# LSimon95/megatts2

Measured on AMD Instinct MI355X. Metric: mel-frames/sec (whole node), higher is better.
Workload: dtype f32; 1 GPU; C3: B=32/GPU x 1 GPU, Np=70, Tp=431, Tm=431; stages vqpe+mrte+adm+plm+decoder+vocoder; forced durations; weights=synthetic (name-seeded), parallelism=dp1 (utterance shards, one RCCL all-gather of mels per step)

## Files before the change

### include/megatts2_hip.h

```cpp
#ifndef MEGATTS2_HIP_H
#define MEGATTS2_HIP_H

#include <stddef.h>
#include <stdint.h>

#ifdef __cplusplus
extern "C" {
#endif

typedef struct mt2_model mt2_model;

typedef struct mt2_config {
    int32_t mel_bins, mrte_hidden, mrte_kernel, mrte_stride, mrte_n_layer, mrte_n_stack, mrte_n_block;
    int32_t content_ff_dim, content_n_heads, content_n_layers, phone_vocab;
    int32_t vq_mel_bins, vq_stride, vq_hidden, vq_kernel, vq_n_layers, vq_n_stacks, vq_n_blocks, vq_bins, vq_dim;
    int32_t dec_kernel, dec_hidden, dec_n_stack, dec_n_block;
    int32_t plm_layers, plm_heads, plm_vq_dim, plm_tc_dim, plm_bins;
    int32_t adm_layers, adm_heads, adm_emb_dim, adm_tc_dim, adm_tc_emb_dim;
    int32_t hg_in_dim, hg_init_channels, hg_n_up, hg_up_rates[8], hg_up_kernels[8];
    int32_t hg_n_res, hg_res_kernels[4], hg_res_dilations[4][3];
    float hg_slope;
    int32_t max_positions;
    int32_t hg_inference_padding;
    int32_t hg_reflect_pad;
// ... 174 lines not shown
    int32_t struct_bytes;
    const float* X; long long strideX; int32_t ldx, Rx;
    const int32_t* rowbase; int32_t a_mul, shift0, taps, dil, Cin;
    const float* W; long long strideW; int32_t ldw;
    const void* W3; long long w3_plane;
    const void* Wh; const float* wh_inv; long long wh_ldb, wh_gstride, wh_inv_stride;
    int32_t a_planes;
    const float* bias; long long strideB;
    const float* R; long long strideR; int32_t ldr;
    const int32_t* valid;
    float* C; long long strideC; int32_t ldc;
    int32_t M, N, groups;
    int32_t pro_act; float pro_slope; int32_t epi_act; float out_scale;
    int32_t force_cfg;
    int32_t* range_flag;
    int32_t* cfg_out;
} mt2_gemm_desc;
int mt2_op_gemm_grouped(void* stream, const mt2_gemm_desc* d);
int mt2_x3h_guard(mt2_model* m, int* tripped);
int mt2_op_gemm_x6_ln(void* stream, const float* X, int ldx, int Rx, int a_mul, int shift0, const float* W, const void* W3,
                      const float* bias, const float* R, int ldr, float* C, int ldc, int M, int N, int K, int epi_act,
                      int force_cfg, float* stat_out, int32_t* stat_nt, int32_t* stat_w, const float* ln_stat, int ln_nt,
                      int ln_w, const float* ln_s, float ln_eps);
int mt2_op_tile_major(void* stream, const float* W, int N, int K, float* out);
int mt2_op_gemm_tm(void* stream, const float* X, long long x_gstride, int ldx, int Rx, int a_mul, int shift0, const float* Wtm,
                   int Kw, int n0, int k0, long long w_gstride, int groups, const float* bias, const float* R, int ldr,
                   const int32_t* valid, float* C, long long c_gstride, int ldc, int M, int N, int K, int pro_act, float pro_slope,
                   int epi_act, const float* ln_gamma, const float* ln_beta, float ln_eps);
int mt2_op_gemm_tm_pairs(void* stream, const float* X, int ldx, int Rx, int a_mul, int shift0, const float* Wtm, int Kw,
                         const float* bias, const float* R, int ldr, float* C, int ldc, int M, int N, int K, int epi_act,
                         const float* ln_gamma, const float* ln_beta, float ln_eps, float* stat_out, const float* ln_stat, int ln_nt);
int mt2_op_layernorm(void* stream, const float* x, int ldx, const float* gamma, const float* beta, const float* R1,
                     int ldr1, const int32_t* valid, float* out, int ldo, int M, int C, float eps, int act);
int mt2_op_layernorm_ex(void* stream, const float* x, int ldx, const float* gamma, const float* beta, int rows_per_group,
                        const float* R1, int ldr1, int r1_rows, const float* R2, int ldr2, const int32_t* valid, int valid_rows,
                        float* out, int ldo, int M, int C, float eps, int act, int out_planes, int32_t* x3h_flag);
int mt2_op_ln_reduce(void* stream, const float* parts, long long pstride, int S, const float* bias, const float* R, int ldr,
                     const float* gamma, const float* beta, float* xout, int ldx, float* hout, int ldh, int M, int C, float eps,
                     int h_planes, int32_t* x3h_flag);
int mt2_op_row(void* stream, const char* op, void* const* ptrs, int nptrs, const long long* ints, int nints, const float* flts,
               int nflts);
int mt2_op_sample_rows(void* stream, const float* logits, int ld, int N, int A, const mt2_sampling* s, const uint64_t* seeds_dev,
                       const int32_t* positions_dev, int64_t* out);
int mt2_op_sample_mix_rows(void* stream, const float* logits, int ld, int N, int A, const mt2_sampling* s,
                           const uint64_t* seeds_dev, const int32_t* positions_dev, const float* gamma_dev, int64_t* out);
int mt2_op_attention(void* stream, const float* Q, int ldq, const float* K, int ldk, const float* V, int ldv,
                     float* O, int ldo, const int32_t* q_start, const int32_t* q_len, const int32_t* kv_start,
                     const int32_t* kv_len, int B, int H, int D, int max_qlen, float scale);
int mt2_op_attention_tuned(void* stream, const float* Q, int ldq, const float* K, int ldk, const float* V, int ldv,
                           float* O, int ldo, const int32_t* q_start, const int32_t* q_len, const int32_t* kv_start,
                           const int32_t* kv_len, int B, int H, int D, int max_qlen, float scale, int lds_min_qlen,
                           int lds_waves, int x6_min_qlen, int max_kvlen);
int mt2_op_attention_x3h(void* stream, const float* Q, int ldq, const float* K, int ldk, const float* V, int ldv,
                         float* O, int ldo, const int32_t* q_start, const int32_t* q_len, const int32_t* kv_start,
                         const int32_t* kv_len, int B, int H, int D, int max_qlen, float scale, int lds_waves, int max_kvlen,
                         int32_t* range_flag);
enum { MT2_ATTN_NONE = 0, MT2_ATTN_GENERIC = 1, MT2_ATTN_REG = 2, MT2_ATTN_DS = 3, MT2_ATTN_LDS = 4, MT2_ATTN_X6 = 5, MT2_ATTN_X3H = 6 };
typedef struct mt2_attn_desc {
    int32_t struct_bytes;
    const float* Q; int32_t ldq;
    const float* K; int32_t ldk;
    const float* V; int32_t ldv;
    float* O; int32_t ldo;
    const int32_t* q_start; const int32_t* q_len; const int32_t* kv_start; const int32_t* kv_len; const int32_t* o_start;
    int32_t u_qstride, u_qlen, u_kvstride, u_kvlen, u_ostride;
    int32_t B, H, D, max_qlen, max_kvlen; float scale;
    int32_t lds_min_qlen, x6_min_qlen, lds_waves, ds_short, x3h, o_planes;
    int32_t* range_flag;
    int32_t* kernel_out;
} mt2_attn_desc;
int mt2_op_attention_desc(void* stream, const mt2_attn_desc* d);
int mt2_attention_route(const mt2_attn_desc* d, int32_t* err, int32_t* kernel, int32_t* tmpl, int32_t* launch, long long* lds);
int mt2_gemm_trace_begin(mt2_model* m);
int mt2_gemm_trace_end(mt2_model* m, int cap, const char** names, int64_t* launches, double* flops, double* ms);
int mt2_gemm_trace_shapes(mt2_model* m, char* buf, int cap, int top);
int mt2_gemm_config_count(void);
const char* mt2_gemm_config_name(int idx);
int mt2_gemm_route(int M, int N, int K, int taps, int dil, int groups, int pro_act, int operands, int misaligned, int force_cfg,
                   int x3h, int* err, int* cfg, int* variant, long long* lds, int* planes);
int mt2_op_gemm_x3h_ln(void* stream, const float* X, int ldx, int Rx, int a_mul, int shift0, const float* W, const void* W3,
                       const void* Wh, const float* wh_inv, const float* bias, const float* R, int ldr, float* C, int ldc, int M, int N,
                       int K, int epi_act, int force_cfg, float* stat_out, int32_t* stat_nt, int32_t* stat_w, const float* ln_stat,
                       int ln_nt, int ln_w, const float* ln_s, float ln_eps);
int mt2_bench_gemm(void* stream, int M, int N, int K, int taps, int dil, int flags, int force_cfg, int iters,
                   int w_copies, float* avg_ms, char* cfg_name, int cfg_name_cap, double* sustained_ghz);

#ifdef __cplusplus
}
#endif
#endif
```

### megatts2_amd/csrc/capi.inc

```

#include <climits>

namespace mt2 {
extern thread_local std::string g_last_error;
void finalize_model(mt2_model& m);
}

using namespace mt2;

#define MT2_API_BEGIN try {
#define MT2_API_END                                 \
    ::CallScope::verdict_of_open_call();            \
    return 0;                                       \
    }                                               \
    catch (const std::exception& e) {               \
        g_last_error = e.what();                    \
        return -1;                                  \
    }                                               \
    catch (...) {                                   \
        g_last_error = "unknown error";             \
        return -1;                                  \
    }

enum Need { NEED_G = 1, NEED_ADM = 2, NEED_PLM = 4, NEED_VOC = 8 };
// ... 1121 lines not shown
    MT2_HIP(launch_gemm(p, (hipStream_t)stream, &o));
    MT2_API_END
}

int mt2_op_gemm_x6(void* stream, const float* X, int ldx, int Rx, int shift0, int taps, int dil, int Cin, const float* W,
                   const void* W3, const float* bias, const float* R, int ldr, const int32_t* valid, float* C, int ldc,
                   int M, int N, int pro_act, float pro_slope, int epi_act, int force_cfg) {
    MT2_API_BEGIN
    GemmP p{};
    p.X = X; p.ldx = ldx; p.Rx = Rx; p.a_mul = 1; p.shift0 = shift0; p.taps = taps; p.dil = dil; p.Cin = Cin; p.W = W;
    p.W3 = W3; p.ldw = taps * Cin; p.bias = bias; p.R = R; p.ldr = ldr; p.valid = valid; p.C = C; p.ldc = ldc; p.M = M;
    p.N = N; p.K = taps * Cin; p.groups = 1; p.pro_act = pro_act; p.pro_slope = pro_slope; p.epi_act = epi_act;
    p.out_scale = 1.0f;
    EngineOpts o;
    o.force_cfg = force_cfg;
    MT2_HIP(launch_gemm(p, (hipStream_t)stream, &o));
    MT2_API_END
}

int mt2_op_gemm_x3h(void* stream, const float* X, int ldx, int Rx, int shift0, int taps, int dil, int Cin, const float* W,
                    const void* W3, const void* Wh, const float* wh_inv, const float* bias, const float* R, int ldr,
                    const int32_t* valid, float* C, int ldc, int M, int N, int pro_act, float pro_slope, int epi_act, int force_cfg,
                    int32_t* range_flag) {
    MT2_API_BEGIN
    GemmP p{};
    p.X = X; p.ldx = ldx; p.Rx = Rx; p.a_mul = 1; p.shift0 = shift0; p.taps = taps; p.dil = dil; p.Cin = Cin; p.W = W;
    p.W3 = W3; p.Wh = Wh; p.wh_inv = wh_inv; p.ldw = taps * Cin; p.bias = bias; p.R = R; p.ldr = ldr; p.valid = valid; p.C = C;
    p.ldc = ldc; p.M = M; p.N = N; p.K = taps * Cin; p.groups = 1; p.pro_act = pro_act; p.pro_slope = pro_slope; p.epi_act = epi_act;
    p.out_scale = 1.0f;
    EngineOpts o;
    if (force_cfg >= 4000) { p.c_planes = 1; force_cfg -= 4000; }
    if (force_cfg >= 2000) { p.a_planes = 1; force_cfg -= 2000; }
    o.ldr64 = force_cfg >= 1000;
    o.force_cfg = force_cfg >= 1000 ? force_cfg - 1000 : force_cfg;
    o.x3h_flag = range_flag;
    MT2_HIP(launch_gemm(p, (hipStream_t)stream, &o));
    MT2_API_END
}
int mt2_x3h_split(const float* W, long long rows, long long row_len, uint16_t* planes, float* inv) {
    MT2_API_BEGIN
    MT2_REQUIRE(W && planes && inv && rows > 0 && row_len > 0, "bad arguments");
    x3h_split_rows(W, (size_t)rows, (size_t)row_len, planes, inv);
    MT2_API_END
}
int mt2_x3h_group_planes(long long row_len, long long w_off, long long ldw, long long strideW, long long groups, int32_t* form,
                         long long* wh_off, long long* wh_ldb, long long* wh_gstride, long long* inv_off, long long* wh_inv_stride) {
    MT2_API_BEGIN
    MT2_REQUIRE(row_len > 0 && w_off >= 0 && groups >= 1 && form && wh_off && wh_ldb && wh_gstride && inv_off && wh_inv_stride,
                "bad arguments");
    const X3hGroupPlanes g = x3h_group_planes(row_len, w_off, ldw, strideW, groups);
    *form = g.form; *wh_off = g.wh_off; *wh_ldb = g.wh_ldb; *wh_gstride = g.wh_gstride; *inv_off = g.inv_off;
    *wh_inv_stride = g.wh_inv_stride;
    MT2_API_END
}

int mt2_op_gemm_grouped(void* stream, const mt2_gemm_desc* d) {
    MT2_API_BEGIN
    MT2_REQUIRE(d != nullptr, "null descriptor");
    MT2_REQUIRE(d->struct_bytes == (int32_t)sizeof(mt2_gemm_desc), "descriptor size mismatch");
    if (d->cfg_out) *d->cfg_out = -1;
    GemmP p{};
    p.X = d->X; p.strideX = d->strideX; p.ldx = d->ldx; p.Rx = d->Rx;
    p.rowbase = d->rowbase; p.a_mul = d->a_mul; p.shift0 = d->shift0; p.taps = d->taps; p.dil = d->dil; p.Cin = d->Cin;
    p.W = d->W; p.strideW = d->strideW; p.ldw = d->ldw;
    p.W3 = d->W3; p.w3_plane = d->w3_plane;
    p.Wh = d->Wh; p.wh_inv = d->wh_inv; p.wh_ldb = d->wh_ldb; p.wh_gstride = d->wh_gstride; p.wh_inv_stride = d->wh_inv_stride;
    p.a_planes = d->a_planes;
    p.bias = d->bias; p.strideB = d->strideB; p.R = d->R; p.strideR = d->strideR; p.ldr = d->ldr; p.valid = d->valid;
    p.C = d->C; p.strideC = d->strideC; p.ldc = d->ldc;
    p.M = d->M; p.N = d->N; p.K = d->taps * d->Cin; p.groups = d->groups;
    p.pro_act = d->pro_act; p.pro_slope = d->pro_slope; p.epi_act = d->epi_act; p.out_scale = d->out_scale;
    MT2_REQUIRE(p.X && p.W && p.C && p.taps >= 1 && p.dil >= 1 && p.a_mul >= 1 && p.groups >= 1, "bad arguments");
    EngineOpts o;
    o.force_cfg = d->force_cfg;
    o.x3h_flag = d->range_flag;
    if (d->cfg_out) *d->cfg_out = gemm_route(p, o).cfg;
    MT2_HIP(launch_gemm(p, (hipStream_t)stream, &o));
    MT2_API_END
}

static int op_gemm_ln_impl(void* stream, const float* X, int ldx, int Rx, int a_mul, int shift0, const float* W, const void* W3,
                           const void* Wh, const float* wh_inv, const float* bias, const float* R, int ldr, float* C, int ldc, int M,
                           int N, int K, int epi_act, int force_cfg, float* stat_out, int32_t* stat_nt, int32_t* stat_w,
                           const float* ln_stat, int ln_nt, int ln_w, const float* ln_s, float ln_eps);
int mt2_op_gemm_x6_ln(void* stream, const float* X, int ldx, int Rx, int a_mul, int shift0, const float* W, const void* W3,
                      const float* bias, const float* R, int ldr, float* C, int ldc, int M, int N, int K, int epi_act,
                      int force_cfg, float* stat_out, int32_t* stat_nt, int32_t* stat_w, const float* ln_stat, int ln_nt,
                      int ln_w, const float* ln_s, float ln_eps) {
    return op_gemm_ln_impl(stream, X, ldx, Rx, a_mul, shift0, W, W3, nullptr, nullptr, bias, R, ldr, C, ldc, M, N, K, epi_act, force_cfg,
                           stat_out, stat_nt, stat_w, ln_stat, ln_nt, ln_w, ln_s, ln_eps);
}
int mt2_op_gemm_x3h_ln(void* stream, const float* X, int ldx, int Rx, int a_mul, int shift0, const float* W, const void* W3,
                       const void* Wh, const float* wh_inv, const float* bias, const float* R, int ldr, float* C, int ldc, int M, int N,
                       int K, int epi_act, int force_cfg, float* stat_out, int32_t* stat_nt, int32_t* stat_w, const float* ln_stat,
                       int ln_nt, int ln_w, const float* ln_s, float ln_eps) {
    return op_gemm_ln_impl(stream, X, ldx, Rx, a_mul, shift0, W, W3, Wh, wh_inv, bias, R, ldr, C, ldc, M, N, K, epi_act, force_cfg,
                           stat_out, stat_nt, stat_w, ln_stat, ln_nt, ln_w, ln_s, ln_eps);
}
static int op_gemm_ln_impl(void* stream, const float* X, int ldx, int Rx, int a_mul, int shift0, const float* W, const void* W3,
                           const void* Wh, const float* wh_inv, const float* bias, const float* R, int ldr, float* C, int ldc, int M,
                           int N, int K, int epi_act, int force_cfg, float* stat_out, int32_t* stat_nt, int32_t* stat_w,
                           const float* ln_stat, int ln_nt, int ln_w, const float* ln_s, float ln_eps) {
    MT2_API_BEGIN
    GemmP p{};
    p.Wh = Wh; p.wh_inv = wh_inv;
    p.X = X; p.ldx = ldx; p.Rx = Rx; p.a_mul = a_mul ? a_mul : 1; p.shift0 = shift0; p.taps = 1; p.dil = 1; p.Cin = K; p.W = W;
    p.W3 = W3; p.ldw = K; p.bias = bias; p.R = R; p.ldr = ldr; p.C = C; p.ldc = ldc; p.M = M; p.N = N; p.K = K; p.groups = 1;
    p.epi_act = epi_act; p.out_scale = 1.0f; p.stat_out = stat_out;
    if (ln_stat) { p.pro_act = 5; p.ln_stat = ln_stat; p.ln_nt = ln_nt; p.ln_w = ln_w; p.ln_g = ln_s; p.ln_eps = ln_eps; }
    EngineOpts o;
    o.ldr64 = force_cfg >= 1000;
    o.force_cfg = force_cfg >= 1000 ? force_cfg - 1000 : force_cfg;
    const hipError_t e = launch_gemm(p, (hipStream_t)stream, &o);
    MT2_REQUIRE(e != hipErrorNotSupported, "this tile configuration has no pair-fed LayerNorm form");
    MT2_HIP(e);
    if (stat_nt) *stat_nt = o.last_stat_nt;
    if (stat_w) *stat_w = o.last_stat_w;
    MT2_API_END
}

int mt2_op_tile_major(void* stream, const float* W, int N, int K, float* out) {
    MT2_API_BEGIN
    MT2_REQUIRE(W && out && N > 0 && K > 0 && N % 16 == 0 && K % 64 == 0, "tile-major layout needs N % 16 == 0 and K % 64 == 0");
    MT2_HIP(launch_tile_major(W, N, K, out, (hipStream_t)stream));
    MT2_API_END
}

int mt2_op_gemm_tm(void* stream, const float* X, long long x_gstride, int ldx, int Rx, int a_mul, int shift0, const float* Wtm,
                   int Kw, int n0, int k0, long long w_gstride, int groups, const float* bias, const float* R, int ldr,
                   const int32_t* valid, float* C, long long c_gstride, int ldc, int M, int N, int K, int pro_act, float pro_slope,
                   int epi_act, const float* ln_gamma, const float* ln_beta, float ln_eps) {
    MT2_API_BEGIN
    MT2_REQUIRE(X && Wtm && C && Kw % 64 == 0 && n0 % 16 == 0 && k0 % 64 == 0 && groups >= 1, "bad arguments");
    GemmP p{};
    p.X = X; p.strideX = x_gstride; p.ldx = ldx; p.Rx = Rx; p.a_mul = a_mul ? a_mul : 1; p.shift0 = shift0; p.taps = 1; p.dil = 1;
    p.Cin = K; p.K = K; p.W = nullptr; p.strideW = w_gstride; p.ldw = Kw; p.Wtm = Wtm; p.tm_n0 = n0 / 16; p.tm_k0 = k0 / 64;
    p.tm_kb = Kw / 64; p.bias = bias; p.R = R; p.ldr = ldr; p.valid = valid; p.C = C; p.strideC = c_gstride; p.ldc = ldc;
    p.M = M; p.N = N; p.groups = groups; p.pro_act = ln_gamma ? 3 : (pro_act & 0xff); p.pro_slope = pro_slope; p.epi_act = epi_act;
    p.sk_nw = (pro_act & 0x100) ? 8 : 16;
    p.out_scale = 1.0f; p.ln_g = ln_gamma; p.ln_b = ln_beta; p.ln_eps = ln_eps;
    MT2_REQUIRE(gemm_skinny_tm_eligible(p, 64), "shape not served by the tile-major weight-streaming kernel");
    MT2_HIP(launch_gemm_skinny_tm(p, (hipStream_t)stream));
    MT2_API_END
}

int mt2_op_gemm_tm_pairs(void* stream, const float* X, int ldx, int Rx, int a_mul, int shift0, const float* Wtm, int Kw,
                         const float* bias, const float* R, int ldr, float* C, int ldc, int M, int N, int K, int epi_act,
                         const float* ln_gamma, const float* ln_beta, float ln_eps, float* stat_out, const float* ln_stat, int ln_nt) {
    MT2_API_BEGIN
    MT2_REQUIRE(X && Wtm && C && Kw % 64 == 0, "bad arguments");
    GemmP p{};
    p.X = X; p.ldx = ldx; p.Rx = Rx; p.a_mul = a_mul ? a_mul : 1; p.shift0 = shift0; p.taps = 1; p.dil = 1; p.Cin = K; p.K = K;
    p.ldw = Kw; p.Wtm = Wtm; p.tm_kb = Kw / 64; p.bias = bias; p.R = R; p.ldr = ldr; p.C = C; p.ldc = ldc; p.M = M; p.N = N; p.groups = 1;
    p.pro_act = ln_gamma ? 3 : 0; p.epi_act = epi_act; p.out_scale = 1.0f; p.ln_g = ln_gamma; p.ln_b = ln_beta; p.ln_eps = ln_eps;
    p.stat_out = stat_out; p.ln_stat = ln_stat; p.ln_nt = ln_nt; p.ln_w = ln_stat ? 16 : 0;
    EngineOpts o;
    hipError_t e = launch_gemm(p, (hipStream_t)stream, &o);
    MT2_HIP(e);
    MT2_REQUIRE(!stat_out || o.last_stat_w == 16, "the launch did not take the tile-major route with the statistics epilogue");
    MT2_API_END
}

int mt2_op_layernorm(void* stream, const float* x, int ldx, const float* gamma, const float* beta, const float* R1,
                     int ldr1, const int32_t* valid, float* out, int ldo, int M, int C, float eps, int act) {
    MT2_API_BEGIN
    LnP p{};
    p.x = x; p.ldx = ldx; p.gamma = gamma; p.beta = beta; p.R1 = R1; p.ldr1 = ldr1; p.valid = valid;
    p.out = out; p.ldo = ldo; p.M = M; p.C = C; p.eps = eps; p.act = act >= 100 ? act - 100 : act;
    p.out_planes = act >= 100 ? 1 : 0;
    MT2_HIP(launch_layernorm(p, (hipStream_t)stream));
    MT2_API_END
}

int mt2_op_layernorm_ex(void* stream, const float* x, int ldx, const float* gamma, const float* beta, int rows_per_group,
                        const float* R1, int ldr1, int r1_rows, const float* R2, int ldr2, const int32_t* valid, int valid_rows,
                        float* out, int ldo, int M, int C, float eps, int act, int out_planes, int32_t* x3h_flag) {
    MT2_API_BEGIN
    LnP p{};
    p.x = x; p.ldx = ldx; p.gamma = gamma; p.beta = beta; p.rows_per_group = rows_per_group;
    p.R1 = R1; p.ldr1 = ldr1; p.r1_rows = r1_rows; p.R2 = R2; p.ldr2 = ldr2; p.valid = valid; p.valid_rows = valid_rows;
    p.out = out; p.ldo = ldo; p.M = M; p.C = C; p.eps = eps; p.act = act; p.out_planes = out_planes; p.x3h_flag = x3h_flag;
    MT2_HIP(launch_layernorm(p, (hipStream_t)stream));
    MT2_API_END
}

int mt2_op_ln_reduce(void* stream, const float* parts, long long pstride, int S, const float* bias, const float* R, int ldr,
                     const float* gamma, const float* beta, float* xout, int ldx, float* hout, int ldh, int M, int C, float eps,
                     int h_planes, int32_t* x3h_flag) {
    MT2_API_BEGIN
    LnReduceP p{};
    p.parts = parts; p.pstride = pstride; p.S = S; p.bias = bias; p.R = R; p.ldr = ldr; p.gamma = gamma; p.beta = beta;
    p.xout = xout; p.ldx = ldx; p.hout = hout; p.ldh = ldh; p.M = M; p.C = C; p.eps = eps; p.h_planes = h_planes;
    p.x3h_flag = x3h_flag;
    MT2_HIP(launch_ln_reduce(p, (hipStream_t)stream));
    MT2_API_END
}

static int row_int(long long v) {
    MT2_REQUIRE(v >= INT_MIN && v <= INT_MAX, "mt2_op_row: integer argument does not fit the launcher's int parameter");
    return (int)v;
// ... 331 lines not shown
```

### megatts2_amd/csrc/gemm_common.h

```cpp
#pragma once
#include "gemm_tiles.h"
#include "planes_store.h"
#include <type_traits>
#include <utility>

namespace mt2 {

typedef float f32x16 __attribute__((ext_vector_type(16)));
typedef float f32x4 __attribute__((ext_vector_type(4)));

template <int ACT>
__device__ __forceinline__ float apply_act(float v, float slope) {
    if (ACT == ACT_RELU) return fmaxf(v, 0.0f);
    if (ACT == ACT_LRELU) return fmaxf(v, v * slope);
    if (ACT == ACT_TANH) return tanhf(v);
    return v;
}

__device__ __forceinline__ float act_rt(int act, float v, float slope) {
    switch (act) {
        case ACT_RELU: return fmaxf(v, 0.0f);
        case ACT_LRELU: return v >= 0.0f ? v : v * slope;
        case ACT_TANH: return tanhf(v);
        case ACT_LOGCLAMP: return logf(fmaxf(v, slope));
// ... 43 lines not shown
    const int nq = p.ln_nt >> 1;
    const float4* __restrict__ pr = reinterpret_cast<const float4*>(p.ln_stat) + (long long)(ok ? src : 0) * nq;
    float4 q[NQ];
#pragma unroll
    for (int j = 0; j < NQ; ++j) {
        const int qi = j * LPR + part;
        q[j] = (ok && qi < nq) ? pr[qi] : make_float4(0.f, 0.f, 0.f, 0.f);
    }
    float sm = 0.0f;
#pragma unroll
    for (int j = 0; j < NQ; ++j) sm += q[j].x + q[j].z;
#pragma unroll
    for (int o = 1; o < LPR; o <<= 1) sm += __shfl_xor(sm, o * xm);
    const float mean = sm / (float)p.ln_nt, w = (float)p.ln_w;
    float m2 = 0.0f;
#pragma unroll
    for (int j = 0; j < NQ; ++j) {
        const int qi = j * LPR + part;
        if (qi < nq) {
            const float d0 = q[j].x - mean, d1 = q[j].z - mean;
            m2 += (q[j].y + w * d0 * d0) + (q[j].w + w * d1 * d1);
        }
    }
#pragma unroll
    for (int o = 1; o < LPR; o <<= 1) m2 += __shfl_xor(m2, o * xm);
    mu = ok ? mean : 0.0f;
    rs = ok ? 1.0f / sqrtf(m2 / ((float)p.ln_nt * w) + p.ln_eps) : 0.0f;
}

template <int TM, int TN, int EPG = 16>
__device__ __forceinline__ void epilogue(const GemmP& p, f32x16 (&acc)[TM][TN], int g, int mw, int nw, int lane,
                                         int esel = 0) {
    const float* __restrict__ bias = p.bias ? p.bias + (long long)g * p.strideB : nullptr;
    const float* __restrict__ R = p.R ? p.R + (long long)g * p.strideR : nullptr;
    float* __restrict__ C = p.C + (long long)g * p.strideC;
    const int epi_act = p.epi_act;
    const float epi_par = p.pro_slope;
    const float out_scale = p.out_scale;
#pragma unroll
    for (int j = 0; j < TN; ++j) {
        const int n = nw + j * 32 + (lane & 31);
        const bool nok = n < p.N;
        const float bv = (bias && nok) ? bias[n] : 0.0f;
#pragma unroll
        for (int i = 0; i < TM; ++i) {
#pragma unroll
            for (int e = 0; e < 16; ++e) {
                if (EPG < 16 && e / EPG != esel) continue;
                const int m = mw + i * 32 + (e & 3) + 8 * (e >> 2) + 4 * (lane >> 5);
                if (nok && m < p.M) {
                    float v = acc[i][j][e] + bv;
                    v = act_rt(epi_act, v, epi_par) * out_scale;
                    if (R) v += R[(long long)m * p.ldr + n];
                    if (p.valid && p.valid[m] == 0) v = 0.0f;
                    C[(long long)m * p.ldc + n] = v;
                }
            }
        }
    }
}

static __device__ __attribute__((aligned(16))) float g_zero16[4] = {0.f, 0.f, 0.f, 0.f};
static __device__ int g_one_i[4] = {1, 1, 1, 1};
template <int NE> struct EpiPre { float r[NE]; int v[NE]; float b; };
template <int NE>
__device__ __forceinline__ void epi_prefetch(const GemmP& p, EpiPre<NE>& q, int g, int mw, int nw, int lane, int e0) {
    const int n = nw + (lane & 31);
    const bool nok = n < p.N;
    const float* __restrict__ bias = p.bias ? p.bias + (long long)g * p.strideB + (nok ? n : 0) : g_zero16;
    const float* __restrict__ R = p.R ? p.R + (long long)g * p.strideR + (nok ? n : 0) : g_zero16;
    const long long ldr = p.R ? p.ldr : 0;
    const int* __restrict__ vp = p.valid ? p.valid : g_one_i;
    const int vs = p.valid ? 1 : 0;
    q.b = *bias;
#pragma unroll
    for (int i = 0; i < NE; ++i) {
        const int e = e0 + i;
        int m = mw + (e & 3) + 8 * (e >> 2) + 4 * (lane >> 5);
        m = m < p.M ? m : 0;
        q.r[i] = R[m * ldr];
        q.v[i] = vp[m * vs];
    }
}
template <int NE, bool STAT = false>
__device__ __forceinline__ void epilogue_pre(const GemmP& p, const float (&acc)[NE], const EpiPre<NE>& q, int g, int mw,
                                             int nw, int lane, int e0) {
    float* __restrict__ C = p.C + (long long)g * p.strideC;
    const int epi_act = p.epi_act;
    const float epi_par = p.pro_slope;
    const float out_scale = p.out_scale;
    const bool hasR = p.R != nullptr;
    const int n = nw + (lane & 31);
    const bool nok = n < p.N;
    float sv[STAT ? NE : 1], qv[STAT ? NE : 1];
#pragma unroll
    for (int i = 0; i < NE; ++i) {
        const int e = e0 + i;
        const int m = mw + (e & 3) + 8 * (e >> 2) + 4 * (lane >> 5);
        float v = 0.0f;
        if (nok && m < p.M) {
            v = acc[i] + q.b;
            v = act_rt(epi_act, v, epi_par) * out_scale;
            if (hasR) v += q.r[i];
            if (q.v[i] == 0) v = 0.0f;
            C[(long long)m * p.ldc + n] = v;
        }
        if constexpr (STAT) { sv[i] = v; qv[i] = v * v; }
    }
    if constexpr (STAT) emit_row_pairs<NE>(p, sv, qv, mw, nw >> 5, 32.0f, lane, e0);
}

template <int TM, int TN> struct EpiPreT { float r[TM][TN][16]; int v[TM][16]; float b[TN]; };
template <int TM, int TN>
__device__ __forceinline__ void epi_prefetch_t(const GemmP& p, EpiPreT<TM, TN>& q, int g, int mw, int nw, int lane) {
    const float* __restrict__ bias0 = p.bias ? p.bias + (long long)g * p.strideB : g_zero16;
    const float* __restrict__ R0 = p.R ? p.R + (long long)g * p.strideR : g_zero16;
    const long long ldr = p.R ? p.ldr : 0;
    const int* __restrict__ vp = p.valid ? p.valid : g_one_i;
    const int vs = p.valid ? 1 : 0;
#pragma unroll
    for (int j = 0; j < TN; ++j) {
        const int n = nw + j * 32 + (lane & 31);
        const int nc = (n < p.N && (p.bias || p.R)) ? n : 0;
        q.b[j] = bias0[p.bias ? nc : 0];
#pragma unroll
        for (int i = 0; i < TM; ++i)
#pragma unroll
            for (int e = 0; e < 16; ++e) {
                int m = mw + i * 32 + (e & 3) + 8 * (e >> 2) + 4 * (lane >> 5);
                m = m < p.M ? m : 0;
                q.r[i][j][e] = R0[m * ldr + (p.R ? nc : 0)];
            }
    }
#pragma unroll
    for (int i = 0; i < TM; ++i)
#pragma unroll
        for (int e = 0; e < 16; ++e) {
            int m = mw + i * 32 + (e & 3) + 8 * (e >> 2) + 4 * (lane >> 5);
            m = m < p.M ? m : 0;
            q.v[i][e] = vp[m * vs];
        }
}
template <int TM, int TN, bool STAT = false>
__device__ __forceinline__ void epilogue_pre_t(const GemmP& p, f32x16 (&acc)[TM][TN], const EpiPreT<TM, TN>& q, int g,
                                               int mw, int nw, int lane) {
    static_assert(!STAT || TM == 1, "row statistics: one 32-row block per wave");
    float* __restrict__ C = p.C + (long long)g * p.strideC;
    const int epi_act = p.epi_act;
    const float epi_par = p.pro_slope;
    const float out_scale = p.out_scale;
    const bool hasR = p.R != nullptr;
    float sv[STAT ? 16 : 1], qv[STAT ? 16 : 1];
    if constexpr (STAT) {
#pragma unroll
        for (int e = 0; e < 16; ++e) { sv[e] = 0.0f; qv[e] = 0.0f; }
    }
#pragma unroll
    for (int j = 0; j < TN; ++j) {
        const int n = nw + j * 32 + (lane & 31);
        const bool nok = n < p.N;
#pragma unroll
        for (int i = 0; i < TM; ++i)
#pragma unroll
            for (int e = 0; e < 16; ++e) {
                const int m = mw + i * 32 + (e & 3) + 8 * (e >> 2) + 4 * (lane >> 5);
                float v = 0.0f;
                if (nok && m < p.M) {
                    v = acc[i][j][e] + q.b[j];
                    v = act_rt(epi_act, v, epi_par) * out_scale;
                    if (hasR) v += q.r[i][j][e];
                    if (q.v[i][e] == 0) v = 0.0f;
                    C[(long long)m * p.ldc + n] = v;
                }
                if constexpr (STAT) { sv[e] += v; qv[e] += v * v; }
            }
    }
    if constexpr (STAT) emit_row_pairs<16>(p, sv, qv, mw, nw / (32 * TN), 32.0f * TN, lane, 0);
}

__device__ __forceinline__ float dpp_quad(float v, const int ctrl) {
    return __builtin_bit_cast(float, ctrl == 0xB1 ? __builtin_amdgcn_mov_dpp(__builtin_bit_cast(int, v), 0xB1, 0xf, 0xf, true)
                                                  : __builtin_amdgcn_mov_dpp(__builtin_bit_cast(int, v), 0x4E, 0xf, 0xf, true));
}
__device__ __forceinline__ bool epilogue_t4_ok(const GemmP& p) {
    return ((p.N | p.ldc | (p.R ? p.ldr : 0)) & 3) == 0 && (((unsigned long long)p.C | (unsigned long long)p.R | (unsigned long long)p.bias) & 15) == 0 &&
           ((p.strideC | p.strideR | p.strideB) & 3) == 0;
}
template <int TM, int TN, bool STAT = false, bool PLN = false>
__device__ __forceinline__ void epilogue_t4(const GemmP& p, f32x16 (&acc)[TM][TN], int g, int mw, int nw, int lane) {
    static_assert(!STAT || TM == 1, "row statistics: one 32-row block per wave");
    float* __restrict__ C = p.C + (long long)g * p.strideC;
    const int epi_act = p.epi_act;
    const float epi_par = p.pro_slope, out_scale = p.out_scale;
    const bool b0 = lane & 1, b1 = lane & 2;
    const int rr = (lane & 3) + 4 * (lane >> 5), c4 = ((lane & 31) >> 2) * 4;
    const bool hasR = p.R != nullptr, hasB = p.bias != nullptr;
    const float* __restrict__ bias0 = hasB ? p.bias + (long long)g * p.strideB : g_zero16;
    const float* __restrict__ R0 = hasR ? p.R + (long long)g * p.strideR : g_zero16;
    const long long ldr = hasR ? p.ldr : 0;
    const int* __restrict__ vp = p.valid ? p.valid : g_one_i;
    const int vs = p.valid ? 1 : 0;
    f32x4 bv[TN], rv[TM][TN][4];
    int vm[TM][4];
#pragma unroll
    for (int j = 0; j < TN; ++j) {
        const int n = nw + j * 32 + c4;
        bv[j] = *reinterpret_cast<const f32x4*>(bias0 + ((hasB && n < p.N) ? n : 0));
    }
#pragma unroll
    for (int i = 0; i < TM; ++i)
#pragma unroll
        for (int q = 0; q < 4; ++q) {
            int m = mw + i * 32 + 8 * q + rr;
            m = m < p.M ? m : 0;
            vm[i][q] = vp[m * vs];
#pragma unroll
            for (int j = 0; j < TN; ++j) {
                const int n = nw + j * 32 + c4;
                rv[i][j][q] = *reinterpret_cast<const f32x4*>(R0 + m * ldr + ((hasR && n < p.N) ? n : 0));
            }
        }
    float sv[STAT ? 4 : 1], qv[STAT ? 4 : 1];
    if constexpr (STAT) {
#pragma unroll
        for (int q = 0; q < 4; ++q) { sv[q] = 0.0f; qv[q] = 0.0f; }
    }
#pragma unroll
    for (int j = 0; j < TN; ++j) {
        const int n = nw + j * 32 + c4;
        const bool nok = n < p.N;
#pragma unroll
        for (int i = 0; i < TM; ++i) {
#pragma unroll
            for (int q = 0; q < 4; ++q) {
                const float x0 = acc[i][j][4 * q], x1 = acc[i][j][4 * q + 1], x2 = acc[i][j][4 * q + 2], x3 = acc[i][j][4 * q + 3];
                const float p0 = dpp_quad(x0, 0xB1), p1 = dpp_quad(x1, 0xB1), p2 = dpp_quad(x2, 0xB1), p3 = dpp_quad(x3, 0xB1);
                const float y0 = b0 ? p1 : x0, y1 = b0 ? x1 : p0, y2 = b0 ? p3 : x2, y3 = b0 ? x3 : p2;
                const float q0 = dpp_quad(y0, 0x4E), q1 = dpp_quad(y1, 0x4E), q2 = dpp_quad(y2, 0x4E), q3 = dpp_quad(y3, 0x4E);
                f32x4 v = {b1 ? q2 : y0, b1 ? q3 : y1, b1 ? y2 : q0, b1 ? y3 : q1};
                const int m = mw + i * 32 + 8 * q + rr;
                const bool in = nok && m < p.M;
                if (in) {
#pragma unroll
                    for (int e = 0; e < 4; ++e) v[e] = act_rt(epi_act, v[e] + bv[j][e], epi_par) * out_scale;
                    if (hasR) {
#pragma unroll
                        for (int e = 0; e < 4; ++e) v[e] += rv[i][j][q][e];
                    }
                    if (vm[i][q] == 0) v = f32x4{0.f, 0.f, 0.f, 0.f};
                    if (PLN && p.c_planes) {
                        if (store_planes4(C + (long long)m * p.ldc, n, v[0], v[1], v[2], v[3]) >= 65504.0f && p.x3h_flag) atomicOr(p.x3h_flag, 1);
                    } else
                    *reinterpret_cast<f32x4*>(C + (long long)m * p.ldc + n) = v;
                }
                if constexpr (STAT) {
                    if (!in) v = f32x4{0.f, 0.f, 0.f, 0.f};
                    sv[q] += (v[0] + v[1]) + (v[2] + v[3]);
                    qv[q] += (v[0] * v[0] + v[1] * v[1]) + (v[2] * v[2] + v[3] * v[3]);
                }
            }
        }
    }
    if constexpr (STAT) {
        const float w_cols = 32.0f * TN;
        const int t = nw / (32 * TN);
#pragma unroll
        for (int q = 0; q < 4; ++q) {
            float S = sv[q], Q = qv[q];
#pragma unroll
            for (int o = 4; o < 32; o <<= 1) { S += __shfl_xor(S, o); Q += __shfl_xor(Q, o); }
            const int m = mw + 8 * q + rr;
            if ((lane & 28) == 0 && m < p.M) {
                const float mean = S / w_cols;
                float2 pr;
                pr.x = mean;
                pr.y = fmaxf(Q - S * mean, 0.0f);
                *reinterpret_cast<float2*>(p.stat_out + ((long long)m * p.stat_nt + t) * 2) = pr;
            }
        }
    }
}

constexpr int PRO_APL = 3;

__device__ __forceinline__ f32x4 lds_read_b128(unsigned byte_addr) {
    f32x4 v;
    asm volatile("ds_read_b128 %0, %1" : "=v"(v) : "v"(byte_addr) : "memory");
    return v;
}

template <int OFF>
__device__ __forceinline__ f32x4 lds_read_b128_imm(unsigned byte_addr) {
    static_assert(OFF >= 0 && OFF < 65536 && (OFF & 15) == 0, "ds_read_b128 immediate offset");
    f32x4 v;
    asm volatile("ds_read_b128 %0, %1 offset:%2" : "=v"(v) : "v"(byte_addr), "n"(OFF) : "memory");
    return v;
}
template <int... Is, typename F>
__device__ __forceinline__ void static_for(std::integer_sequence<int, Is...>, F&& f) {
    (f(std::integral_constant<int, Is>{}), ...);
}

__device__ __forceinline__ void loader_priority(int prio) {
    if (prio >= 3) __builtin_amdgcn_s_setprio(3);
    else if (prio == 2) __builtin_amdgcn_s_setprio(2);
    else if (prio == 1) __builtin_amdgcn_s_setprio(1);
}

template <int N> __device__ __forceinline__ void wait_vmcnt() {
    static_assert(N >= 0 && N < 64, "vmcnt is a 6-bit field on gfx9");
    __builtin_amdgcn_s_waitcnt((N & 0xF) | ((N >> 4) << 14) | (7 << 4) | (15 << 8));
}

}
```

### megatts2_amd/csrc/gemm_dispatch.hip

```cpp
#include "gemm_tiles.h"

#include <algorithm>
#include <atomic>
#include <cstdio>
#include <cstdlib>
#include <utility>
#include <vector>

namespace mt2 {


static const TileCfg kSkinnyRows[] = {
    { CFG_SKINNY32, 32, 32, 512, 0, "skinny32_f32", {} },
    { CFG_SKINNY64, 64, 32, 512, 0, "skinny64_f32", {} },
    { CFG_SKINNYTM32, 32, 32, 512, 0, "skinnytm32_f32", {} },
    { CFG_SKINNYTM64, 64, 32, 512, 0, "skinnytm64_f32", {} },
};
static const struct { int index; const char* name; } kRetired[] = {
    {0, "retired:128x128_2x2"}, {1, "retired:64x128_2x2"}, {2, "retired:128x64_2x2"}, {4, "retired:32x128_1x4"},
    {5, "retired:32x64_1x2"}, {6, "retired:128x32_4x1"}, {7, "retired:64x32_2x1"},
    {8, "retired:dma128x128_2x2_s3"}, {9, "retired:dma128x128_2x2_s4"}, {10, "retired:dma64x128_2x2_s4"},
    {11, "retired:dma64x64_2x2_s4"}, {13, "retired:dma32x128_1x4_s4"}, {14, "retired:dma32x64_1x2_s4"},
    {19, "retired:dma64x64_2x2_k2_s4"}, {21, "retired:dma32x64_1x2_k4_s3"}, {24, "retired:dma128x64_4x2_s4"},
    {25, "retired:dma128x64_4x2_s2"}, {26, "retired:dma64x64_2x2_k1_s2"}, {27, "retired:dma128x64_4x2_k2_s2"},
// ... 115 lines not shown
        fl_all += fl;
        ++n;
    }
    if (ok && n < cap && !iv.empty()) {
        std::sort(iv.begin(), iv.end());
        double uni = 0.0, lo = iv[0].first, hi = iv[0].second;
        for (auto& x : iv) {
            if (x.first > hi) { uni += hi - lo; lo = x.first; hi = x.second; }
            else if (x.second > hi) hi = x.second;
        }
        uni += hi - lo;
        names[n] = "union"; launches[n] = (int64_t)iv.size(); flops[n] = fl_all; ms[n] = uni;
        ++n;
    }
    for (auto& r : tr) { (void)hipEventDestroy(r.e0); (void)hipEventDestroy(r.e1); }
    tr.clear();
    return ok ? n : -1;
}

template <typename F>
static hipError_t traced_launch(EngineOpts* opts, int cfg, const GemmP& p, hipStream_t s, F&& launch) {
    if (opts) opts->last_cfg = gemm_config_name(cfg);
    if (!(opts && opts->trace_on)) return launch();
    TraceRec r;
    r.cfg = cfg;
    r.flops = 2.0 * p.M * p.N * p.K * p.groups;
    r.M = p.M; r.N = p.N; r.K = p.K; r.groups = p.groups;
    if (hipEventCreate(&r.e0) != hipSuccess || hipEventCreate(&r.e1) != hipSuccess) return hipErrorUnknown;
    (void)hipEventRecord(r.e0, s);
    const hipError_t e = launch();
    (void)hipEventRecord(r.e1, s);
    opts->trace.push_back(r);
    return e;
}


static bool win_eligible(const GemmP& p) {
    return p.taps >= 2 && !p.rowbase && p.a_mul == 1 && p.groups == 1 && p.N == p.Cin &&
           (p.Cin == 32 || p.Cin == 64 || p.Cin == 128) && (p.taps - 1) * p.dil <= 64 && p.pro_act < PRO_LN;
}
static int choose_cfg(const GemmP& p, const EngineOpts& o) {
    const bool forced = o.force_cfg >= 0 && o.force_cfg < kNumCfgs;
    const bool x3h_ok = p.Wh && p.wh_inv;
    if (o.win_conv && win_eligible(p) && !forced) {
        int bi = p.Cin == 32 ? CFG_WIN256x32 : (p.Cin == 64 ? CFG_WIN256x64 : CFG_WIN128x128);
        if (o.x6_conv && p.W3) {
            bi = paired(kX6Form, bi);
            if ((o.x3h & 4) && x3h_ok) bi = paired(kX3hForm, bi);
        }
        return bi;
    }
    if (forced) return o.force_cfg;
    const long long t32 = (long long)((p.M + 31) / 32) * ((p.N + 63) / 64) * p.groups;
    const long long t32x32 = (long long)((p.M + 31) / 32) * ((p.N + 31) / 32) * p.groups;
    const long long t64 = (long long)((p.M + 63) / 64) * ((p.N + 63) / 64) * p.groups;
    const long long t128 = (long long)((p.M + 127) / 128) * ((p.N + 127) / 128) * p.groups;
    const long long t256 = (long long)((p.M + 255) / 256) * ((p.N + 127) / 128) * p.groups;
    int bi = CFG_DMA64x64_S3;
    if (p.N <= 32) bi = CFG_DMA128x32_S4;
    else if (p.N <= 64 && t128 >= 400) bi = CFG_DMA256x64_S3;
    else if (p.N <= 256 && t128 >= 400) bi = CFG_DMA128x128_S4;
    else if (t256 >= 400 || (t256 >= 200 && t256 <= 256)) bi = CFG_DMA256x128_S3;
    else if (t128 >= 400 || (t128 >= 200 && t128 <= 256)) bi = CFG_DMA128x128_S4;
    else if (t32x32 <= o.t32x32 && p.K >= 512) bi = CFG_DMA32x32_K8;
    else if (t32 <= o.t32) bi = CFG_DMA32x64_K4;
    else if (t64 <= o.t_ks4) bi = CFG_DMA64x64_K4;
    else if (t64 <= o.t_ks2) bi = CFG_DMA64x64_K2;
    if (o.x6_gemm && p.W3 && (p.K & 7) == 0 && (p.ldw & 7) == 0 && (p.pro_act < PRO_LN || p.pro_act == PRO_LNX) && p.N > 64) {
        const bool h1 = (o.x3h & 1) && x3h_ok;
        if (t256 >= o.t_x6_256) bi = CFG_X6LDR256x128;
        else if (t128 >= (h1 ? o.t_x3h_128 : o.t_x6_128)) bi = CFG_X6LDR128x128;
        if (o.x6_ks && p.taps == 1) {
            if (bi == CFG_DMA32x64_K4 && p.K % (BK * 4) == 0 && o.x6_ks != 5) bi = paired(kX6Form, bi);
            else if ((bi == CFG_DMA64x64_K4 || bi == CFG_DMA64x64_K2) && p.K % (BK * 2) == 0) bi = paired(kX6Form, bi);
            else if ((o.x6_ks == 2 || o.x6_ks == 4) && bi == CFG_DMA32x32_K8 && p.K % (BK * 8) == 0) bi = paired(kX6Form, bi);
        }
    }
    if ((o.x3h & 1) && x3h_ok && (bi == CFG_X6LDR128x128 || bi == CFG_X6LDR256x128)) bi = paired(kX3hForm, bi);
    if ((o.x3h & 2) && x3h_ok && cfg_table().row[bi]->pipe == PIPE_X6 && cfg_table().row[bi]->x6_ks) bi = paired(kX3hForm, bi);
    return bi;
}


static bool a_planes_ok(const GemmP& p, const TileCfg& c, bool stat) {
    return c.pipe == PIPE_X3H && !c.win_qs && p.pro_act == ACT_NONE && !stat && (p.Cin % BK) == 0 && (p.ldx % BK) == 0 &&
           !(p.groups > 1 && (p.strideX % BK) != 0) && p.a_mul == 1 && !p.rowbase && !(((unsigned long long)p.X) & 127);
}
static bool c_planes_ok(const GemmP& p, const TileCfg& c, bool stat) {
    return c.pipe == PIPE_X3H && !c.x6_ks && !c.win_qs && p.groups == 1 && !p.R && !stat && (p.N & 31) == 0 && (p.ldc & 31) == 0 &&
           (((unsigned long long)p.C) & 127) == 0 && (((unsigned long long)p.bias) & 15) == 0 && ((p.strideC | p.strideB) & 3) == 0 && p.Wh && p.wh_inv && p.M > 64;
}
static long long wh_ldb_of(const GemmP& p) { return p.wh_ldb ? p.wh_ldb : 4ll * ((p.ldw + 31) / 32 * 32); }
static long long wh_gstride_of(const GemmP& p) { return p.groups > 1 && p.wh_gstride == 0 ? p.strideW * 4 : p.wh_gstride; }

GemmRoute gemm_route(const GemmP& p, const EngineOpts& o) {
    GemmRoute r{hipSuccess, -1, V_NONE, 0, 0, 0};
    const auto fail = [&r](hipError_t e) { r.err = e; r.lds = 0; r.stat_nt = r.stat_w = 0; return r; };
    if (p.M <= 0 || p.N <= 0 || p.groups <= 0) return r;
    if ((p.Cin & 3) || (p.ldx & 3) || (p.ldw & 3) || p.K != p.taps * p.Cin) return fail(hipErrorInvalidValue);
    if (p.pro_act < 0 || p.pro_act > PRO_LNX) return fail(hipErrorInvalidValue);
    if (p.c_planes && p.M <= 64) return fail(hipErrorNotSupported);
    if (p.pro_act == PRO_LNX && (p.taps != 1 || p.groups != 1 || !p.ln_g || !p.ln_stat || p.ln_nt < 2 || p.ln_nt > 32 ||
                                 (p.ln_nt & 1) || p.ln_w <= 0 || p.ln_nt * p.ln_w != p.K || (((unsigned long long)p.ln_stat) & 15)))
        return fail(hipErrorInvalidValue);
    const bool sk_forced = o.force_cfg == CFG_SKINNY32 || o.force_cfg == CFG_SKINNY64;
    const bool tm_forced = o.force_cfg == CFG_SKINNYTM32 || o.force_cfg == CFG_SKINNYTM64;
    if (tm_forced || (!p.a_planes && o.skinny_tm && o.skinny_rows > 0 && o.force_cfg < 0 &&
                      gemm_skinny_tm_eligible(p, o.skinny_rows))) {
        if (!gemm_skinny_tm_eligible(p, 64)) return fail(hipErrorInvalidValue);
        r.cfg = p.M <= 32 ? CFG_SKINNYTM32 : CFG_SKINNYTM64;
        if (p.stat_out) {
            const int nt = p.N / 16;
            if (p.groups == 1 && (nt & 1) == 0 && nt <= 64 && ((((unsigned long long)p.stat_out) & 15) == 0)) { r.stat_nt = nt; r.stat_w = 16; }
        }
        return r;
    }
    if (sk_forced || (o.skinny_rows > 0 && o.force_cfg < 0 && gemm_skinny_eligible(p, o.skinny_rows))) {
        if (!gemm_skinny_eligible(p, 64)) return fail(hipErrorInvalidValue);
        r.cfg = p.M <= 32 ? CFG_SKINNY32 : CFG_SKINNY64;
        return r;
    }
    r.cfg = choose_cfg(p, o);
    const TileCfg* c = cfg_table().row[r.cfg];
    if (!c) return fail(hipErrorNotSupported);
    const bool x3h = c->pipe == PIPE_X3H, x3h_ldr = x3h && !c->x6_ks && !c->win_qs;
    const bool has_lnx = c->stat_w && c->fn[V_LNX];
    if (p.pro_act == PRO_LNX && !has_lnx) return fail(hipErrorNotSupported);
    bool stat = p.stat_out != nullptr;
    if (x3h_ldr && (p.pro_act == PRO_LNX || stat)) {
        const bool t4 = ((p.N | p.ldc | (p.R ? p.ldr : 0)) & 3) == 0 && ((p.strideC | p.strideR | p.strideB) & 3) == 0 &&
                        (((unsigned long long)p.C | (unsigned long long)p.R | (unsigned long long)p.bias) & 15) == 0;
        if (!t4) {
            if (p.pro_act == PRO_LNX) return fail(hipErrorNotSupported);
            stat = false;
        }
    }
    if (stat) {
        const int nt = c->stat_w ? p.N / c->stat_w : 0;
        stat = has_lnx && (p.pro_act == ACT_NONE || p.pro_act == PRO_LNX) && p.groups == 1 && p.N % c->stat_w == 0 && nt >= 2 &&
               nt <= 32 && (nt & 1) == 0 && ((((unsigned long long)p.stat_out) & 15) == 0);
        if (stat) { r.stat_w = c->stat_w; r.stat_nt = nt; }
    }
    if (p.a_planes && !a_planes_ok(p, *c, stat)) return fail(hipErrorNotSupported);
    if (p.c_planes && !c_planes_ok(p, *c, stat)) return fail(hipErrorNotSupported);
    if (p.pro_act == PRO_LN || p.pro_act == PRO_LNA) return fail(hipErrorNotSupported);
    r.variant = p.a_planes ? V_APLANES : ((p.pro_act == PRO_LNX || stat) ? V_LNX : (GemmVariant)p.pro_act);
    r.lds = c->lds;
    if (r.variant == V_LNX && !c->x6_ks) r.lds += (size_t)c->bm * 2 * sizeof(float);
    if (x3h) {
        if (!p.Wh || !p.wh_inv || (p.K & 7) || (p.ldw & 7)) return fail(hipErrorInvalidValue);
        if ((((unsigned long long)p.Wh) & 127) || (wh_ldb_of(p) & 127) || (wh_gstride_of(p) & 127)) return fail(hipErrorInvalidValue);
    } else if (c->pipe == PIPE_X6 && (!p.W3 || (p.K & 7) || (p.ldw & 7))) return fail(hipErrorInvalidValue);
    if (c->x6_ks && (p.taps != 1 || p.K % (BK * c->x6_ks) != 0)) return fail(hipErrorInvalidValue);
    if (c->win_qs) {
        if (!win_eligible(p) || p.Cin != 32 * c->win_qs) return fail(hipErrorInvalidValue);
        const int wrp = (c->bm + (p.taps - 1) * p.dil + 7) & ~7;
        r.lds = c->lds + (size_t)c->win_qs * wrp * BK * sizeof(float);
    }
    if (!c->fn[r.variant]) return fail(hipErrorNotSupported);
    return r;
}

static GemmP normalise(GemmP p) {
    if (p.taps <= 0) p.taps = 1;
    if (p.groups <= 0) p.groups = 1;
    if (p.a_mul == 0) p.a_mul = 1;
    p.K = p.taps * p.Cin;
    if (p.ldw == 0) p.ldw = p.K;
    return p;
}
bool gemm_takes_planes(const GemmP& p_in, const EngineOpts& o) {
    const GemmP p = normalise(p_in);
    if (!(o.x3h & 3) || o.force_cfg >= 0 || p.M <= 64 || !p.Wh || !p.wh_inv) return false;
    const TileCfg* c = cfg_table().row[choose_cfg(p, o)];
    return a_planes_ok(p, *c, p.stat_out != nullptr) && c->fn[V_APLANES] != nullptr;
}
bool gemm_writes_planes(const GemmP& p_in, const EngineOpts& o) {
    const GemmP p = normalise(p_in);
    if (!(o.x3h & 1) || o.force_cfg >= 0 || p.M <= 64) return false;
    return c_planes_ok(p, *cfg_table().row[choose_cfg(p, o)], p.stat_out != nullptr);
}

static std::atomic<unsigned long long> g_attr_done[kNumCfgs][kGemmVariants];

hipError_t launch_gemm(const GemmP& p_in, hipStream_t s, EngineOpts* opts) {
    static const EngineOpts kDefaults;
    const EngineOpts& o = opts ? *opts : kDefaults;
    const GemmRoute r = gemm_route(p_in, o);
    if (r.cfg < 0 && r.err == hipSuccess) return hipSuccess;
    if (opts) { opts->last_stat_nt = r.stat_nt; opts->last_stat_w = r.stat_w; }
    if (r.err != hipSuccess) return r.err;
    GemmP p = p_in;
    if (!r.stat_nt) p.stat_out = nullptr;
    p.stat_nt = r.stat_nt; p.stat_w = r.stat_w;
    if (r.cfg == CFG_SKINNYTM32 || r.cfg == CFG_SKINNYTM64) {
        p.sk_nw = o.skinny_nw;
        return traced_launch(opts, r.cfg, p, s, [&] { return launch_gemm_skinny_tm(p, s); });
    }
    if (r.cfg == CFG_SKINNY32 || r.cfg == CFG_SKINNY64) return traced_launch(opts, r.cfg, p, s, [&] { return launch_gemm_skinny(p, s); });
    const TileCfg* c = cfg_table().row[r.cfg];
    if (c->pipe == PIPE_X3H) {
        p.wh_ldb = wh_ldb_of(p);
        p.wh_gstride = wh_gstride_of(p);
        p.x3h_flag = o.x3h_flag;
    }
    if (c->pipe == PIPE_X6 && p.w3_plane == 0) p.w3_plane = (long long)p.N * p.ldw;
    const GemmKernel fn = c->fn[r.variant];
    const size_t lds_attr = c->win_qs ? c->lds + (size_t)c->win_qs * ((c->bm + 64 + 7) & ~7) * BK * sizeof(float) : r.lds;
    const hipError_t e = dyn_lds_once(g_attr_done[r.cfg][r.variant], reinterpret_cast<const void*>(fn), lds_attr);
    if (e != hipSuccess) return e;
    const int tiles = ((p.M + c->bm - 1) / c->bm) * ((p.N + c->bn - 1) / c->bn);
    p.epi_t4 = 1;
    p.ldr_prio = o.ldr_prio;
    p.ldr64 = o.ldr64 ? 1 : 0;
    const dim3 grid(tiles, 1, p.groups), block(c->threads);
    return traced_launch(opts, r.cfg, p, s, [&] {
        hipLaunchKernelGGL(fn, grid, block, r.lds, s, p);
        return hipGetLastError();
    });
}

}
```

### megatts2_amd/csrc/gemm_tiles.h

```cpp
#pragma once
#include "mt2_kernels.h"

namespace mt2 {

constexpr int BK = 32;
constexpr int PRO_LN = 3;
constexpr int PRO_LNA = 4;
constexpr int PRO_LNX = 5;

enum GemmVariant : int {
    V_NONE, V_RELU, V_LRELU,
    V_APLANES,
    V_LNX,
    kGemmVariants
};
static_assert((int)V_NONE == ACT_NONE && (int)V_RELU == ACT_RELU && (int)V_LRELU == ACT_LRELU, "the activation variants are indexed by Act");

enum GemmPipe : int { PIPE_F32, PIPE_X6, PIPE_X3H };

enum CfgIndex : int {
    CFG_64x64 = 3,
    CFG_DMA64x64_S3 = 12, CFG_DMA128x32_S4 = 15, CFG_DMA256x128_S3 = 16, CFG_DMA128x128_S4 = 17,
    CFG_DMA64x64_K2 = 18, CFG_DMA64x64_K4 = 20, CFG_DMA32x64_K4 = 22, CFG_DMA256x64_S3 = 23, CFG_DMA32x32_K8 = 28,
    CFG_WIN256x32 = 30, CFG_WIN256x64 = 31, CFG_WIN128x128 = 32,
    CFG_X6WIN256x32 = 34,
    CFG_X6LDR256x128 = 51, CFG_X6LDR128x128 = 55,
    CFG_X6WINL256x64 = 58, CFG_X6WINL128x128 = 59,
    CFG_X6KS32x64_K4 = 84, CFG_X6KS64x64_K2 = 85, CFG_X6KS32x32_K8 = 86,
    CFG_SKINNY32 = 87, CFG_SKINNY64 = 88, CFG_SKINNYTM32 = 89, CFG_SKINNYTM64 = 90,
    CFG_X3HKS32x64_K4 = 95, CFG_X3HKS64x64_K2 = 96, CFG_X3HKS32x32_K8 = 97,
    CFG_X3HWIN256x32 = 98, CFG_X3HWIN256x64 = 99, CFG_X3HWIN128x128 = 100,
    CFG_X3HLDR128x128 = 103,
    kNumCfgs = 106
};

typedef void (*GemmKernel)(GemmP);
struct TileCfg {
    CfgIndex index;
    int bm, bn, threads;
    size_t lds;
    const char* name;
    GemmKernel fn[kGemmVariants];
    GemmPipe pipe = PIPE_F32;
    int win_qs = 0;
    int x6_ks = 0;
    int stat_w = 0;
};
struct TileRows { const TileCfg* rows; int n; };
TileRows gemm_f32_tile_rows();
TileRows gemm_x3h_tile_rows();

}
```

### megatts2_amd/csrc/gemm_x3h.hip

```cpp
#include "gemm_common.h"

#include <atomic>

#ifndef MT2_X3H_ABLATE
#define MT2_X3H_ABLATE 0
#endif
#define MT2_ABL_NOINGEST (MT2_X3H_ABLATE == 2 || MT2_X3H_ABLATE == 5 || MT2_X3H_ABLATE == 6 || MT2_X3H_ABLATE == 7)
#define MT2_ABL_NOSPLIT (MT2_X3H_ABLATE == 3 || MT2_X3H_ABLATE == 5 || MT2_X3H_ABLATE == 6)
#define MT2_ABL_NOBARRIER (MT2_X3H_ABLATE == 6 || MT2_X3H_ABLATE == 7)
#ifdef MT2_X3H_NO_BUFFER_LOADS
#define MT2_BUFFER_LOADS false
#else
#define MT2_BUFFER_LOADS true
#endif

namespace mt2 {

typedef _Float16 f16x8 __attribute__((ext_vector_type(8)));
typedef _Float16 f16x2 __attribute__((ext_vector_type(2)));
typedef float f32x2 __attribute__((ext_vector_type(2)));
typedef unsigned u32x4 __attribute__((ext_vector_type(4)));

constexpr float kX3hLoScale = 2048.0f, kX3hLoInv = 1.0f / 2048.0f, kX3hMaxIn = 65504.0f;

// ... 130 lines not shown
                for (int j = 0; j < A_IT; ++j) {
                    const int src = abase[j] + dsrc;
                    const long long off = (unsigned)src < (unsigned)Rx ? (long long)src * ldx + (s_cc + akl[j]) : zoff_x;
                    __builtin_amdgcn_global_load_lds((const __attribute__((address_space(1))) void*)(X + off),
                                                     (__attribute__((address_space(3))) void*)(As + j * NL * 256), 16, 0, 0);
                }
#pragma unroll
                for (int j = 0; j < B_IT; ++j) {
                    const long long off = wofs[j] >= 0 ? wofs[j] + (long long)kchunk * 4 : zoff_w;
                    __builtin_amdgcn_global_load_lds((const __attribute__((address_space(1))) void*)(Wh + off),
                                                     (__attribute__((address_space(3))) void*)(Bs + j * NL * 1024), 16, 0, 0);
                }
                s_cc += BK;
                if (multi_tap && s_cc == Cin) { s_cc = 0; ++s_tap; }
                return;
            }
#pragma unroll
            for (int j = 0; j < A_IT; ++j) {
                const int k = kchunk + akl[j];
                int tap = 0, cc = k;
                if (multi_tap) { tap = k / Cin; cc = k - tap * Cin; }
                const int src = abase[j] + tap * dil;
                const bool ok = (k < Kt) & ((unsigned)src < (unsigned)Rx);
                const long long off = ok ? (long long)src * ldx + cc : zoff_x;
                __builtin_amdgcn_global_load_lds((const __attribute__((address_space(1))) void*)(X + off),
                                                 (__attribute__((address_space(3))) void*)(As + j * NL * 256), 16, 0, 0);
            }
#pragma unroll
            for (int j = 0; j < B_IT; ++j) {
                const bool ok = (kchunk < Kt) & (wofs[j] >= 0);
                const long long off = ok ? wofs[j] + (long long)kchunk * 4 : zoff_w;
                __builtin_amdgcn_global_load_lds((const __attribute__((address_space(1))) void*)(Wh + off),
                                                 (__attribute__((address_space(3))) void*)(Bs + j * NL * 1024), 16, 0, 0);
            }
        };
#pragma unroll
        for (int st = 0; st < NST - 1; ++st)
            if (st < nk) issue(st, st);
#ifdef MT2_PHASE_TIMING
        const bool lprobe = p.dbg != nullptr && bid == (int)(gridDim.x / 2) && lw == 0;
        unsigned long long lacc[3] = {0, 0, 0}, lprev = lprobe ? __builtin_readcyclecounter() : 0ull;
#define MT2_LT(i_) do { if (lprobe) { const unsigned long long t_ = __builtin_readcyclecounter(); lacc[i_] += t_ - lprev; lprev = t_; } } while (0)
#define MT2_LT_END() do { if (lprobe && lane == 0) { p.dbg[11] = lacc[0]; p.dbg[12] = lacc[1]; p.dbg[13] = lacc[2]; } } while (0)
#else
#define MT2_LT(i_) do { } while (0)
#define MT2_LT_END() do { } while (0)
#endif
        static_assert(NST >= 3, "cross-chunk form: chunk c-1 is still being read at barrier c");
        for (int c = 0; c < nk; ++c) {
            if (c == 0) { if (NST - 2 < nk) wait_vmcnt<(NST - 2) * L>(); else wait_vmcnt<0>(); }
            else if (c + NST - 3 < nk) wait_vmcnt<(NST - 3) * L>();
            else wait_vmcnt<0>();
            MT2_LT(0);
            if (!MT2_ABL_NOBARRIER || c == 0)
            __builtin_amdgcn_s_barrier();
            MT2_LT(1);
#if MT2_ABL_NOINGEST
            if (c >= 1 && c + NST - 2 < nk && c < 2) {
#else
            if (c >= 1 && c + NST - 2 < nk) {
#endif
                const int cs = (c + NST - 2) % NST;
                issue(c + NST - 2, cs);
            }
            MT2_LT(2);
        }
        MT2_LT_END();
#undef MT2_LT
#undef MT2_LT_END
        return;
    }

    const int wave = wave_all;
    const int wm = wave / WGN, wn = wave % WGN;
    float inv_s[TN];
    {
        const float* __restrict__ inv = p.wh_inv + (long long)g * p.wh_inv_stride;
#pragma unroll
        for (int j = 0; j < TN; ++j) {
            const int n = n0 + wn * WTN + j * 32 + (lane & 31);
            inv_s[j] = inv[n < p.N ? n : 0];
        }
    }
    constexpr bool LNXOK = TM == 1 && TM * TN <= 2 && PRO == PRO_LNX;
    const bool lnx = LNXOK && p.pro_act == PRO_LNX;
    [[maybe_unused]] float* lnstat = reinterpret_cast<float*>(ring + NST * STAGE);
    if constexpr (LNXOK) {
        if (lnx) {
            constexpr int LPR = NW * 64 / BM;
            static_assert(LPR >= 1 && LPR <= 16 && (LPR & (LPR - 1)) == 0, "lanes per row");
            const int tc = wave * 64 + lane, row = tc / LPR;
            float mu, rs;
            lnx_row_stats<LPR>(p, m0 + row, tc % LPR, 1, mu, rs);
            if (tc % LPR == 0) { lnstat[2 * row] = mu; lnstat[2 * row + 1] = rs; }
            asm volatile("s_waitcnt lgkmcnt(0)" ::: "memory");
        }
    }

    f32x16 acc[TM][TN], acl[TM][TN];
#pragma unroll
    for (int i = 0; i < TM; ++i)
#pragma unroll
        for (int j = 0; j < TN; ++j)
#pragma unroll
            for (int e = 0; e < 16; ++e) { acc[i][j][e] = 0.0f; acl[i][j][e] = 0.0f; }

    const float pro_slope = p.pro_slope;
    const int half = lane >> 5;
    const unsigned lds0 = (unsigned)(unsigned long long)(__attribute__((address_space(3))) char*)ring;
    const int swza = (lane >> 1) & 7;
    const unsigned a_lane = lds0 + ((wm * WTM + (lane & 31)) * BK) * 4;
    const int nrow = wn * WTN + (lane & 31);
    const int swzb = (nrow >> 1) & 7;
    const unsigned b_lane = lds0 + STAGE_A + nrow * 128;
    unsigned koffa[2][2], koffb[2][2];
#pragma unroll
    for (int b = 0; b < 2; ++b) {
        koffa[b][0] = (unsigned)(((b * 4 + half * 2) ^ swza) * 16);
        koffa[b][1] = (unsigned)(((b * 4 + half * 2 + 1) ^ swza) * 16);
        koffb[b][0] = (unsigned)(((b * 2 + half) ^ swzb) * 16);
        koffb[b][1] = (unsigned)(((4 + b * 2 + half) ^ swzb) * 16);
    }

    float amax = 0.0f;
    const bool probe = p.dbg != nullptr && bid == (int)(gridDim.x / 2) && wave == 0;
    unsigned long long treal0 = 0, tcyc0 = 0;
    if (probe) {
        treal0 = __builtin_amdgcn_s_memrealtime();
        tcyc0 = __builtin_readcyclecounter();
        if (lane == 0) p.dbg[9] = treal0 - t_entry;
    }
    if constexpr (PRO == PRO_APL) {
        constexpr int N1 = 2 * TM + 2 * TN;
        static_assert(N1 <= 15, "lgkmcnt is four bits wide");
        u32x4 ra[2][TM][2];
        u32x4 rb[2][2][TN];
        unsigned koffah[2][2];
#pragma unroll
        for (int b = 0; b < 2; ++b) {
            koffah[b][0] = (unsigned)(((b * 2 + half) ^ swza) * 16);
            koffah[b][1] = (unsigned)(((4 + b * 2 + half) ^ swza) * 16);
        }
        auto fetch_a = [&](int b, unsigned sa) __attribute__((always_inline)) {
            const unsigned vh = sa + koffah[b][0], vl = sa + koffah[b][1];
            static_for(std::make_integer_sequence<int, TM>{}, [&](auto ic) {
                constexpr int i = decltype(ic)::value;
                ra[b][i][0] = __builtin_bit_cast(u32x4, lds_read_b128_imm<i * 32 * BK * 4>(vh));
                ra[b][i][1] = __builtin_bit_cast(u32x4, lds_read_b128_imm<i * 32 * BK * 4>(vl));
            });
        };
        auto fetch_b = [&](int b, unsigned sb) __attribute__((always_inline)) {
            const unsigned vb0 = sb + koffb[b][0], vb1 = sb + koffb[b][1];
            static_for(std::make_integer_sequence<int, TN>{}, [&](auto ic) {
                constexpr int j = decltype(ic)::value;
                rb[b][0][j] = __builtin_bit_cast(u32x4, lds_read_b128_imm<j * 32 * 128>(vb0));
                rb[b][1][j] = __builtin_bit_cast(u32x4, lds_read_b128_imm<j * 32 * 128>(vb1));
            });
        };
        auto tie_set = [&](int b) __attribute__((always_inline)) {
#pragma unroll
            for (int i = 0; i < TM; ++i) asm volatile("" : "+v"(ra[b][i][0]), "+v"(ra[b][i][1]));
#pragma unroll
            for (int pl = 0; pl < 2; ++pl)
#pragma unroll
                for (int j = 0; j < TN; ++j) asm volatile("" : "+v"(rb[b][pl][j]));
        };
        auto products = [&](int b) __attribute__((always_inline)) {
#pragma unroll
            for (int i = 0; i < TM; ++i) {
                const f16x8 Ah = __builtin_bit_cast(f16x8, ra[b][i][0]), Al = __builtin_bit_cast(f16x8, ra[b][i][1]);
#pragma unroll
                for (int j = 0; j < TN; ++j)
                    acl[i][j] = __builtin_amdgcn_mfma_f32_32x32x16_f16(Ah, __builtin_bit_cast(f16x8, rb[b][1][j]), acl[i][j], 0, 0, 0);
#pragma unroll
                for (int j = 0; j < TN; ++j)
                    acc[i][j] = __builtin_amdgcn_mfma_f32_32x32x16_f16(Ah, __builtin_bit_cast(f16x8, rb[b][0][j]), acc[i][j], 0, 0, 0);
#pragma unroll
                for (int j = 0; j < TN; ++j)
                    acl[i][j] = __builtin_amdgcn_mfma_f32_32x32x16_f16(Al, __builtin_bit_cast(f16x8, rb[b][0][j]), acl[i][j], 0, 0, 0);
            }
        };
        __builtin_amdgcn_s_barrier();
        asm volatile("" ::: "memory");
        fetch_a(0, a_lane); fetch_b(0, b_lane); fetch_a(1, a_lane); fetch_b(1, b_lane);
        __builtin_amdgcn_sched_barrier(0);
        int stn = 1 % NST;
        auto chunk = [&](auto last_c) __attribute__((always_inline)) {
            constexpr bool last = decltype(last_c)::value;
            const unsigned sa = a_lane + (unsigned)stn * STAGE, sb = b_lane + (unsigned)stn * STAGE;
#pragma unroll
            for (int b = 0; b < 2; ++b) {
                if (last && b == 1) asm volatile("s_waitcnt lgkmcnt(0)" ::: "memory");
                else asm volatile("s_waitcnt lgkmcnt(%0)" :: "n"(N1) : "memory");
                tie_set(b);
                __builtin_amdgcn_sched_barrier(0);
                products(b);
                __builtin_amdgcn_sched_barrier(0);
                if constexpr (!last) {
                    if (b == 0) {
                        __builtin_amdgcn_s_barrier();
                        asm volatile("" ::: "memory");
                    }
                    fetch_a(b, sa);
                    fetch_b(b, sb);
                    __builtin_amdgcn_sched_barrier(0);
                }
            }
            stn = stn + 1 == NST ? 0 : stn + 1;
        };
        for (int c = 0; c + 1 < nk; ++c) chunk(std::false_type{});
        chunk(std::true_type{});
    } else {
    f32x4 ra[2][TM][2];
    u32x4 rb[2][2][TN];
    u32x4 pln[2][2];
// ... 67 lines not shown
        auto chunk = [&](auto last_c) __attribute__((always_inline)) {
            constexpr bool last = decltype(last_c)::value;
            const unsigned sa = a_lane + (unsigned)stn * STAGE, sb = b_lane + (unsigned)stn * STAGE;
#pragma unroll
            for (int s = 0; s < FS; ++s) {
                const int b = s / TM, i = s % TM;
                if (i == 0 && TM > 1) {
                    if constexpr (last) asm volatile("s_waitcnt lgkmcnt(0)" ::: "memory");
                    else asm volatile("s_waitcnt lgkmcnt(%0)" :: "n"(N1) : "memory");
                    tie_b(b);
                    __builtin_amdgcn_sched_barrier(0);
                }
                if (i == TM - 1) {
                    if constexpr (!last) {
                        if (b == 0 && !MT2_ABL_NOBARRIER) {
                            __builtin_amdgcn_s_barrier();
                            asm volatile("" ::: "memory");
                        }
                        fetch_a(b, sa);
                        __builtin_amdgcn_sched_barrier(0);
                        asm volatile("s_waitcnt lgkmcnt(%0)" :: "n"(N1) : "memory");
                    } else {
                        asm volatile("s_waitcnt lgkmcnt(0)" ::: "memory");
                    }
                    tie_a(b ^ 1);
                    if (TM == 1) tie_b(b);
                    __builtin_amdgcn_sched_barrier(0);
                }
                const bool more = s + 1 < FS || !last;
                if (more) {
                    const int s2 = (s + 1) % FS, b2 = s2 / TM, i2 = s2 % TM;
                    if (b2 == b) tie(b2, i2);
                    split2_f16<PRO>(ra[b2][i2][0], ra[b2][i2][1], pro_slope, pln[(s + 1) & 1][0], pln[(s + 1) & 1][1], amax);
                    products(b, i, pln[s & 1]);
                    pattern();
                    __builtin_amdgcn_sched_barrier(0);
                } else {
                    products(b, i, pln[s & 1]);
                    __builtin_amdgcn_sched_barrier(0);
                }
                if constexpr (!last) {
                    if (i == TM - 1) {
                        fetch_b(b, sb);
                        __builtin_amdgcn_sched_barrier(0);
                    }
                }
            }
            stn = stn + 1 == NST ? 0 : stn + 1;
        };
        for (int c = 0; c + 1 < nk; ++c) chunk(std::false_type{});
        chunk(std::true_type{});
    }
    }
    unsigned long long t_loop_end = 0;
    if (probe) {
        t_loop_end = __builtin_amdgcn_s_memrealtime();
        if (lane == 0) {
            p.dbg[6] = (unsigned long long)nk;
            p.dbg[7] = t_loop_end - treal0;
            p.dbg[8] = __builtin_readcyclecounter() - tcyc0;
        }
    }
    if (p.x3h_flag != nullptr && __builtin_amdgcn_ballot_w64(amax >= kX3hMaxIn) != 0ull && lane == 0) atomicOr(p.x3h_flag, 1);
#pragma unroll
    for (int i = 0; i < TM; ++i)
#pragma unroll
        for (int j = 0; j < TN; ++j)
#pragma unroll
            for (int e = 0; e < 16; ++e) acc[i][j][e] = __builtin_fmaf(acl[i][j][e], kX3hLoInv, acc[i][j][e]) * inv_s[j];

    if constexpr (LNXOK) {
        if (lnx) {
#pragma unroll
            for (int j = 0; j < TN; ++j) {
                const int n = n0 + wn * WTN + j * 32 + (lane & 31);
                const float s_n = n < p.N ? p.ln_g[n] : 0.0f;
#pragma unroll
                for (int e = 0; e < 16; ++e) {
                    const float2 st2 = reinterpret_cast<const float2*>(lnstat)[wm * WTM + (e & 3) + 8 * (e >> 2) + 4 * half];
                    acc[0][j][e] = st2.y * (acc[0][j][e] - st2.x * s_n);
                }
            }
        }
        if (p.stat_out) epilogue_t4<TM, TN, true>(p, acc, g, m0 + wm * WTM, n0 + wn * WTN, lane);
        else epilogue_t4<TM, TN, false, true>(p, acc, g, m0 + wm * WTM, n0 + wn * WTN, lane);
    } else if (p.epi_t4 && epilogue_t4_ok(p)) epilogue_t4<TM, TN, false, true>(p, acc, g, m0 + wm * WTM, n0 + wn * WTN, lane);
    else epilogue<TM, TN>(p, acc, g, m0 + wm * WTM, n0 + wn * WTN, lane);
    if (probe) {
        __builtin_amdgcn_s_waitcnt(0);
        const unsigned long long t_end = __builtin_amdgcn_s_memrealtime();
        if (lane == 0) p.dbg[10] = t_end - t_loop_end;
    }
}

template <int BM, int BN, int WGM, int WGN, int KS, int NL, int NST, int PRO>
__global__ __launch_bounds__((WGM * WGN * KS + NL) * 64) void gemm_x3h_ks_kernel(GemmP p) {
    constexpr int NW = WGM * WGN;
    constexpr int NWC = NW * KS;
    constexpr int PA = BM / 8, PB = BN / 8;
    constexpr int PG = PA + PB, PT = PG * KS;
    constexpr int LW = PT / NL;
    constexpr int STAGE_A = BM * BK * 4, STAGE_B = PB * 1024, STAGE = STAGE_A + STAGE_B;
    constexpr int EPG = 16 / KS;
    static_assert(BM == 32 * WGM && BN == 32 * WGN, "one 32x32 tile per wave");
    static_assert(PT % NL == 0 && 16 % KS == 0 && NST >= 2 && (NST - 2) * LW < 64 && NWC + NL <= 16, "config");
    static_assert(KS * NST * STAGE >= NWC * 16 * 64 * 4 || KS == 1, "the K-group reduction reuses the ring");

    extern __shared__ __attribute__((aligned(16))) float smem[];
    char* ring = reinterpret_cast<char*>(smem);
    const int tid = threadIdx.x, lane = tid & 63;
    const int wave_all = __builtin_amdgcn_readfirstlane(tid >> 6);
    const int g = blockIdx.z;
    const unsigned long long t_entry = p.dbg ? __builtin_amdgcn_s_memrealtime() : 0ull;
    const int ntm = (p.M + BM - 1) / BM, ntn = (p.N + BN - 1) / BN, nt = ntm * ntn;
    const int bid = blockIdx.x;
    const int xcd = bid & 7, q = nt >> 3, r = nt & 7;
    const int tile = (xcd < r ? xcd * (q + 1) : r * (q + 1) + (xcd - r) * q) + (bid >> 3);
    const bool nmajor = p.M < p.N;
    const int m0 = (nmajor ? tile % ntm : tile / ntn) * BM, n0 = (nmajor ? tile / ntm : tile % ntn) * BN;
    const int nr = p.K / (BK * KS);

    if (wave_all >= NWC) {
        loader_priority(p.ldr_prio);
        const int lw = wave_all - NWC;
        const char* __restrict__ Xb = reinterpret_cast<const char*>(p.X + (long long)g * p.strideX);
        const char* __restrict__ Wb = reinterpret_cast<const char*>(p.Wh) + (long long)g * p.wh_gstride;
        const char* zero = reinterpret_cast<const char*>(g_zero16);
        const char* base[LW];
        long long rowb[LW];
        int ldsoff[LW];
        int grp[LW];
#pragma unroll
        for (int j = 0; j < LW; ++j) {
            const int pi = j * NL + lw, kg = pi / PG, w = pi - kg * PG;
            grp[j] = kg;
            if (w < PA) {
                const int m = m0 + w * 8 + (lane >> 3);
                int src = kInvalidRow;
                if (m < p.M) src = p.rowbase ? p.rowbase[m] : m * p.a_mul + p.shift0;
                const int kl = ((lane & 7) ^ ((w * 4 + (lane >> 4)) & 7)) * 4;
                base[j] = Xb; ldsoff[j] = w * 1024;
                rowb[j] = (unsigned)src < (unsigned)p.Rx ? ((long long)src * p.ldx + kl) * 4 : -1;
            } else {
                const int bp = w - PA;
                const int nl = bp * 8 + (lane >> 3), n = n0 + nl;
                const int sl = (lane & 7) ^ ((nl >> 1) & 7);
                base[j] = Wb; ldsoff[j] = STAGE_A + bp * 1024;
                rowb[j] = n < p.N ? (long long)n * p.wh_ldb + sl * 16 : -1;
            }
        }
        wait_vmcnt<0>();
        constexpr unsigned kOut = 0x80000000u;
        const bool fast32 = MT2_BUFFER_LOADS && !p.ldr64 && (long long)p.Rx * p.ldx * 4 + (long long)p.K * 4 < 0x7fffffffll && (long long)p.N * p.wh_ldb < 0x7fffffffll;
        const __amdgpu_buffer_rsrc_t rs_x = __builtin_amdgcn_make_buffer_rsrc(const_cast<char*>(Xb), 0, (int)kOut, 0x00020000);
        const __amdgpu_buffer_rsrc_t rs_w = __builtin_amdgcn_make_buffer_rsrc(const_cast<char*>(Wb), 0, (int)kOut, 0x00020000);
        unsigned vo[LW];
#pragma unroll
        for (int j = 0; j < LW; ++j) vo[j] = rowb[j] >= 0 ? (unsigned)rowb[j] + (unsigned)grp[j] * (BK * 4) : kOut;
        auto issue = [&](int rd, int st) __attribute__((always_inline)) {
            if (fast32) {
                const int so = rd * KS * BK * 4;
#pragma unroll
                for (int j = 0; j < LW; ++j) {
                    const bool is_a = base[j] == Xb;
                    __builtin_amdgcn_raw_ptr_buffer_load_lds(is_a ? rs_x : rs_w,
                                                             (__attribute__((address_space(3))) void*)(ring + (grp[j] * NST + st) * STAGE + ldsoff[j]),
                                                             16, (int)vo[j], so, 0, 0);
                }
                return;
            }
#pragma unroll
            for (int j = 0; j < LW; ++j) {
                const long long kb = (long long)(rd * KS + grp[j]) * BK * 4;
                const char* src = rowb[j] >= 0 ? base[j] + rowb[j] + kb : zero;
                __builtin_amdgcn_global_load_lds((const __attribute__((address_space(1))) void*)src,
                                                 (__attribute__((address_space(3))) void*)(ring + (grp[j] * NST + st) * STAGE + ldsoff[j]),
                                                 16, 0, 0);
            }
        };
#pragma unroll
        for (int st = 0; st < NST - 1; ++st)
            if (st < nr) issue(st, st);
#ifdef MT2_PHASE_TIMING
        const bool lprobe = p.dbg != nullptr && bid == (int)(gridDim.x / 2) && lw == 0;
        unsigned long long lacc[3] = {0, 0, 0}, lprev = lprobe ? __builtin_readcyclecounter() : 0ull;
#define MT2_LT(i_) do { if (lprobe) { const unsigned long long t_ = __builtin_readcyclecounter(); lacc[i_] += t_ - lprev; lprev = t_; } } while (0)
#else
#define MT2_LT(i_) do { } while (0)
#endif
        int st = 0;
        for (int rd = 0; rd < nr; ++rd) {
            if (rd + NST - 2 < nr) wait_vmcnt<(NST - 2) * LW>();
            else wait_vmcnt<0>();
            MT2_LT(0);
            __builtin_amdgcn_s_barrier();
            MT2_LT(1);
            if (rd + NST - 1 < nr) issue(rd + NST - 1, st == 0 ? NST - 1 : st - 1);
            MT2_LT(2);
            st = st + 1 == NST ? 0 : st + 1;
        }
#ifdef MT2_PHASE_TIMING
        if (lprobe && lane == 0) { p.dbg[11] = lacc[0]; p.dbg[12] = lacc[1]; p.dbg[13] = lacc[2]; }
#endif
#undef MT2_LT
        return;
    }

    const int kg = wave_all / NW, wave = wave_all % NW;
    const int wm = wave / WGN, wn = wave % WGN;
    EpiPre<EPG> pre;
    epi_prefetch<EPG>(p, pre, g, m0 + wm * 32, n0 + wn * 32, lane, kg * EPG);
    float inv_s;
    {
        const int n = n0 + wn * 32 + (lane & 31);
        inv_s = (p.wh_inv + (long long)g * p.wh_inv_stride)[n < p.N ? n : 0];
    }
    float ln_mu = 0.0f, ln_rs = 0.0f;
    const bool lnx = PRO == PRO_LNX && p.pro_act == PRO_LNX;
    if (lnx) lnx_row_stats<2>(p, m0 + wm * 32 + (lane & 31), lane >> 5, 32, ln_mu, ln_rs);
    f32x16 acc, acl;
#pragma unroll
    for (int e = 0; e < 16; ++e) { acc[e] = 0.0f; acl[e] = 0.0f; }
    const float pro_slope = p.pro_slope;
    const int half = lane >> 5;
    const unsigned lds0 = (unsigned)(unsigned long long)(__attribute__((address_space(3))) char*)ring + (unsigned)(kg * NST) * STAGE;
    const int swza = (lane >> 1) & 7;
    const unsigned a_lane = lds0 + ((wm * 32 + (lane & 31)) * BK) * 4;
    const int nrow = wn * 32 + (lane & 31);
    const int swzb = (nrow >> 1) & 7;
    const unsigned b_lane = lds0 + STAGE_A + nrow * 128;
    unsigned koffa[2][2], koffb[2][2];
#pragma unroll
    for (int b = 0; b < 2; ++b) {
        koffa[b][0] = (unsigned)(((b * 4 + half * 2) ^ swza) * 16);
        koffa[b][1] = (unsigned)(((b * 4 + half * 2 + 1) ^ swza) * 16);
        koffb[b][0] = (unsigned)(((b * 2 + half) ^ swzb) * 16);
        koffb[b][1] = (unsigned)(((4 + b * 2 + half) ^ swzb) * 16);
    }
    float amax = 0.0f;
    f32x4 ra[2][2];
    u32x4 rb[2][2], pln[2];
    auto fetch = [&](int b, unsigned sa, unsigned sb) {
        ra[b][0] = lds_read_b128(sa + (PRO == PRO_APL ? (unsigned)(((b * 2 + half) ^ swza) * 16) : koffa[b][0]));
        ra[b][1] = lds_read_b128(sa + (PRO == PRO_APL ? (unsigned)(((4 + b * 2 + half) ^ swza) * 16) : koffa[b][1]));
        rb[b][0] = __builtin_bit_cast(u32x4, lds_read_b128(sb + koffb[b][0]));
        rb[b][1] = __builtin_bit_cast(u32x4, lds_read_b128(sb + koffb[b][1]));
    };
    auto wait_block = [&](int b) {
        asm volatile("s_waitcnt lgkmcnt(0)" ::: "memory");
        asm volatile("" : "+v"(ra[b][0]), "+v"(ra[b][1]), "+v"(rb[b][0]), "+v"(rb[b][1]));
    };
    auto products = [&](int b) {
        const f16x8 Ah = __builtin_bit_cast(f16x8, pln[0]), Al = __builtin_bit_cast(f16x8, pln[1]);
        acl = __builtin_amdgcn_mfma_f32_32x32x16_f16(Ah, __builtin_bit_cast(f16x8, rb[b][1]), acl, 0, 0, 0);
        acc = __builtin_amdgcn_mfma_f32_32x32x16_f16(Ah, __builtin_bit_cast(f16x8, rb[b][0]), acc, 0, 0, 0);
        acl = __builtin_amdgcn_mfma_f32_32x32x16_f16(Al, __builtin_bit_cast(f16x8, rb[b][0]), acl, 0, 0, 0);
    };
    const bool probe = p.dbg != nullptr && blockIdx.x == gridDim.x / 2 && wave_all == 0;
    unsigned long long treal0 = 0, tcyc0 = 0;
    if (probe) {
        treal0 = __builtin_amdgcn_s_memrealtime();
        tcyc0 = __builtin_readcyclecounter();
        if (lane == 0) p.dbg[9] = treal0 - t_entry;
    }
    int st = 0;
    for (int rd = 0; rd < nr; ++rd) {
        __builtin_amdgcn_s_barrier();
        asm volatile("" ::: "memory");
        const unsigned sa = a_lane + (unsigned)st * STAGE, sb = b_lane + (unsigned)st * STAGE;
        fetch(0, sa, sb);
        fetch(1, sa, sb);
        __builtin_amdgcn_sched_barrier(0);
        wait_block(0);
        wait_block(1);
        __builtin_amdgcn_sched_barrier(0);
        if constexpr (PRO == PRO_APL) { pln[0] = __builtin_bit_cast(u32x4, ra[0][0]); pln[1] = __builtin_bit_cast(u32x4, ra[0][1]); }
        else split2_f16<PRO>(ra[0][0], ra[0][1], pro_slope, pln[0], pln[1], amax);
        products(0);
        __builtin_amdgcn_sched_barrier(0);
        if constexpr (PRO == PRO_APL) { pln[0] = __builtin_bit_cast(u32x4, ra[1][0]); pln[1] = __builtin_bit_cast(u32x4, ra[1][1]); }
        else split2_f16<PRO>(ra[1][0], ra[1][1], pro_slope, pln[0], pln[1], amax);
        products(1);
        __builtin_amdgcn_sched_barrier(0);
        st = st + 1 == NST ? 0 : st + 1;
    }
    unsigned long long t_loop_end = 0;
    if (probe) {
        t_loop_end = __builtin_amdgcn_s_memrealtime();
        if (lane == 0) {
            p.dbg[6] = (unsigned long long)(nr * KS);
            p.dbg[7] = t_loop_end - treal0;
            p.dbg[8] = __builtin_readcyclecounter() - tcyc0;
        }
    }
    if (p.x3h_flag != nullptr && __builtin_amdgcn_ballot_w64(amax >= kX3hMaxIn) != 0ull && lane == 0) atomicOr(p.x3h_flag, 1);
#pragma unroll
    for (int e = 0; e < 16; ++e) acc[e] = __builtin_fmaf(acl[e], kX3hLoInv, acc[e]);
    if constexpr (KS > 1) {
        __syncthreads();
        float* red = smem + ((kg * NW + wave) * 16) * 64 + lane;
#pragma unroll
        for (int e = 0; e < 16; ++e) red[e * 64] = acc[e];
        __syncthreads();
        float out[EPG];
#pragma unroll
        for (int i = 0; i < EPG; ++i) {
            const int e = kg * EPG + i;
            float v = 0.0f;
#pragma unroll
            for (int g2 = 0; g2 < KS; ++g2) v += smem[(((g2 * NW + wave) * 16) + e) * 64 + lane];
            out[i] = v * inv_s;
        }
        if (lnx) {
            const int n = n0 + wn * 32 + (lane & 31);
            const float s_n = n < p.N ? p.ln_g[n] : 0.0f;
#pragma unroll
            for (int i = 0; i < EPG; ++i) {
                const int e = kg * EPG + i, rr = (e & 3) + 8 * (e >> 2) + 4 * half;
                out[i] = __shfl(ln_rs, rr) * (out[i] - __shfl(ln_mu, rr) * s_n);
            }
        }
        if (PRO == PRO_LNX && p.stat_out) epilogue_pre<EPG, PRO == PRO_LNX>(p, out, pre, g, m0 + wm * 32, n0 + wn * 32, lane, kg * EPG);
        else epilogue_pre<EPG>(p, out, pre, g, m0 + wm * 32, n0 + wn * 32, lane, kg * EPG);
    } else {
        float out[16];
#pragma unroll
        for (int e = 0; e < 16; ++e) out[e] = acc[e] * inv_s;
        if (lnx) {
            const int n = n0 + wn * 32 + (lane & 31);
            const float s_n = n < p.N ? p.ln_g[n] : 0.0f;
#pragma unroll
            for (int e = 0; e < 16; ++e) {
                const int rr = (e & 3) + 8 * (e >> 2) + 4 * half;
                out[e] = __shfl(ln_rs, rr) * (out[e] - __shfl(ln_mu, rr) * s_n);
            }
        }
        if (PRO == PRO_LNX && p.stat_out) epilogue_pre<16, PRO == PRO_LNX>(p, out, pre, g, m0 + wm * 32, n0 + wn * 32, lane, 0);
        else epilogue_pre<16>(p, out, pre, g, m0 + wm * 32, n0 + wn * 32, lane, 0);
    }
    if (probe) {
        __builtin_amdgcn_s_waitcnt(0);
        const unsigned long long t_end = __builtin_amdgcn_s_memrealtime();
        if (lane == 0) p.dbg[10] = t_end - t_loop_end;
    }
}

template <int QS, int BM, int BN, int WGM, int WGN, int NST, int PRO, int NL>
__global__ __launch_bounds__((WGM * WGN + NL) * 64) void conv_win_x3h_kernel(GemmP p) {
    constexpr int NW = WGM * WGN;
    constexpr int WTM = BM / WGM, WTN = BN / WGN;
    constexpr int TM = WTM / 32, TN = WTN / 32;
    constexpr int BPIECES = BN / 8;
    constexpr int NI = NL;
    constexpr int B_IT = (BPIECES + NI - 1) / NI;
    constexpr int STAGE_B = B_IT * NI * 1024;
    static_assert(NL > 0 && WTM % 32 == 0 && WTN % 32 == 0 && NST >= 3 && (NST - 2) * B_IT < 64 && BN == 32 * QS, "config");

    extern __shared__ __attribute__((aligned(16))) float smem[];
    const int tid = threadIdx.x, lane = tid & 63;
    const int wave_all = __builtin_amdgcn_readfirstlane(tid >> 6);
    const bool loader = wave_all >= NW;
    const int wave = loader ? wave_all - NW : wave_all;
    const int wm = wave / WGN, wn = wave % WGN;
    const int taps = p.taps, dil = p.dil;
    const int WR = BM + (taps - 1) * dil, WRp = (WR + 7) & ~7;
    char* ring = reinterpret_cast<char*>(smem);
    float* win = smem + NST * STAGE_B / 4;

    const int ntm = (p.M + BM - 1) / BM;
    const int bid = blockIdx.x;
    const int xcd = bid & 7, qq = ntm >> 3, rr = ntm & 7;
    const int tile = (xcd < rr ? xcd * (qq + 1) : rr * (qq + 1) + (xcd - rr) * qq) + (bid >> 3);
    const int m0 = tile * BM;

    const float* __restrict__ X = p.X;
    const char* __restrict__ Wh = reinterpret_cast<const char*>(p.Wh);
    const long long zoff_x = (const float*)g_zero16 - X;
    const long long zoff_w = (const char*)g_zero16 - Wh;
    const int ldx = p.ldx, Rx = p.Rx, Kt = p.K;

    {
        const int lrow = lane >> 3;
        const int ppq = WRp >> 3, pieces = QS * ppq;
        const int row_first = m0 + p.shift0;
        for (int pc = wave_all; pc < pieces; pc += NW + NL) {
            const int q = pc / ppq, r8 = pc - q * ppq;
            const int row = r8 * 8 + lrow;
            const int grow = row_first + row;
            const int slot = (lane & 7) ^ ((row >> 1) & 7);
            const bool ok = (row < WR) & ((unsigned)grow < (unsigned)Rx);
            const long long off = ok ? (long long)grow * ldx + q * 32 + slot * 4 : zoff_x;
            __builtin_amdgcn_global_load_lds((const __attribute__((address_space(1))) void*)(X + off),
                                             (__attribute__((address_space(3))) void*)(win + (q * WRp + r8 * 8) * 32), 16, 0, 0);
        }
    }
    const int nk = Kt / 32;
    long long wofs[B_IT];
#pragma unroll
    for (int j = 0; j < B_IT; ++j) {
        const int pc = j * NI + wave;
        const int n = pc * 8 + (lane >> 3);
        const int sl = (lane & 7) ^ ((n >> 1) & 7);
        wofs[j] = (pc < BPIECES && n < p.N) ? (long long)n * p.wh_ldb + sl * 16 : -1;
    }
    constexpr unsigned kOut = 0x80000000u;
    const bool fast32 = MT2_BUFFER_LOADS && !p.ldr64 && (long long)p.N * p.wh_ldb < 0x7fffffffll;
    const __amdgpu_buffer_rsrc_t rs_w = __builtin_amdgcn_make_buffer_rsrc(const_cast<char*>(Wh), 0, (int)kOut, 0x00020000);
    unsigned vob[B_IT];
#pragma unroll
    for (int j = 0; j < B_IT; ++j) vob[j] = wofs[j] >= 0 ? (unsigned)wofs[j] : kOut;
    auto issue = [&](int c, int st) __attribute__((always_inline)) {
        char* Bs = ring + st * STAGE_B + wave * 1024;
        if (fast32) {
#pragma unroll
            for (int j = 0; j < B_IT; ++j)
                __builtin_amdgcn_raw_ptr_buffer_load_lds(rs_w, (__attribute__((address_space(3))) void*)(Bs + j * NI * 1024), 16, (int)vob[j], c * 128, 0, 0);
            return;
        }
#pragma unroll
        for (int j = 0; j < B_IT; ++j) {
            const long long off = wofs[j] >= 0 ? wofs[j] + (long long)c * 128 : zoff_w;
// ... 112 lines not shown
            constexpr int j = decltype(ic)::value;
            rb[b][0][j] = __builtin_bit_cast(u32x4, lds_read_b128_imm<j * 32 * 128>(vb0));
            rb[b][1][j] = __builtin_bit_cast(u32x4, lds_read_b128_imm<j * 32 * 128>(vb1));
        });
    };
    auto tie_set = [&](int b) __attribute__((always_inline)) {
#pragma unroll
        for (int i = 0; i < TM; ++i) asm volatile("" : "+v"(ra[b][i][0]), "+v"(ra[b][i][1]));
#pragma unroll
        for (int pl = 0; pl < 2; ++pl)
#pragma unroll
            for (int j = 0; j < TN; ++j) asm volatile("" : "+v"(rb[b][pl][j]));
    };
    auto products = [&](int b) __attribute__((always_inline)) {
#pragma unroll
        for (int i = 0; i < TM; ++i) {
            const f16x8 Ah = __builtin_bit_cast(f16x8, ra[b][i][0]), Al = __builtin_bit_cast(f16x8, ra[b][i][1]);
#pragma unroll
            for (int j = 0; j < TN; ++j)
                acl[i][j] = __builtin_amdgcn_mfma_f32_32x32x16_f16(Ah, __builtin_bit_cast(f16x8, rb[b][1][j]), acl[i][j], 0, 0, 0);
#pragma unroll
            for (int j = 0; j < TN; ++j)
                acc[i][j] = __builtin_amdgcn_mfma_f32_32x32x16_f16(Ah, __builtin_bit_cast(f16x8, rb[b][0][j]), acc[i][j], 0, 0, 0);
#pragma unroll
            for (int j = 0; j < TN; ++j)
                acl[i][j] = __builtin_amdgcn_mfma_f32_32x32x16_f16(Al, __builtin_bit_cast(f16x8, rb[b][0][j]), acl[i][j], 0, 0, 0);
        }
    };
    __builtin_amdgcn_s_barrier();
    asm volatile("" ::: "memory");
    {
        const unsigned sa0 = lds_win + (unsigned)(arow0 * BK) * 4;
        const int swz0 = (arow0 >> 1) & 7;
        fetch_a(0, sa0, swz0); fetch_b(0, b_lane); fetch_a(1, sa0, swz0); fetch_b(1, b_lane);
    }
    __builtin_amdgcn_sched_barrier(0);
    int stn = 1 % NST, tapn = 0, qn = 1;
    if (qn == QS) { qn = 0; tapn = 1; }
    auto chunk = [&](auto last_c) __attribute__((always_inline)) {
        constexpr bool last = decltype(last_c)::value;
        const int arow = arow0 + tapn * dil;
        const int swza = (arow >> 1) & 7;
        const unsigned sa = lds_win + (unsigned)((qn * WRp + arow) * BK) * 4;
        const unsigned sb = b_lane + (unsigned)stn * STAGE_B;
#pragma unroll
        for (int b = 0; b < 2; ++b) {
            if (last && b == 1) asm volatile("s_waitcnt lgkmcnt(0)" ::: "memory");
            else asm volatile("s_waitcnt lgkmcnt(%0)" :: "n"(N1) : "memory");
            tie_set(b);
            __builtin_amdgcn_sched_barrier(0);
            products(b);
            __builtin_amdgcn_sched_barrier(0);
            if constexpr (!last) {
                if (b == 0) {
                    __builtin_amdgcn_s_barrier();
                    asm volatile("" ::: "memory");
                }
                fetch_a(b, sa, swza);
                fetch_b(b, sb);
                __builtin_amdgcn_sched_barrier(0);
            }
        }
        stn = stn + 1 == NST ? 0 : stn + 1;
        if (++qn == QS) { qn = 0; ++tapn; }
    };
    for (int c = 0; c + 1 < nk; ++c) chunk(std::false_type{});
    chunk(std::true_type{});
#pragma unroll
    for (int i = 0; i < TM; ++i)
#pragma unroll
        for (int j = 0; j < TN; ++j)
#pragma unroll
            for (int e = 0; e < 16; ++e) acc[i][j][e] = __builtin_fmaf(acl[i][j][e], kX3hLoInv, acc[i][j][e]) * inv_s[j];
    if (epilogue_t4_ok(p)) epilogue_t4<TM, TN>(p, acc, 0, m0 + wm * WTM, wn * WTN, lane);
    else epilogue<TM, TN>(p, acc, 0, m0 + wm * WTM, wn * WTN, lane);
}


#define MT2_X3H_LDR(IDX_, BM_, BN_, WM_, WN_, NL_, NST_)                                                                    \
    { IDX_, BM_, BN_, (WM_* WN_ + NL_) * 64, (size_t)NST_ * ((size_t)BM_ * BK * 4 + (size_t)(2 * BN_ / 16) * 1024),         \
      "x3hldr" #BM_ "x" #BN_ "_" #WM_ "x" #WN_ "+" #NL_ "_s" #NST_ "xc",                                                    \
      { gemm_x3h_ldr_kernel<BM_, BN_, WM_, WN_, NL_, NST_, ACT_NONE>, gemm_x3h_ldr_kernel<BM_, BN_, WM_, WN_, NL_, NST_, ACT_RELU>, \
        gemm_x3h_ldr_kernel<BM_, BN_, WM_, WN_, NL_, NST_, ACT_LRELU>, gemm_x3h_ldr_kernel<BM_, BN_, WM_, WN_, NL_, NST_, PRO_APL>, \
        gemm_x3h_ldr_kernel<BM_, BN_, WM_, WN_, NL_, NST_, PRO_LNX> }, PIPE_X3H, 0, 0, (BN_) / (WN_) }
#define MT2_X3H_KS(IDX_, BM_, BN_, WM_, WN_, KS_, NL_, NST_)                                                                \
    { IDX_, BM_, BN_, (WM_* WN_ * KS_ + NL_) * 64, (size_t)KS_ * NST_ * ((size_t)BM_ * BK * 4 + (size_t)(2 * BN_ / 16) * 1024), \
      "x3hks" #BM_ "x" #BN_ "_" #WM_ "x" #WN_ "_k" #KS_ "+" #NL_ "_s" #NST_,                                                \
      { gemm_x3h_ks_kernel<BM_, BN_, WM_, WN_, KS_, NL_, NST_, ACT_NONE>, gemm_x3h_ks_kernel<BM_, BN_, WM_, WN_, KS_, NL_, NST_, ACT_RELU>, \
        gemm_x3h_ks_kernel<BM_, BN_, WM_, WN_, KS_, NL_, NST_, ACT_LRELU>, gemm_x3h_ks_kernel<BM_, BN_, WM_, WN_, KS_, NL_, NST_, PRO_APL>, \
        gemm_x3h_ks_kernel<BM_, BN_, WM_, WN_, KS_, NL_, NST_, PRO_LNX> }, PIPE_X3H, 0, KS_, 32 }
#define MT2_X3H_WIN(IDX_, QS_, BM_, BN_, WM_, WN_, NST_, NL_)                                                               \
    { IDX_, BM_, BN_, (WM_* WN_ + NL_) * 64, (size_t)NST_ * (((2 * BN_ / 16 + NL_ - 1) / NL_) * NL_ * 1024),                  \
      "x3hwin" #BM_ "x" #BN_ "_" #WM_ "x" #WN_ "+" #NL_ "_s" #NST_,                                                          \
      { conv_win_x3h_kernel<QS_, BM_, BN_, WM_, WN_, NST_, ACT_NONE, NL_>, conv_win_x3h_kernel<QS_, BM_, BN_, WM_, WN_, NST_, ACT_RELU, NL_>, \
        conv_win_x3h_kernel<QS_, BM_, BN_, WM_, WN_, NST_, ACT_LRELU, NL_> }, PIPE_X3H, QS_ }

static const TileCfg kX3hRows[] = {
    MT2_X3H_KS(CFG_X3HKS32x64_K4, 32, 64, 1, 2, 4, 8, 2),
    MT2_X3H_KS(CFG_X3HKS64x64_K2, 64, 64, 2, 2, 2, 8, 3),
    MT2_X3H_KS(CFG_X3HKS32x32_K8, 32, 32, 1, 1, 8, 8, 2),
    MT2_X3H_WIN(CFG_X3HWIN256x32, 1, 256, 32, 8, 1, 4, 4),
    MT2_X3H_WIN(CFG_X3HWIN256x64, 2, 256, 64, 8, 1, 4, 4),
    MT2_X3H_WIN(CFG_X3HWIN128x128, 4, 128, 128, 4, 2, 3, 4),
    MT2_X3H_LDR(CFG_X3HLDR128x128, 128, 128, 4, 2, 4, 4),
};
TileRows gemm_x3h_tile_rows() { return {kX3hRows, (int)(sizeof(kX3hRows) / sizeof(kX3hRows[0]))}; }

}
```

### megatts2_amd/csrc/model_stages.hip

```cpp
#include "mt2_model.h"
#include "x3h_planes.h"
#include "gemm_tiles.h"

#include <algorithm>
#include <cmath>
#include <cstring>
#include <numeric>

namespace mt2 {



static RowSet make_rows(const int* lens, int B, int G) {
    RowSet rs;
    rs.B = B; rs.G = G;
    rs.len.assign(lens, lens + B);
    rs.off.resize(B);
    int r = G;
    for (int b = 0; b < B; ++b) {
        MT2_REQUIRE(lens[b] >= 0, "negative utterance length");
        rs.off[b] = r;
        r += lens[b] + G;
        rs.maxlen = std::max(rs.maxlen, lens[b]);
    }
// ... 27 lines not shown
struct Ctx {
    mt2_model& m;
    hipStream_t s;
    Arena& ws;
};

static void attach_planes(const mt2_model& m, GemmP& p) {
    if (p.W3 || m.planes.empty()) return;
    auto it = std::upper_bound(m.planes.begin(), m.planes.end(), p.W,
                               [](const float* w, const PlaneRange& r) { return w < r.base; });
    if (it == m.planes.begin()) return;
    --it;
    if (p.W < it->base + it->n) {
        p.W3 = it->p3 + (p.W - it->base);
        p.w3_plane = (long long)it->n;
        const int ldw = p.ldw ? p.ldw : (p.taps > 0 ? p.taps : 1) * p.Cin;
        const X3hGroupPlanes g = x3h_group_planes((long long)it->row_len, (long long)(p.W - it->base), ldw, p.strideW, p.groups);
        if (it->ph && g.form != X3H_NO_PLANES) {
            p.Wh = reinterpret_cast<const char*>(it->ph) + g.wh_off;
            p.wh_ldb = g.wh_ldb;
            p.wh_gstride = g.wh_gstride;
            p.wh_inv = it->inv + g.inv_off;
            p.wh_inv_stride = g.wh_inv_stride;
        }
    }
}
static void attach_tm(const mt2_model& m, GemmP& p) {
    if (p.Wtm || m.tm.empty() || p.M > 64) return;
    auto it = std::upper_bound(m.tm.begin(), m.tm.end(), p.W, [](const float* w, const TmRange& r) { return w < r.base; });
    if (it == m.tm.begin()) return;
    --it;
    if (p.W >= it->base + it->n) return;
    const size_t off = (size_t)(p.W - it->base);
    const int n0 = (int)(off / it->K), k0 = (int)(off % it->K);
    if ((n0 & 15) || (k0 & 63) || p.ldw != it->K) return;
    p.Wtm = it->tm; p.tm_n0 = n0 / 16; p.tm_k0 = k0 / 64; p.tm_kb = it->K / 64;
}
static void gemm(const Ctx& c, GemmP p) {
    attach_planes(c.m, p);
    if (p.ldw == 0) p.ldw = p.taps > 0 ? p.taps * p.Cin : p.Cin;
    attach_tm(c.m, p);
    if (p.taps <= 0) p.taps = 1;
    if (p.dil <= 0) p.dil = 1;
    if (p.a_mul == 0) p.a_mul = 1;
    if (p.groups <= 0) p.groups = 1;
    if (p.out_scale == 0.0f) p.out_scale = 1.0f;
    p.K = p.taps * p.Cin;
    if (p.ldw == 0) p.ldw = p.K;
    MT2_HIP(launch_gemm(p, c.s, &c.m.opts));
}

static void linear(const Ctx& c, const float* x, int ldx, int M, const float* W, const float* b, int N, int K,
                   float* y, int ldy, const float* R = nullptr, int ldr = 0, const int* valid = nullptr,
                   int epi_act = ACT_NONE, bool a_planes = false, bool c_planes = false) {
    GemmP p{};
    p.X = x; p.ldx = ldx; p.Rx = M; p.Cin = K; p.W = W; p.bias = b; p.R = R; p.ldr = ldr; p.valid = valid;
    p.C = y; p.ldc = ldy; p.M = M; p.N = N; p.epi_act = epi_act; p.a_planes = a_planes ? 1 : 0; p.c_planes = c_planes ? 1 : 0;
    gemm(c, p);
}
static GemmP planned(const Ctx& c, GemmP p) {
    if (p.taps <= 0) p.taps = 1;
    if (p.dil <= 0) p.dil = 1;
    if (p.a_mul == 0) p.a_mul = 1;
    if (p.groups <= 0) p.groups = 1;
    if (p.out_scale == 0.0f) p.out_scale = 1.0f;
    p.K = p.taps * p.Cin;
    if (p.ldw == 0) p.ldw = p.K;
    attach_planes(c.m, p);
    return p;
}
static bool linear_takes_planes(const Ctx& c, const float* x, int ldx, int M, const float* W, const float* b, int N, int K,
                                float* y, int ldy, int epi_act) {
    if (!(c.m.opts.a_planes & 1)) return false;
    GemmP p{};
    p.X = x; p.ldx = ldx; p.Rx = M; p.Cin = K; p.W = W; p.bias = b; p.C = y; p.ldc = ldy; p.M = M; p.N = N; p.epi_act = epi_act;
    p.taps = 1; p.dil = 1; p.a_mul = 1; p.groups = 1; p.out_scale = 1.0f; p.K = K; p.ldw = K;
    attach_planes(c.m, p);
    return gemm_takes_planes(p, c.m.opts);
}

struct Pending {
    const float* parts = nullptr; long long pstride = 0; int S = 0; const float* bias = nullptr;
    const float* stat = nullptr; int stat_nt = 0, stat_w = 0;
};
struct LnOps {
    const float *g, *b, *W, *bias;
    const float *Wl, *s, *c;
};
static LnOps ln_ops(const float* g, const float* b, const float* W, const float* bias, const float* Wl, const float* s,
                    const float* c, int n0, int K) {
    return LnOps{g, b, W + (size_t)n0 * K, bias + n0, Wl ? Wl + (size_t)n0 * K : nullptr, s ? s + n0 : nullptr,
                 c ? c + n0 : nullptr};
}
static void ln_linear(const Ctx& c, const float* x, int ldx, int Rx, int a_mul, int shift0, int M, const LnOps& w, int N,
                      int K, float* y, int ldy, float* h_scratch, int epi_act = ACT_NONE, const Pending* st = nullptr,
                      bool c_planes = false) {
    GemmP p{};
    p.c_planes = c_planes ? 1 : 0;
    p.X = x; p.ldx = ldx; p.Rx = Rx; p.a_mul = a_mul ? a_mul : 1; p.shift0 = shift0; p.taps = 1; p.dil = 1; p.Cin = K;
    p.K = K; p.W = w.W; p.ldw = K; p.bias = w.bias; p.C = y; p.ldc = ldy; p.M = M; p.N = N; p.groups = 1; p.out_scale = 1.0f;
    p.epi_act = epi_act; p.ln_eps = 1e-5f;
    if (c.m.opts.skinny_tm && M <= c.m.opts.skinny_rows && c.m.opts.force_cfg < 0) {
        GemmP q = p;
        q.pro_act = 3; q.ln_g = w.g; q.ln_b = w.b;
        if (st && st->stat && st->stat_w == 16 && c.m.opts.skinny_pairs) {
            q.ln_stat = st->stat; q.ln_nt = st->stat_nt; q.ln_w = 16;
        }
        attach_tm(c.m, q);
        if (q.Wtm && gemm_skinny_tm_eligible(q, c.m.opts.skinny_rows)) {
            const hipError_t e = launch_gemm(q, c.s, &c.m.opts);
            if (e == hipSuccess) return;
            if (e != hipErrorNotSupported) MT2_HIP(e);
        }
    }
    if (st && st->stat && st->stat_nt > 0 && st->stat_w != 16 && st->stat_nt <= 32 && (st->stat_nt & 1) == 0 && c.m.opts.ln_pairs && w.Wl &&
        c.m.opts.force_cfg < 0 && M <= c.m.opts.ln_pairs_maxm) {
        GemmP q = p;
        q.pro_act = 5; q.W = w.Wl; q.bias = w.c; q.ln_g = w.s; q.ln_stat = st->stat; q.ln_nt = st->stat_nt; q.ln_w = st->stat_w;
        attach_planes(c.m, q);
        const hipError_t e = launch_gemm(q, c.s, &c.m.opts);
        if (e == hipSuccess) return;
        if (e != hipErrorNotSupported) MT2_HIP(e);
    }
    const bool planes = linear_takes_planes(c, h_scratch, K, M, w.W, w.bias, N, K, y, ldy, epi_act);
    LnP q{};
    q.x = x + (long long)shift0 * ldx; q.ldx = ldx * p.a_mul; q.gamma = w.g; q.beta = w.b; q.out = h_scratch; q.ldo = K;
    q.M = M; q.C = K; q.eps = 1e-5f; q.act = ACT_NONE; q.out_planes = planes ? 1 : 0; q.x3h_flag = c.m.opts.x3h_flag;
    MT2_HIP(launch_layernorm(q, c.s));
    linear(c, h_scratch, K, M, w.W, w.bias, N, K, y, ldy, nullptr, 0, nullptr, epi_act, planes, c_planes);
}
static LnOps ln1_qkv(const EncLayerW& w, int d, int n0 = 0) {
    return ln_ops(w.ln1g, w.ln1b, w.wqkv, w.bqkv, w.wqkv_l, w.sqkv, w.cqkv, n0, d);
}
static LnOps ln2_ff0(const EncLayerW& w, int d) {
    return ln_ops(w.ln2g, w.ln2b, w.ff0w, w.ff0b, w.ff0_l, w.sff0, w.cff0, 0, d);
}

static void conv_same(const Ctx& c, const float* x, int ldx, int R, const ConvW& w, float* y, int ldy,
                      const int* valid, int pro_act = ACT_NONE, float slope = 0.f, int epi_act = ACT_NONE,
                      const float* Rsd = nullptr, int ldr = 0, int dil = 1) {
    GemmP p{};
    p.X = x; p.ldx = ldx; p.Rx = R; p.taps = w.k; p.dil = dil; p.shift0 = -((w.k - 1) / 2) * dil; p.Cin = w.cin;
    p.W = w.w; p.bias = w.b; p.R = Rsd; p.ldr = ldr; p.valid = valid; p.C = y; p.ldc = ldy; p.M = R; p.N = w.cout;
    p.pro_act = pro_act; p.pro_slope = slope; p.epi_act = epi_act;
    gemm(c, p);
}

static void layernorm(const Ctx& c, const float* x, int ldx, const float* g, const float* b, int M, int C,
                      float* out, int ldo, const int* valid = nullptr, int valid_rows = 0,
                      const float* R1 = nullptr, int ldr1 = 0, int r1_rows = 0, int rows_per_group = 0,
                      int act = ACT_NONE, bool out_planes = false) {
    LnP p{};
    p.x = x; p.ldx = ldx; p.gamma = g; p.beta = b; p.rows_per_group = rows_per_group;
    p.R1 = R1; p.ldr1 = ldr1; p.r1_rows = r1_rows; p.valid = valid; p.valid_rows = valid_rows;
    p.out = out; p.ldo = ldo; p.M = M; p.C = C; p.eps = 1e-5f; p.act = act;
    p.out_planes = out_planes ? 1 : 0; p.x3h_flag = c.m.opts.x3h_flag;
    MT2_HIP(launch_layernorm(p, c.s));
}

static float* run_stack(const Ctx& c, const StackW& w, const float* x_in, bool shared_in, int R,
                        const int* valid) {
    const int C = w.C, G = w.groups;
    const size_t per = (size_t)R * C;
    float* T = c.ws.get<float>(per * G);
    float* Y = c.ws.get<float>(per * G);
    float* XA = c.ws.get<float>(per * G);
    float* XB = c.ws.get<float>(per * G);
    const float* cur = x_in;
    bool cur_shared = shared_in;
    float* nxt = XA;
    const size_t wsz = (size_t)C * w.k * C;
    for (int st = 0; st < w.nstack; ++st) {
        const float* bin = cur;
        bool bin_shared = cur_shared;
        bool bin_relued = false;
        bool bin_planes = false;
        auto block_conv = [&](int blk, const float* in, bool in_shared, bool relued, bool planes) {
            const size_t e = w.idx(st, blk);
            GemmP p{};
            p.X = in; p.strideX = in_shared ? 0 : (long long)per; p.ldx = C; p.Rx = R;
            p.taps = w.k; p.shift0 = -((w.k - 1) / 2); p.Cin = C;
            p.W = w.w + e * wsz; p.strideW = (long long)wsz;
            p.bias = w.b + e * C; p.strideB = C;
            p.valid = valid; p.C = T; p.strideC = (long long)per; p.ldc = C; p.M = R; p.N = C; p.groups = G;
            p.pro_act = relued ? ACT_NONE : ACT_RELU;
            p.a_planes = planes ? 1 : 0;
            return p;
        };
        for (int blk = 0; blk < w.nblock; ++blk) {
            const size_t e = w.idx(st, blk);
            gemm(c, block_conv(blk, bin, bin_shared, bin_relued, bin_planes));
            const bool last = blk == w.nblock - 1;
            bool planes = false;
            if (!last && (c.m.opts.a_planes & 1)) {
                GemmP q = block_conv(blk + 1, Y, false, true, false);
                q.dil = 1; q.a_mul = 1; q.out_scale = 1.0f; q.K = q.taps * q.Cin; q.ldw = q.K;
                attach_planes(c.m, q);
                planes = gemm_takes_planes(q, c.m.opts);
            }
            if (last)
                layernorm(c, T, C, w.g + e * C, w.be + e * C, R * G, C, nxt, C, valid, R, cur, C,
                          cur_shared ? R : 0, R);
            else
                layernorm(c, T, C, w.g + e * C, w.be + e * C, R * G, C, Y, C, valid, R, nullptr, 0, 0, R, ACT_RELU, planes);
            bin = Y;
            bin_shared = false;
            bin_relued = !last;
            bin_planes = planes;
        }
        cur = nxt;
        cur_shared = false;
        nxt = (nxt == XA) ? XB : XA;
    }
    return const_cast<float*>(cur);
}

struct AttnGeom {
    const int* start = nullptr; const int* len = nullptr;
    int u_stride = 0, u_len = 0, B = 0, max_len = 0;
};
struct EncScratch { float *h, *qkv, *att, *f, *parts, *stat; };
static EncScratch enc_scratch(const Ctx& c, const EncW& e, int M) {
    EncScratch s;
    s.h = c.ws.get<float>((size_t)M * e.d);
    s.qkv = c.ws.get<float>((size_t)M * 3 * e.d);
    s.att = c.ws.get<float>((size_t)M * e.d);
    s.f = c.ws.get<float>((size_t)M * e.ff);
    s.parts = c.ws.get<float>(std::max((size_t)256 * 32 * 64 + (size_t)16 * 32 * e.d, (size_t)8 * M * e.d));
    s.stat = c.ws.get<float>((size_t)M * 128);
    return s;
}
static AttnP attn_params(const Ctx& c, int H, int D) {
    AttnP a{};
    a.H = H; a.D = D; a.scale = 1.0f / std::sqrt((float)D);
    a.lds_min_qlen = c.m.opts.attn_lds_min; a.x6_min_qlen = c.m.opts.attn_x6_min;
    a.x3h = (c.m.opts.x3h & 8) ? 1 : 0; a.x3h_flag = c.m.opts.x3h_flag;
    return a;
}
static AttnP attn_params(const Ctx& c, const EncW& e) { return attn_params(c, e.heads, e.d / e.heads); }
static void attention_self(const Ctx& c, const EncW& e, const AttnGeom& g, const float* qkv, float* att, bool o_planes = false) {
    AttnP a = attn_params(c, e);
    a.o_planes = o_planes ? 1 : 0;
    const int d = e.d;
    a.Q = qkv; a.ldq = 3 * d; a.K = qkv + d; a.ldk = 3 * d; a.V = qkv + 2 * d; a.ldv = 3 * d;
    a.O = att; a.ldo = d;
    a.q_start = g.start; a.q_len = g.len; a.kv_start = g.start; a.kv_len = g.len;
    a.u_qstride = g.u_stride; a.u_qlen = g.u_len; a.u_kvstride = g.u_stride; a.u_kvlen = g.u_len;
    a.B = g.B; a.max_qlen = g.max_len; a.max_kvlen = g.max_len;
    MT2_HIP(launch_attention(a, c.s));
}
static void encoder_layer(const Ctx& c, const EncW& e, const EncLayerW& w, float* x, int M, const AttnGeom& g,
                          const int* valid, const EncScratch& s) {
    const int d = e.d;
    layernorm(c, x, d, w.ln1g, w.ln1b, M, d, s.h, d, valid);
    linear(c, s.h, d, M, w.wqkv, w.bqkv, 3 * d, d, s.qkv, 3 * d);
    attention_self(c, e, g, s.qkv, s.att);
    linear(c, s.att, d, M, w.wo, w.bo, d, d, x, d, x, d, valid);
    if (e.conv_ff) {
        layernorm(c, x, d, w.ln2g, w.ln2b, M, d, s.h, d, valid);
        ConvW c1{w.ff0w, w.ff0b, e.ff, d, 5}, c2{w.ff1w, w.ff1b, d, e.ff, 5};
        conv_same(c, s.h, d, M, c1, s.f, e.ff, valid, ACT_NONE, 0.f, ACT_RELU);
        conv_same(c, s.f, e.ff, M, c2, x, d, valid, ACT_NONE, 0.f, ACT_NONE, s.h, d);
    } else {
        layernorm(c, x, d, w.ln2g, w.ln2b, M, d, s.h, d, valid);
        linear(c, s.h, d, M, w.ff0w, w.ff0b, e.ff, d, s.f, e.ff, nullptr, 0, nullptr, ACT_RELU);
        linear(c, s.f, e.ff, M, w.ff1w, w.ff1b, d, e.ff, x, d, x, d, valid);
    }
}

static int choose_split(const Ctx& c, int M, int N, int K) {
    if (!c.m.opts.splitk) return 1;
    if (c.m.opts.skinny_tm && c.m.opts.skinny_rows > 0 && M <= c.m.opts.skinny_rows && M <= 64 && c.m.opts.force_cfg < 0 &&
        (N & 15) == 0 && (K & 63) == 0) {
        if (K <= 1536) return 1;
        int S = 1;
        const int kmin = 1024;
        while (S < 16 && K % (S * 2) == 0 && K / (S * 2) >= kmin && (K / (S * 2)) % 64 == 0) S *= 2;
        return S;
    }
    if (c.m.opts.x6_gemm && (N & 127) == 0 && (K & 31) == 0) {
        const long long t128 = (long long)((M + 127) / 128) * (N / 128);
        if (t128 < c.m.opts.t_x6_128) {
            int S = 1;
            while (S < 8 && t128 * S < 2 * c.m.opts.t_x6_128 && K % (S * 2) == 0 && K / (S * 2) >= 512 && (K / (S * 2)) % 32 == 0)
                S *= 2;
            if (S > 1 && t128 * S >= c.m.opts.t_x6_128) return S;
        }
    }
    const long long tiles = (long long)((M + 31) / 32) * ((N + 63) / 64);
    int S = 1;
    while (S < 16 && tiles * (S * 2) <= 256 && K % (S * 2) == 0 && K / (S * 2) >= 256 && (K / (S * 2)) % 32 == 0) S *= 2;
    return S;
}
static GemmP splitk_params(const float* x, int ldx, int M, const float* W, int N, int K, int S, float* parts) {
    GemmP p{};
    p.X = x; p.strideX = K / S; p.ldx = ldx; p.Rx = M; p.Cin = K / S; p.W = W; p.strideW = K / S; p.ldw = K;
    p.C = parts; p.strideC = (long long)M * N; p.ldc = N; p.M = M; p.N = N; p.groups = S;
    return p;
}
static void linear_splitk(const Ctx& c, const float* x, int ldx, int M, const float* W, int N, int K, int S,
                          float* parts, bool a_planes = false) {
    GemmP p = splitk_params(x, ldx, M, W, N, K, S, parts);
    p.a_planes = a_planes ? 1 : 0;
    gemm(c, p);
}
static void ln_pending(const Ctx& c, float* x, int d, int M, const Pending& in, const float* g, const float* b,
                       float* h, bool h_planes = false) {
    if (in.S == 0) {
        LnP q{};
        q.x = x; q.ldx = d; q.gamma = g; q.beta = b; q.out = h; q.ldo = d; q.M = M; q.C = d; q.eps = 1e-5f; q.act = ACT_NONE;
        q.out_planes = h_planes ? 1 : 0; q.x3h_flag = c.m.opts.x3h_flag;
        MT2_HIP(launch_layernorm(q, c.s));
        return;
    }
    LnReduceP p{};
    p.parts = in.parts; p.pstride = in.pstride; p.S = in.S; p.bias = in.bias; p.R = x; p.ldr = d;
    p.gamma = g; p.beta = b; p.xout = x; p.ldx = d; p.hout = h; p.ldh = d; p.M = M; p.C = d; p.eps = 1e-5f;
    p.h_planes = h_planes ? 1 : 0; p.x3h_flag = c.m.opts.x3h_flag;
    MT2_HIP(launch_ln_reduce(p, c.s));
}
static void ln_pending_linear(const Ctx& c, float* x, int d, int M, const Pending& in, const float* g, const float* b, float* h,
                              const float* W, const float* bias, int N, float* y, int ldy, int epi_act = ACT_NONE,
                              bool c_planes = false) {
    const bool planes = M <= 4096 && linear_takes_planes(c, h, d, M, W, bias, N, d, y, ldy, epi_act);
    ln_pending(c, x, d, M, in, g, b, h, planes);
    linear(c, h, d, M, W, bias, N, d, y, ldy, nullptr, 0, nullptr, epi_act, planes, c_planes);
}
static GemmP residual_params(const Ctx& c, const float* a, int lda, int M, const float* W, const float* b, int N, int K,
                             float* x, float* stat, const float* res, int ldr) {
    GemmP p{};
    p.X = a; p.ldx = lda; p.Rx = M; p.Cin = K; p.W = W; p.bias = b; p.R = res ? res : x; p.ldr = res ? ldr : N; p.C = x; p.ldc = N;
    p.M = M; p.N = N;
    const bool small = M <= 64 && M <= c.m.opts.skinny_rows && c.m.opts.skinny_tm && c.m.opts.skinny_pairs;
    const bool want = stat != nullptr && c.m.opts.force_cfg < 0 &&
                      (small || (c.m.opts.ln_pairs > 0 && M > 64 && M <= c.m.opts.ln_pairs_maxm));
    if (want) p.stat_out = stat;
    return p;
}
static Pending linear_residual(const Ctx& c, const float* a, int lda, int M, const float* W, const float* b, int N, int K,
                               float* x, float* stat, const float* res = nullptr, int ldr = 0, bool a_planes = false) {
    GemmP p = residual_params(c, a, lda, M, W, b, N, K, x, stat, res, ldr);
    const bool want = p.stat_out != nullptr;
    p.a_planes = a_planes ? 1 : 0;
    gemm(c, p);
    Pending r{};
    if (want && c.m.opts.last_stat_nt > 0) { r.stat = stat; r.stat_nt = c.m.opts.last_stat_nt; r.stat_w = c.m.opts.last_stat_w; }
    return r;
}
static void ar_tail_splits(const Ctx& c, const EncW& e, int M, int& S1, int& S2) {
    const int d = e.d;
    const bool unsplit = c.m.opts.ln_pairs >= 2 && M > 64 && M <= c.m.opts.ln_pairs_maxm && c.m.opts.force_cfg < 0;
    S1 = choose_split(c, M, d, d);
    if (unsplit && d <= c.m.opts.ln_pairs_maxk) S1 = 1;
    S2 = choose_split(c, M, d, e.ff);
    if (unsplit && e.ff <= c.m.opts.ln_pairs_maxk) S2 = 1;
}
static bool ar_outproj_takes_planes(const Ctx& c, const EncW& e, const EncLayerW& w, float* x, int M, const float* att,
                                    const EncScratch& s) {
    const int d = e.d;
    if (!(c.m.opts.a_planes & 4) || M <= 64 || M > 4096 || (d & 31) || ((d / e.heads) & 31)) return false;
    int S1, S2;
    ar_tail_splits(c, e, M, S1, S2);
    const GemmP q = S1 > 1 ? splitk_params(att, d, M, w.wo, d, d, S1, s.parts)
                           : residual_params(c, att, d, M, w.wo, w.bo, d, d, x, s.stat, nullptr, 0);
    return gemm_takes_planes(planned(c, q), c.m.opts);
}
static Pending ar_layer_tail(const Ctx& c, const EncW& e, const EncLayerW& w, float* x, int M, const float* att,
                             const EncScratch& s, bool att_planes = false) {
    const int d = e.d;
    int S1, S2;
    ar_tail_splits(c, e, M, S1, S2);
    bool fpl = false;
    if ((c.m.opts.a_planes & 2) && M > 64 && M <= 4096) {
        GemmP q0{};
        q0.X = s.h; q0.ldx = d; q0.Rx = M; q0.Cin = d; q0.W = w.ff0w; q0.bias = w.ff0b; q0.C = s.f; q0.ldc = e.ff; q0.M = M; q0.N = e.ff;
        q0.epi_act = ACT_RELU;
        const GemmP q3 = S2 > 1 ? splitk_params(s.f, e.ff, M, w.ff1w, d, e.ff, S2, s.parts)
                                : residual_params(c, s.f, e.ff, M, w.ff1w, w.ff1b, d, e.ff, x, s.stat, nullptr, 0);
        fpl = gemm_writes_planes(planned(c, q0), c.m.opts) && gemm_takes_planes(planned(c, q3), c.m.opts);
    }
    if (S1 > 1) {
        linear_splitk(c, att, d, M, w.wo, d, d, S1, s.parts, att_planes);
        Pending p1{s.parts, (long long)M * d, S1, w.bo};
        ln_pending_linear(c, x, d, M, p1, w.ln2g, w.ln2b, s.h, w.ff0w, w.ff0b, e.ff, s.f, e.ff, ACT_RELU, fpl);
    } else {
        const Pending p1 = linear_residual(c, att, d, M, w.wo, w.bo, d, d, x, s.stat, nullptr, 0, att_planes);
        ln_linear(c, x, d, M, 1, 0, M, ln2_ff0(w, d), e.ff, d, s.f, e.ff, s.h, ACT_RELU, &p1, fpl);
    }
    if (S2 > 1) {
        linear_splitk(c, s.f, e.ff, M, w.ff1w, d, e.ff, S2, s.parts, fpl);
        return Pending{s.parts, (long long)M * d, S2, w.ff1b};
    }
    return linear_residual(c, s.f, e.ff, M, w.ff1w, w.ff1b, d, e.ff, x, s.stat, nullptr, 0, fpl);
}

static Pending encoder_layer_ar(const Ctx& c, const EncW& e, const EncLayerW& w, float* x, int M, const AttnGeom& g,
                                const EncScratch& s, const Pending& in) {
    MT2_REQUIRE(!e.conv_ff, "AR step layers use the Linear feed-forward");
    const int d = e.d;
    if (in.S) {
        ln_pending_linear(c, x, d, M, in, w.ln1g, w.ln1b, s.h, w.wqkv, w.bqkv, 3 * d, s.qkv, 3 * d);
    } else {
        ln_linear(c, x, d, M, 1, 0, M, ln1_qkv(w, d), 3 * d, d, s.qkv, 3 * d, s.h, ACT_NONE, &in);
    }
    const bool opl = !g.start && ar_outproj_takes_planes(c, e, w, x, M, s.att, s);
    attention_self(c, e, g, s.qkv, s.att, opl);
    return ar_layer_tail(c, e, w, x, M, s.att, s, opl);
}

static void encoder_layer_last(const Ctx& c, const EncW& e, const EncLayerW& w, float* x, int n, int A,
                               const EncScratch& s, float* y, const Pending& in) {
    MT2_REQUIRE(!e.conv_ff, "AR step layers use the Linear feed-forward");
    const int d = e.d, M = A * n;
    float* kv = s.qkv;
    float* q = s.att;
    float* att = s.att + (size_t)A * d;
    AttnP a = attn_params(c, e);
    if (c.m.opts.skinny_tm && M <= c.m.opts.skinny_rows && M <= 64 && c.m.opts.force_cfg < 0) {
        float* qkv = s.qkv;
        if (in.S) {
            ln_pending(c, x, d, M, in, w.ln1g, w.ln1b, s.h);
            linear(c, s.h, d, M, w.wqkv, w.bqkv, 3 * d, d, qkv, 3 * d);
        } else {
            ln_linear(c, x, d, M, 1, 0, M, ln1_qkv(w, d), 3 * d, d, qkv, 3 * d, s.h, ACT_NONE, &in);
        }
        a.Q = qkv + (size_t)(n - 1) * 3 * d; a.ldq = 3 * d; a.u_qstride = n;
        a.K = qkv + d; a.ldk = 3 * d; a.V = qkv + 2 * d; a.ldv = 3 * d;
        a.u_ostride = 1;
    } else if (in.S) {
        ln_pending(c, x, d, M, in, w.ln1g, w.ln1b, s.h);
        linear(c, s.h, d, M, w.wqkv + (size_t)d * d, w.bqkv + d, 2 * d, d, kv, 2 * d);
        GemmP p{};
        p.X = s.h; p.ldx = d; p.Rx = M; p.a_mul = n; p.shift0 = n - 1; p.Cin = d; p.W = w.wqkv; p.bias = w.bqkv;
        p.C = q; p.ldc = d; p.M = A; p.N = d;
        gemm(c, p);
    } else {
        ln_linear(c, x, d, M, 1, 0, M, ln1_qkv(w, d, d), 2 * d, d, kv, 2 * d, s.h, ACT_NONE, &in);
        ln_linear(c, x, d, M, n, n - 1, A, ln1_qkv(w, d), d, d, q, d, s.f, ACT_NONE, &in);
    }
    if (!a.Q) {
        a.Q = q; a.ldq = d; a.K = kv; a.ldk = 2 * d; a.V = kv + d; a.ldv = 2 * d;
        a.u_qstride = 1;
    }
    a.O = att; a.ldo = d;
    a.u_qlen = 1; a.u_kvstride = n; a.u_kvlen = n; a.B = A; a.max_qlen = 1;
    MT2_HIP(launch_attention(a, c.s));
    const Pending py = linear_residual(c, att, d, A, w.wo, w.bo, d, d, y, s.stat, x + (size_t)(n - 1) * d, n * d);
    ln_linear(c, y, d, A, 1, 0, A, ln2_ff0(w, d), e.ff, d, s.f, e.ff, s.h, ACT_RELU, &py);
    linear(c, s.f, e.ff, A, w.ff1w, w.ff1b, d, e.ff, y, d, y, d);
}

static Pending encoder_layer_first_cached(const Ctx& c, const EncW& e, const EncLayerW& w, float* x, int n, int A,
                                          float* qkv_cache, int cs, const EncScratch& s, bool fill_all) {
    MT2_REQUIRE(!e.conv_ff, "AR step layers use the Linear feed-forward");
    const int d = e.d, M = A * n;
    if (fill_all && n > 1) {
        ln_linear(c, x, d, M, 1, 0, M, ln1_qkv(w, d), 3 * d, d, s.qkv, 3 * d, s.h);
        MT2_HIP(launch_copy_2d(s.qkv, (long long)n * 3 * d, qkv_cache, (long long)cs * 3 * d, (long long)n * 3 * d, A,
                               c.s));
    } else {
        ln_linear(c, x, d, M, n, n - 1, A, ln1_qkv(w, d), 3 * d, d, qkv_cache + (size_t)(n - 1) * 3 * d, cs * 3 * d, s.h);
    }
    AttnP a = attn_params(c, e);
    a.Q = qkv_cache; a.ldq = 3 * d; a.K = qkv_cache + d; a.ldk = 3 * d; a.V = qkv_cache + 2 * d; a.ldv = 3 * d;
    a.O = s.att; a.ldo = d;
    a.u_qstride = cs; a.u_qlen = n; a.u_kvstride = cs; a.u_kvlen = n; a.u_ostride = n;
    a.B = A; a.max_qlen = n;
    const bool opl = ar_outproj_takes_planes(c, e, w, x, M, s.att, s);
    a.o_planes = opl ? 1 : 0;
    MT2_HIP(launch_attention(a, c.s));
    return ar_layer_tail(c, e, w, x, M, s.att, s, opl);
}

static const float* ar_step_layers(const Ctx& c, const EncW& e, float* x, int n, int A, float* qkv_cache, int cs,
                                   const EncScratch& sc, float* ylast, bool fill_cache = false) {
    const int L = (int)e.layers.size();
    AttnGeom g;
    g.u_stride = n; g.u_len = n; g.B = A; g.max_len = n;
    Pending pend;
    for (int l = 0; l < L; ++l) {
        if (l == L - 1) encoder_layer_last(c, e, e.layers[l], x, n, A, sc, ylast, pend);
        else if (l == 0 && qkv_cache) pend = encoder_layer_first_cached(c, e, e.layers[l], x, n, A, qkv_cache, cs, sc, fill_cache);
        else pend = encoder_layer_ar(c, e, e.layers[l], x, A * n, g, sc, pend);
    }
    return ylast;
}


struct Stages {
    mt2_model& m;
    hipStream_t s;
    std::vector<hipEvent_t> ev;
    std::vector<std::string> names;
    explicit Stages(mt2_model& mm, hipStream_t ss) : m(mm), s(ss) {}
    int nmark = 0;
    void mark(const char* name) {
        if (m.opts.markers) MT2_HIP(launch_stage_marker(nmark, s));
        ++nmark;
        if (!m.profiling) return;
        hipEvent_t e;
        MT2_HIP(hipEventCreate(&e));
        MT2_HIP(hipEventRecord(e, s));
        ev.push_back(e);
        names.push_back(name);
    }
    void finish() {
        if (!m.profiling || ev.empty()) return;
        MT2_HIP(hipEventSynchronize(ev.back()));
        m.stage_names.clear();
        m.stage_ms.clear();
        for (size_t i = 1; i < ev.size(); ++i) {
            float ms = 0.f;
            MT2_HIP(hipEventElapsedTime(&ms, ev[i - 1], ev[i]));
            m.stage_names.push_back(names[i]);
            m.stage_ms.push_back(ms);
        }
        for (auto e : ev) (void)hipEventDestroy(e);
        ev.clear();
    }
};


static float* mel_context_rows(const Ctx& c, const float* xmel, int ld_mel, RowSet& F, RowSet& X,
                               const int* d_rowbase) {
    mt2_model& m = c.m;
    const int C = m.cfg.mrte_hidden, G = m.mel_s1.groups;
    float* h0 = c.ws.get<float>((size_t)F.R * C);
    {
        GemmP p{};
        p.X = xmel; p.ldx = ld_mel; p.Rx = F.R; p.taps = m.mel_first.k; p.shift0 = -((m.mel_first.k - 1) / 2);
        p.Cin = m.mel_first.cin; p.W = m.mel_first.w; p.bias = m.mel_first.b; p.valid = F.d_valid;
        p.C = h0; p.ldc = C; p.M = F.R; p.N = C;
        gemm(c, p);
    }
    float* s1 = run_stack(c, m.mel_s1, h0, true, F.R, F.d_valid);
    float* mid = c.ws.get<float>((size_t)G * X.R * C);
    {
        GemmP p{};
        p.X = s1; p.strideX = (long long)F.R * C; p.ldx = C; p.Rx = F.R; p.rowbase = d_rowbase;
        p.taps = m.mel_mid.k; p.Cin = C; p.W = m.mel_mid.w; p.strideW = 0; p.bias = m.mel_mid.b; p.strideB = 0;
        p.valid = X.d_valid; p.C = mid; p.strideC = (long long)X.R * C; p.ldc = C; p.M = X.R; p.N = C; p.groups = G;
        gemm(c, p);
    }
    float* s2 = run_stack(c, m.mel_s2, mid, false, X.R, X.d_valid);
    float* sum = c.ws.get<float>((size_t)X.R * C);
    MT2_HIP(launch_sum_groups(s2, (long long)X.R * C, G, C, sum, C, C, X.R, c.s));
    float* ctx = c.ws.get<float>((size_t)X.R * C);
    conv_same(c, sum, C, X.R, m.mel_last, ctx, C, X.d_valid);
    return ctx;
}

struct MelPlan {
    RowSet F, X;
    int o_rowmapF, o_rowbase, o_rowmapX;
    RowPlanOffsets oF, oX;
};
static MelPlan plan_mel(IntPlan& ip, const mt2_config& cfg, const int* mel_lens, int B, int Tp_max, int Tc_max) {
    MelPlan mp;
    const int s = cfg.mrte_stride;
    mp.F = make_rows(mel_lens, B, std::max(s / 2, 2));
    std::vector<int> xl(B);
    for (int b = 0; b < B; ++b) {
        MT2_REQUIRE(mel_lens[b] >= 1 && mel_lens[b] <= Tp_max, "prompt mel length out of range");
        xl[b] = (mel_lens[b] - 1) / s + 1;
    }
    mp.X = make_rows(xl.data(), B, 2);
// ... 1256 lines not shown
```

### megatts2_amd/csrc/mt2_kernels.h

```cpp
#pragma once
#include <hip/hip_runtime.h>
#include <stdint.h>

#include <atomic>
#include <vector>

namespace mt2 {

inline hipError_t dyn_lds_once(std::atomic<unsigned long long>& done, const void* fn, size_t bytes) {
    int dev = 0;
    hipError_t e = hipGetDevice(&dev);
    if (e != hipSuccess) return e;
    const unsigned long long bit = 1ull << (dev & 63);
    if (done.load(std::memory_order_acquire) & bit) return hipSuccess;
    e = hipFuncSetAttribute(fn, hipFuncAttributeMaxDynamicSharedMemorySize, (int)bytes);
    if (e != hipSuccess) return e;
    done.fetch_or(bit, std::memory_order_release);
    return hipSuccess;
}

constexpr int kInvalidRow = -(1 << 30);

enum Act : int { ACT_NONE = 0, ACT_RELU = 1, ACT_LRELU = 2, ACT_TANH = 3,
                 ACT_LOGCLAMP = 4 };

struct GemmP {
    const float* X; long long strideX; int ldx; int Rx;
    const int* rowbase; int a_mul; int shift0; int taps; int dil; int Cin;
    const float* W; long long strideW; int ldw;
    unsigned long long* dbg = nullptr;
    int epi_t4 = 1;
    int sk_nw = 8;
    int a_planes = 0;
    int c_planes = 0;
    int ldr64 = 0;
    int ldr_prio = 0;
    const void* W3 = nullptr;
    long long w3_plane = 0;
    const void* Wh = nullptr;
    long long wh_ldb = 0;
    long long wh_gstride = 0;
    const float* wh_inv = nullptr;
    long long wh_inv_stride = 0;
    int* x3h_flag = nullptr;
    const float* Wtm = nullptr;
    int tm_n0 = 0, tm_k0 = 0;
    int tm_kb = 0;
    const float* bias; long long strideB;
    const float* R; long long strideR; int ldr;
    const int* valid;
    float* C; long long strideC; int ldc;
    int M, N, K, groups;
    int pro_act; float pro_slope; int epi_act; float out_scale;
    const float* ln_g; const float* ln_b; float ln_eps;
    float* stat_out = nullptr; int stat_nt = 0, stat_w = 0;
    const float* ln_stat = nullptr; int ln_nt = 0, ln_w = 0;
};
struct TraceRec { int cfg; double flops; hipEvent_t e0, e1; int M, N, K, groups; };
struct EngineOpts {
    int force_cfg = -1;
    int t_ks4 = 256, t_ks2 = 640, t32 = 64, t32x32 = 160;
    bool splitk = true;
    int voc_streams = 3;
    bool win_conv = true;
    bool x6_conv = true;
    bool x6_gemm = true;
    int x3h = 15;
    int* x3h_flag = nullptr;
    int t_x3h_128 = 72;
    int t_x6_256 = 160, t_x6_128 = 72;
    int x6_ks = 4;
    int a_planes = 3;
    bool ldr64 = false;
    int ldr_prio = 3;
    int skinny_rows = 64;
    int attn_lds_min = 640;
    int attn_x6_min = 192;
    bool skinny_tm = true;
    int skinny_pairs = 1;
    int skinny_nw = 16;
    bool markers = false;
    bool trace_on = false;
    std::vector<TraceRec> trace;
    const char* last_cfg = "";
    int last_stat_nt = 0, last_stat_w = 0;
    int ln_pairs = 0;
    int ln_pairs_adm = 2;
    int ln_pairs_maxk = 1024;
    int ln_pairs_maxm = 1280;
};
struct GemmRoute { hipError_t err; int cfg; int variant; size_t lds; int stat_nt, stat_w; };
GemmRoute gemm_route(const GemmP& p, const EngineOpts& o);
hipError_t launch_gemm(const GemmP& p, hipStream_t s, EngineOpts* o = nullptr);
bool gemm_takes_planes(const GemmP& p, const EngineOpts& o);
bool gemm_writes_planes(const GemmP& p, const EngineOpts& o);
bool gemm_skinny_eligible(const GemmP& p, int max_rows);
hipError_t launch_gemm_skinny(const GemmP& p, hipStream_t s);
bool gemm_skinny_tm_eligible(const GemmP& p, int max_rows);
hipError_t launch_gemm_skinny_tm(const GemmP& p, hipStream_t s);
hipError_t launch_tile_major(const float* W, int N, int K, float* out, hipStream_t s);
int gemm_num_configs();
const char* gemm_config_name(int idx);
int gemm_trace_collect(EngineOpts& o, int cap, const char** names, int64_t* launches, double* flops, double* ms);
int gemm_trace_shapes(EngineOpts& o, char* buf, int cap, int top);

struct LnP {
    const float* x; int ldx;
    const float* gamma; const float* beta; int rows_per_group;
    const float* R1; int ldr1; int r1_rows; const float* R2; int ldr2;
    const int* valid; int valid_rows;
    float* out; int ldo;
    int M, C; float eps; int act;
    int out_planes = 0;
    int* x3h_flag = nullptr;
};
hipError_t launch_layernorm(const LnP& p, hipStream_t s);

struct LnReduceP {
    const float* parts; long long pstride; int S;
    const float* bias; const float* R; int ldr;
    const float* gamma; const float* beta;
    float* xout; int ldx; float* hout; int ldh;
    int M, C; float eps;
    int h_planes = 0;
    int* x3h_flag = nullptr;
};
hipError_t launch_ln_reduce(const LnReduceP& p, hipStream_t s);

struct AttnP {
    const float* Q; int ldq; const float* K; int ldk; const float* V; int ldv;
    float* O; int ldo;
    const int* q_start; const int* q_len; const int* kv_start; const int* kv_len; const int* o_start;
    int u_qstride, u_qlen, u_kvstride, u_kvlen, u_ostride;
    int B, H, D, max_qlen; float scale;
    int max_kvlen;
    int lds_min_qlen = 640;
    int x6_min_qlen = 0;
    int lds_waves = 0;
    int ds_short = 1;
    int x3h = 0;
    int o_planes = 0;
    int* x3h_flag = nullptr;
};
enum AttnKernel {
    ATTN_NONE = 0,
    ATTN_GENERIC = 1,
    ATTN_REG = 2,
    ATTN_DS = 3,
    ATTN_LDS = 4,
    ATTN_X6 = 5,
    ATTN_X3H = 6,
};
struct AttnRoute {
    hipError_t err; int kernel;
    int d;
    int nwq;
    int nkv;
    int nwv;
    unsigned gx, gy, gz, block;
    size_t lds;
};
AttnRoute attn_route(const AttnP& p);
hipError_t launch_attention(const AttnP& p, hipStream_t s);

hipError_t launch_embed_pe(const float* table, int C, const int64_t* ids, const int* idmap, const int* pos,
                           const float* pe, float* out, int ldo, int R, int vocab, hipStream_t s);
hipError_t launch_gather_rows(const float* src, int lds_, const int* map, float* out, int ldo, int C, int R,
                              hipStream_t s);
hipError_t launch_pool_max(const float* src, int lds_, const int* first, const int* cnt, float* out, int ldo,
                           int C, int R, hipStream_t s);
hipError_t launch_sum_groups(const float* x, long long strideG, int groups, int ld, float* out, int ldo, int C,
                             int R, hipStream_t s);
hipError_t launch_avg3(const float* a, const float* b, const float* d, float scale, float* out, long long n,
                       hipStream_t s);
// ... 138 lines not shown
```

### megatts2_amd/csrc/mt2_model.h

```cpp
#pragma once
#include "../../include/megatts2_hip.h"
#include "mt2_kernels.h"

#include <map>
#include <mutex>
#include <stdexcept>
#include <string>
#include <vector>

namespace mt2 {

struct Error : std::runtime_error {
    using std::runtime_error::runtime_error;
};
void check_hip(hipError_t e, const char* what, const char* file, int line);
#define MT2_HIP(x) ::mt2::check_hip((x), #x, __FILE__, __LINE__)
#define MT2_REQUIRE(cond, msg)                                                                   \
    do {                                                                                         \
        if (!(cond)) throw ::mt2::Error(std::string(msg) + " [" #cond "] at " __FILE__ ":" +     \
                                        std::to_string(__LINE__));                               \
    } while (0)

class Arena {
  public:
// ... 35 lines not shown
    const int* d_valid = nullptr;
    const int* d_start = nullptr;
    const int* d_len = nullptr;
};

class IntPlan {
  public:
    int add(const std::vector<int>& v);
    int add_fill(size_t n, int value);
    std::vector<int>& host() { return h_; }
    void upload(Arena& a, PinnedPool& pin, hipStream_t s);
    const int* dev(int offset) const { return d_ + offset; }

  private:
    std::vector<int> h_;
    int* d_ = nullptr;
};

struct ConvW { float* w = nullptr; float* b = nullptr; int cout = 0, cin = 0, k = 0; };
struct PlaneRange { const float* base; size_t n; const uint16_t* p3; const uint16_t* ph = nullptr; const float* inv = nullptr; size_t row_len = 0; };
struct TmRange { const float* base; size_t n; int K; const float* tm; };
struct StackW {
    float *w = nullptr, *b = nullptr, *g = nullptr, *be = nullptr;
    int C = 0, k = 0, nstack = 0, nblock = 0, groups = 0;
    size_t idx(int s, int blk) const { return (size_t)(s * nblock + blk) * groups; }
};
struct EncLayerW {
    float *ln1g, *ln1b, *ln2g, *ln2b, *wqkv, *bqkv, *wo, *bo, *ff0w, *ff0b, *ff1w, *ff1b;
    float *wqkv_l = nullptr, *sqkv = nullptr, *cqkv = nullptr, *ff0_l = nullptr, *sff0 = nullptr, *cff0 = nullptr;
};
struct EncW {
    std::vector<EncLayerW> layers;
    int d = 0, ff = 0, heads = 0;
    bool conv_ff = false;
};
struct UpW { float *wlo, *whi, *bias; int cin, cout, stride; };
struct ResW { ConvW c1[3], c2[3]; int k; int dil[3]; };

struct StageTimer {
    std::vector<std::string> names;
    std::vector<hipEvent_t> ev;
};

}

struct mt2_model {
    mt2_config cfg{};
    bool finalized = false;
    bool has_g = false, has_adm = false, has_plm = false;
    std::map<std::string, mt2::HostTensor> host;
    std::vector<void*> dev_allocs;
    std::vector<mt2::PlaneRange> planes;
    std::vector<mt2::TmRange> tm;
    size_t weight_bytes = 0;
    mt2::Arena ws;

    float *phone_emb = nullptr, *pe_mrte = nullptr;
    mt2::ConvW mel_first, mel_mid, mel_last;
    mt2::StackW mel_s1, mel_s2;
    mt2::EncW phone_enc;
    float *x_wq, *x_bq, *x_wkv, *x_bkv, *x_wo, *x_bo, *x_ng, *x_nb;
    mt2::ConvW vq_first, vq_last;
    mt2::StackW vq_s1, vq_s2;
    float *codebook = nullptr, *codebook_sq = nullptr;
    mt2::ConvW dec_first, dec_last;
    mt2::StackW dec_stack;
    mt2::EncW adm_enc;
    float *adm_wdt, *adm_wtc, *adm_wpred, *pe_adm;
    mt2::EncW plm_enc;
    float *plm_emb, *plm_wpred, *pe_plm;
    bool has_vocoder = false;
    mt2::ConvW hg_pre, hg_post;
    std::vector<mt2::UpW> hg_up;
    std::vector<mt2::ResW> hg_res;

    std::mutex call_mutex;
    mt2::PinnedPool pin[2];
    int pin_idx = 0;
    hipStream_t last_stream = nullptr;
    hipEvent_t ev_call_end = nullptr;
    bool call_pending = false;
    mt2::PinnedPool& pinned() { return pin[pin_idx]; }

    mt2::EngineOpts opts;

    int ar_groups = 2;
    int adm_groups = 0, plm_groups = 0;
    std::vector<hipStream_t> aux_streams;
    hipEvent_t ev_fork = nullptr;
    std::vector<hipEvent_t> ev_join;
    hipStream_t vq_stream = nullptr;
    hipEvent_t ev_vq_fork = nullptr, ev_vq_join = nullptr, ev_vq_t0 = nullptr, ev_vq_t1 = nullptr;
    bool aux_forked = false, vq_forked = false;
    hipStream_t id_stream = nullptr;
    hipEvent_t ev_id_fork = nullptr, ev_id_done = nullptr;
    int* id_flag_dev = nullptr;
    int* id_flag_host = nullptr;
    bool id_open = false;
    int* x3h_flag_dev = nullptr;
    int* x3h_flag_host = nullptr;

    mt2_audio_config fe_cfg{};
    float *fe_basis = nullptr, *fe_fb = nullptr;
    int fe_nfreq = 0, fe_nfreq_pad = 0;
    float *gl_ibasis = nullptr, *gl_w2 = nullptr, *gl_P = nullptr;
    std::map<std::pair<int, int>, float*> rs_tables;

    bool profiling = false;
    std::vector<std::string> stage_names;
    std::vector<float> stage_ms;
};
```

### megatts2_amd/csrc/planes_store.h

```cpp
#pragma once
#include <hip/hip_runtime.h>

namespace mt2 {

typedef _Float16 pl_f16x2 __attribute__((ext_vector_type(2)));
typedef float pl_f32x2 __attribute__((ext_vector_type(2)));
__device__ __forceinline__ float store_planes4(float* __restrict__ row, int c, float y0, float y1, float y2, float y3) {
    const pl_f16x2 h01 = __builtin_convertvector((pl_f32x2){y0, y1}, pl_f16x2), h23 = __builtin_convertvector((pl_f32x2){y2, y3}, pl_f16x2);
    const float s = 2048.0f;
    const pl_f16x2 l01 = __builtin_convertvector((pl_f32x2){__builtin_fmaf((float)h01[0], -s, y0 * s), __builtin_fmaf((float)h01[1], -s, y1 * s)}, pl_f16x2);
    const pl_f16x2 l23 = __builtin_convertvector((pl_f32x2){__builtin_fmaf((float)h23[0], -s, y2 * s), __builtin_fmaf((float)h23[1], -s, y3 * s)}, pl_f16x2);
    char* blk = reinterpret_cast<char*>(row) + (c >> 5) * 128 + (c & 31) * 2;
    *reinterpret_cast<uint2*>(blk) = make_uint2(__builtin_bit_cast(unsigned, h01), __builtin_bit_cast(unsigned, h23));
    *reinterpret_cast<uint2*>(blk + 64) = make_uint2(__builtin_bit_cast(unsigned, l01), __builtin_bit_cast(unsigned, l23));
    return fmaxf(fmaxf(fabsf(y0), fabsf(y1)), fmaxf(fabsf(y2), fabsf(y3)));
}
__device__ __forceinline__ float store_planes4(float* __restrict__ row, int c, const float4& y) {
    return store_planes4(row, c, y.x, y.y, y.z, y.w);
}

}
```

### megatts2_amd/runtime.py

```python
from __future__ import annotations

import ctypes as C
import math
import os
from typing import Dict, Optional, Sequence

import numpy as np

from . import config as cfgmod
from . import sampling as sampmod

_LIB = None
MAX_POSITIONS = 8192

MT2_RUN_PLM, MT2_RUN_VOCODER, MT2_SKIP_ADM, MT2_PROMPT_VQPE = 1, 2, 4, 8
ACT_NONE, ACT_RELU, ACT_LRELU, ACT_TANH = 0, 1, 2, 3
ACT_LOGCLAMP = 4
MT2_RESAMPLE_NORMALIZE = 1
TRIM_FRAME, TRIM_HOP = 2048, 512
F0_FRAME, F0_WINDOW, F0_MAX_LAG = 1024, 768, 256
DTW_MAX_LEN, DTW_DIR_COLS = 4096, 16


class NativeError(RuntimeError):
# ... 886 lines not shown
    nz = mx > 0
    e[nz] = np.clip(15 - np.frexp(mx[nz])[1], -100, 100)
    s = np.ldexp(np.float32(1), e).astype(np.float32)
    v = (w * s[:, None]).astype(np.float32)
    hi = v.astype(np.float16)
    lo = ((v - hi.astype(np.float32)) * np.float32(2048)).astype(np.float16)
    Kp = -(-K // 32) * 32
    planes = np.zeros((N, Kp // 32, 2, 32), np.int16)
    pad = np.zeros((N, Kp), np.int16)
    pad[:, :K] = hi.view(np.int16)
    planes[:, :, 0, :] = pad.reshape(N, Kp // 32, 32)
    pad[:, :K] = lo.view(np.int16)
    planes[:, :, 1, :] = pad.reshape(N, Kp // 32, 32)
    return torch.from_numpy(planes), torch.from_numpy(np.ldexp(np.float32(1), -e).astype(np.float32))


def x3h_split_native(W):
    import torch
    lib = load_library()
    w = W.detach().to(torch.float32).cpu().contiguous()
    kp = -(-w.shape[1] // 32) * 32
    planes = torch.empty(w.shape[0], kp // 32, 2, 32, dtype=torch.int16)
    inv = torch.empty(w.shape[0], dtype=torch.float32)
    _check(lib.mt2_x3h_split(C.c_void_p(w.data_ptr()), C.c_longlong(w.shape[0]), C.c_longlong(w.shape[1]),
                             C.c_void_p(planes.data_ptr()), C.c_void_p(inv.data_ptr())))
    return planes, inv


def op_conv_x3h(X, W, bias=None, R=None, valid=None, shift0=0, taps=1, dil=1, Cin=None, pro_act=ACT_NONE, pro_slope=0.0,
                epi_act=ACT_NONE, force_cfg=-1, want_flag=False):
    import torch
    lib = load_library()
    Cin = Cin or X.shape[1]
    N, M = W.shape[0], X.shape[0]
    W3 = split_bf16x3(W).to(X.device)
    ph, inv = split_f16x2_rows(W)
    ph, inv = ph.to(X.device), inv.to(X.device)
    out = torch.empty(M, N, device=X.device, dtype=torch.float32)
    flag = torch.zeros(4, device=X.device, dtype=torch.int32)
    _check(lib.mt2_op_gemm_x3h(_stream(), _ptr(X), X.shape[1], M, shift0, taps, dil, Cin, _ptr(W), _ptr(W3), _ptr(ph), _ptr(inv),
                               _ptr(bias), _ptr(R), R.shape[1] if R is not None else 0, _ptr(valid), _ptr(out), N, M, N, pro_act,
                               C.c_float(pro_slope), epi_act, force_cfg, _ptr(flag)))
    return (out, int(flag[0].item())) if want_flag else out


def op_gemm_x6_ln(X, W, bias=None, R=None, M=None, a_mul=1, shift0=0, epi_act=ACT_NONE, force_cfg=-1, want_stats=False,
                  ln=None, eps=1e-5, x3h=False):
    import torch
    lib = load_library()
    K, N = X.shape[1], W.shape[0]
    M = M or X.shape[0]
    dev = X.device
    out = torch.empty(M, N, device=dev, dtype=torch.float32)
    stat = torch.zeros(M, 32, 2, device=dev, dtype=torch.float32) if want_stats else None
    nt, pw = C.c_int32(0), C.c_int32(0)
    ln_stat, ln_nt, ln_w, ln_s = None, 0, 0, None
    if ln is not None:
        gamma, beta, pairs, ln_w = ln
        Wd = W.double().cpu()
        Wl = (W.cpu() * gamma.cpu()[None, :]).to(torch.float32)
        ln_s = Wl.double().sum(1).to(torch.float32).to(dev)
        bias = (Wd @ beta.double().cpu() + (bias.double().cpu() if bias is not None else 0.0)).to(torch.float32).to(dev)
        W = Wl.to(dev)
        ln_stat = pairs.contiguous()
        ln_nt = pairs.shape[1]
    W = W.contiguous()
    W3 = split_bf16x3(W).to(dev)
    if x3h:
        ph, inv = split_f16x2_rows(W)
        ph, inv = ph.to(dev), inv.to(dev)
        _check(lib.mt2_op_gemm_x3h_ln(_stream(), _ptr(X), K, X.shape[0], a_mul, shift0, _ptr(W), _ptr(W3), _ptr(ph), _ptr(inv),
                                      _ptr(bias), _ptr(R), R.shape[1] if R is not None else 0, _ptr(out), N, M, N, K, epi_act,
                                      force_cfg, _ptr(stat), C.byref(nt), C.byref(pw), _ptr(ln_stat), ln_nt, int(ln_w), _ptr(ln_s),
                                      C.c_float(eps)))
    else:
        _check(lib.mt2_op_gemm_x6_ln(_stream(), _ptr(X), K, X.shape[0], a_mul, shift0, _ptr(W), _ptr(W3), _ptr(bias), _ptr(R),
                                     R.shape[1] if R is not None else 0, _ptr(out), N, M, N, K, epi_act, force_cfg, _ptr(stat),
                                     C.byref(nt), C.byref(pw), _ptr(ln_stat), ln_nt, int(ln_w), _ptr(ln_s), C.c_float(eps)))
    if want_stats:
        return out, stat.view(-1)[:M * nt.value * 2].reshape(M, nt.value, 2).clone(), pw.value
    return out


def op_sample_rows(logits, sampling, seeds, positions):
    import torch
    lib = load_library()
    A, N = logits.shape
    assert logits.is_cuda and logits.dtype == torch.float32 and logits.stride(1) == 1
    seeds = seeds.contiguous().to(torch.int64)
    positions = positions.contiguous().to(torch.int32)
    assert seeds.shape == (A,) and positions.shape == (A,)
    out = torch.empty(A, device=logits.device, dtype=torch.int64)
    s = sampmod.as_sampling(sampling).to_c(np.zeros(1, np.uint64))
    s.seeds = C.cast(C.c_void_p(0), C.POINTER(C.c_uint64))
    _check(lib.mt2_op_sample_rows(_stream(), _ptr(logits), logits.stride(0), N, A, C.byref(s), _ptr(seeds), _ptr(positions),
                                  _ptr(out)))
    return out


def op_sample_mix_rows(logits, sampling, seeds, positions, gamma):
    import torch
    lib = load_library()
    A, N = logits.shape[0] // 2, logits.shape[1]
    assert logits.is_cuda and logits.dtype == torch.float32 and logits.stride(1) == 1 and logits.shape[0] == 2 * A
    gamma = gamma.contiguous().to(torch.float32)
    assert gamma.shape == (A,)
    s = None
    if sampling is not None:
        seeds = seeds.contiguous().to(torch.int64)
        positions = positions.contiguous().to(torch.int32)
        assert seeds.shape == (A,) and positions.shape == (A,)
        s = sampmod.as_sampling(sampling).to_c(np.zeros(1, np.uint64))
        s.seeds = C.cast(C.c_void_p(0), C.POINTER(C.c_uint64))
    else:
        seeds = positions = None
    out = torch.empty(2 * A, device=logits.device, dtype=torch.int64)
    _check(lib.mt2_op_sample_mix_rows(_stream(), _ptr(logits), logits.stride(0), N, A, C.byref(s) if s is not None else None,
                                      _ptr(seeds), _ptr(positions), _ptr(gamma), _ptr(out)))
    return out


def op_layernorm(x, gamma, beta, R1=None, valid=None, eps=1e-5, act=ACT_NONE):
    import torch
    lib = load_library()
    M, Cc = x.shape
    out = torch.empty_like(x)
    _check(lib.mt2_op_layernorm(_stream(), _ptr(x), Cc, _ptr(gamma), _ptr(beta), _ptr(R1), Cc, _ptr(valid), _ptr(out),
                                Cc, M, Cc, C.c_float(eps), act))
    return out



def op_layernorm_ex(x, ldx, gamma, beta, rows_per_group, R1, ldr1, r1_rows, R2, ldr2, valid, valid_rows, out, ldo, M, Cc, eps=1e-5,
                    act=ACT_NONE, out_planes=0, x3h_flag=None):
    _check(load_library().mt2_op_layernorm_ex(_stream(), _ptr(x), ldx, _ptr(gamma), _ptr(beta), rows_per_group, _ptr(R1), ldr1,
                                              r1_rows, _ptr(R2), ldr2, _ptr(valid), valid_rows, _ptr(out), ldo, M, Cc,
                                              C.c_float(eps), act, out_planes, _ptr(x3h_flag)))


def op_ln_reduce(parts, pstride, S, bias, R, ldr, gamma, beta, xout, ldx, hout, ldh, M, Cc, eps=1e-5, h_planes=0, x3h_flag=None):
    _check(load_library().mt2_op_ln_reduce(_stream(), _ptr(parts), C.c_longlong(pstride), S, _ptr(bias), _ptr(R), ldr, _ptr(gamma),
                                           _ptr(beta), _ptr(xout), ldx, _ptr(hout), ldh, M, Cc, C.c_float(eps), h_planes,
                                           _ptr(x3h_flag)))


def op_row(op, *args, stream=None):
    ptrs, ints, flts = [], [], []
    for a in args:
        if isinstance(a, float):
            flts.append(a)
        elif isinstance(a, (int, np.integer)) and not isinstance(a, bool):
            ints.append(int(a))
        else:
            ptrs.append(a.data_ptr() if a is not None else 0)
    _check(load_library().mt2_op_row(stream if stream is not None else _stream(), op.encode(), (C.c_void_p * len(ptrs))(*ptrs), len(ptrs),
                                     (C.c_longlong * len(ints))(*ints), len(ints), (C.c_float * len(flts))(*flts), len(flts)))


def op_embed_pe(table, Cc, ids, idmap, pos, pe, out, ldo, R, vocab): op_row("embed_pe", table, Cc, ids, idmap, pos, pe, out, ldo, R, vocab)
def op_gather_rows(src, lds_, map_, out, ldo, Cc, R): op_row("gather_rows", src, lds_, map_, out, ldo, Cc, R)
def op_pool_max(src, lds_, first, cnt, out, ldo, Cc, R): op_row("pool_max", src, lds_, first, cnt, out, ldo, Cc, R)
def op_sum_groups(x, strideG, groups, ld, out, ldo, Cc, R): op_row("sum_groups", x, strideG, groups, ld, out, ldo, Cc, R)
def op_avg3(a, b, d, scale, out, n): op_row("avg3", a, b, d, float(scale), out, n)
def op_conv_post(x0, x1, x2, scale, R, ch, k, w, bias, slope, valid, out): op_row("conv_post", x0, x1, x2, float(scale), R, ch, k, w, bias, float(slope), valid, out)
def op_fill_reflect(x, ld, Cc, start, len_, B, scale, G): op_row("fill_reflect", x, ld, Cc, start, len_, B, scale, G)
def op_pack_rows(src, Cc, Tmax, cmajor, rowmap, dst, ldd, R): op_row("pack_rows", src, Cc, Tmax, cmajor, rowmap, dst, ldd, R)
# ... 250 lines not shown
```

Measured before the change: 78320 mel-frames/s.

## Hand over f16 plane-split activations between fused LayerNorm GEMM stages

Adds a LayerNorm-prologue variant that reads pre-split f16 A planes (V_LNXAPL). GEMM epilogues that emit row statistics can now also write a plane-split copy of their output, and the pair-row epilogue can store planes directly. The encoder AR layers pass this copy to the next LN-fused GEMM, so the consumer does not have to re-split f32 activations. It costs extra epilogue stores and shuffles, more kernel variants, and overflow-flag checks, and it is enabled through the model's default engine options.

After: 78550 mel-frames/s, median of 2. No clear change (+0.3%).

```diff
diff --git a/include/megatts2_hip.h b/include/megatts2_hip.h
--- a/include/megatts2_hip.h
+++ b/include/megatts2_hip.h
@@ -280,6 +280,11 @@
                        const void* Wh, const float* wh_inv, const float* bias, const float* R, int ldr, float* C, int ldc, int M, int N,
                        int K, int epi_act, int force_cfg, float* stat_out, int32_t* stat_nt, int32_t* stat_w, const float* ln_stat,
                        int ln_nt, int ln_w, const float* ln_s, float ln_eps);
+int mt2_op_gemm_x3h_handover(void* stream, const float* X, int ldx, int Rx, int a_mul, int shift0, const float* W, const void* W3,
+                             const void* Wh, const float* wh_inv, const float* bias, const float* R, int ldr, float* C, int ldc, int M,
+                             int N, int K, int epi_act, int force_cfg, float* stat_out, int32_t* stat_nt, int32_t* stat_w,
+                             const float* ln_stat, int ln_nt, int ln_w, const float* ln_s, float ln_eps, int planes, float* c_copy,
+                             int32_t* copied, int32_t* range_flag);
 int mt2_bench_gemm(void* stream, int M, int N, int K, int taps, int dil, int flags, int force_cfg, int iters,
                    int w_copies, float* avg_ms, char* cfg_name, int cfg_name_cap, double* sustained_ghz);
 
diff --git a/megatts2_amd/csrc/capi.inc b/megatts2_amd/csrc/capi.inc
--- a/megatts2_amd/csrc/capi.inc
+++ b/megatts2_amd/csrc/capi.inc
@@ -1227,7 +1227,8 @@
 static int op_gemm_ln_impl(void* stream, const float* X, int ldx, int Rx, int a_mul, int shift0, const float* W, const void* W3,
                            const void* Wh, const float* wh_inv, const float* bias, const float* R, int ldr, float* C, int ldc, int M,
                            int N, int K, int epi_act, int force_cfg, float* stat_out, int32_t* stat_nt, int32_t* stat_w,
-                           const float* ln_stat, int ln_nt, int ln_w, const float* ln_s, float ln_eps);
+                           const float* ln_stat, int ln_nt, int ln_w, const float* ln_s, float ln_eps, int planes = 0,
+                           float* c_copy = nullptr, int32_t* copied = nullptr, int32_t* range_flag = nullptr);
 int mt2_op_gemm_x6_ln(void* stream, const float* X, int ldx, int Rx, int a_mul, int shift0, const float* W, const void* W3,
                       const float* bias, const float* R, int ldr, float* C, int ldc, int M, int N, int K, int epi_act,
                       int force_cfg, float* stat_out, int32_t* stat_nt, int32_t* stat_w, const float* ln_stat, int ln_nt,
@@ -1242,10 +1243,19 @@
     return op_gemm_ln_impl(stream, X, ldx, Rx, a_mul, shift0, W, W3, Wh, wh_inv, bias, R, ldr, C, ldc, M, N, K, epi_act, force_cfg,
                            stat_out, stat_nt, stat_w, ln_stat, ln_nt, ln_w, ln_s, ln_eps);
 }
+int mt2_op_gemm_x3h_handover(void* stream, const float* X, int ldx, int Rx, int a_mul, int shift0, const float* W, const void* W3,
+                             const void* Wh, const float* wh_inv, const float* bias, const float* R, int ldr, float* C, int ldc, int M,
+                             int N, int K, int epi_act, int force_cfg, float* stat_out, int32_t* stat_nt, int32_t* stat_w,
+                             const float* ln_stat, int ln_nt, int ln_w, const float* ln_s, float ln_eps, int planes, float* c_copy,
+                             int32_t* copied, int32_t* range_flag) {
+    return op_gemm_ln_impl(stream, X, ldx, Rx, a_mul, shift0, W, W3, Wh, wh_inv, bias, R, ldr, C, ldc, M, N, K, epi_act, force_cfg,
+                           stat_out, stat_nt, stat_w, ln_stat, ln_nt, ln_w, ln_s, ln_eps, planes | 0x100, c_copy, copied, range_flag);
+}
 static int op_gemm_ln_impl(void* stream, const float* X, int ldx, int Rx, int a_mul, int shift0, const float* W, const void* W3,
                            const void* Wh, const float* wh_inv, const float* bias, const float* R, int ldr, float* C, int ldc, int M,
                            int N, int K, int epi_act, int force_cfg, float* stat_out, int32_t* stat_nt, int32_t* stat_w,
-                           const float* ln_stat, int ln_nt, int ln_w, const float* ln_s, float ln_eps) {
+                           const float* ln_stat, int ln_nt, int ln_w, const float* ln_s, float ln_eps, int planes, float* c_copy,
+                           int32_t* copied, int32_t* range_flag) {
     MT2_API_BEGIN
     GemmP p{};
     p.Wh = Wh; p.wh_inv = wh_inv;
@@ -1253,14 +1263,18 @@
     p.W3 = W3; p.ldw = K; p.bias = bias; p.R = R; p.ldr = ldr; p.C = C; p.ldc = ldc; p.M = M; p.N = N; p.K = K; p.groups = 1;
     p.epi_act = epi_act; p.out_scale = 1.0f; p.stat_out = stat_out;
     if (ln_stat) { p.pro_act = 5; p.ln_stat = ln_stat; p.ln_nt = ln_nt; p.ln_w = ln_w; p.ln_g = ln_s; p.ln_eps = ln_eps; }
+    p.a_planes = (planes & 1) ? 1 : 0; p.c_planes = (planes & 2) ? 1 : 0; p.Cpl = c_copy;
     EngineOpts o;
+    if (planes & 0x100) o.a_planes |= kModelPlanesBits;
     o.ldr64 = force_cfg >= 1000;
     o.force_cfg = force_cfg >= 1000 ? force_cfg - 1000 : force_cfg;
+    o.x3h_flag = range_flag;
     const hipError_t e = launch_gemm(p, (hipStream_t)stream, &o);
     MT2_REQUIRE(e != hipErrorNotSupported, "this tile configuration has no pair-fed LayerNorm form");
     MT2_HIP(e);
     if (stat_nt) *stat_nt = o.last_stat_nt;
     if (stat_w) *stat_w = o.last_stat_w;
+    if (copied) *copied = o.last_cpl;
     MT2_API_END
 }
 
diff --git a/megatts2_amd/csrc/gemm_common.h b/megatts2_amd/csrc/gemm_common.h
--- a/megatts2_amd/csrc/gemm_common.h
+++ b/megatts2_amd/csrc/gemm_common.h
@@ -149,10 +149,15 @@
         q.v[i] = vp[m * vs];
     }
 }
-template <int NE, bool STAT = false>
+template <int NE, bool STAT = false, bool PLN = false>
 __device__ __forceinline__ void epilogue_pre(const GemmP& p, const float (&acc)[NE], const EpiPre<NE>& q, int g, int mw,
                                              int nw, int lane, int e0) {
     float* __restrict__ C = p.C + (long long)g * p.strideC;
+    float* __restrict__ P = nullptr;
+    if constexpr (PLN) P = p.c_planes ? C : (p.Cpl ? p.Cpl + (long long)g * p.strideC : nullptr);
+    const bool f32_out = !(PLN && p.c_planes);
+    float pv[PLN ? NE : 1];
+    static_assert(!PLN || (NE & 1) == 0, "planes: rows in pairs");
     const int epi_act = p.epi_act;
     const float epi_par = p.pro_slope;
     const float out_scale = p.out_scale;
@@ -170,9 +175,23 @@
             v = act_rt(epi_act, v, epi_par) * out_scale;
             if (hasR) v += q.r[i];
             if (q.v[i] == 0) v = 0.0f;
-            C[(long long)m * p.ldc + n] = v;
-        }
+            if (f32_out) C[(long long)m * p.ldc + n] = v;
+        }
+        if constexpr (PLN) pv[i] = v;
         if constexpr (STAT) { sv[i] = v; qv[i] = v * v; }
+    }
+    if constexpr (PLN) {
+        if (P) {
+            float amax = 0.0f;
+#pragma unroll
+            for (int i = 0; i < NE; i += 2) {
+                const int ea = e0 + i, eb = ea + 1;
+                const int ma = mw + (ea & 3) + 8 * (ea >> 2) + 4 * (lane >> 5), mb = mw + (eb & 3) + 8 * (eb >> 2) + 4 * (lane >> 5);
+                amax = fmaxf(amax, store_planes_pair(P + (long long)ma * p.ldc, P + (long long)mb * p.ldc, n, pv[i], pv[i + 1], nok && ma < p.M,
+                                                     nok && mb < p.M, lane));
+            }
+            if (p.x3h_flag != nullptr && __builtin_amdgcn_ballot_w64(amax >= 65504.0f) != 0ull && lane == 0) atomicOr(p.x3h_flag, 1);
+        }
     }
     if constexpr (STAT) emit_row_pairs<NE>(p, sv, qv, mw, nw >> 5, 32.0f, lane, e0);
 }
@@ -253,7 +272,7 @@
     return ((p.N | p.ldc | (p.R ? p.ldr : 0)) & 3) == 0 && (((unsigned long long)p.C | (unsigned long long)p.R | (unsigned long long)p.bias) & 15) == 0 &&
            ((p.strideC | p.strideR | p.strideB) & 3) == 0;
 }
-template <int TM, int TN, bool STAT = false, bool PLN = false>
+template <int TM, int TN, bool STAT = false, bool PLN = false, bool CPL = false>
 __device__ __forceinline__ void epilogue_t4(const GemmP& p, f32x16 (&acc)[TM][TN], int g, int mw, int nw, int lane) {
     static_assert(!STAT || TM == 1, "row statistics: one 32-row block per wave");
     float* __restrict__ C = p.C + (long long)g * p.strideC;
@@ -319,6 +338,10 @@
                         if (store_planes4(C + (long long)m * p.ldc, n, v[0], v[1], v[2], v[3]) >= 65504.0f && p.x3h_flag) atomicOr(p.x3h_flag, 1);
                     } else
                     *reinterpret_cast<f32x4*>(C + (long long)m * p.ldc + n) = v;
+                    if (CPL && p.Cpl) {
+                        if (store_planes4(p.Cpl + (long long)g * p.strideC + (long long)m * p.ldc, n, v[0], v[1], v[2], v[3]) >= 65504.0f && p.x3h_flag)
+                            atomicOr(p.x3h_flag, 1);
+                    }
                 }
                 if constexpr (STAT) {
                     if (!in) v = f32x4{0.f, 0.f, 0.f, 0.f};
@@ -349,6 +372,7 @@
 }
 
 constexpr int PRO_APL = 3;
+constexpr int PRO_LNXAPL = 6;
 
 __device__ __forceinline__ f32x4 lds_read_b128(unsigned byte_addr) {
     f32x4 v;
diff --git a/megatts2_amd/csrc/gemm_dispatch.hip b/megatts2_amd/csrc/gemm_dispatch.hip
--- a/megatts2_amd/csrc/gemm_dispatch.hip
+++ b/megatts2_amd/csrc/gemm_dispatch.hip
@@ -221,12 +221,16 @@
 }
 
 
-static bool a_planes_ok(const GemmP& p, const TileCfg& c, bool stat) {
-    return c.pipe == PIPE_X3H && !c.win_qs && p.pro_act == ACT_NONE && !stat && (p.Cin % BK) == 0 && (p.ldx % BK) == 0 &&
+static GemmVariant planes_variant(const GemmP& p, bool stat) { return (p.pro_act == PRO_LNX || stat) ? V_LNXAPL : V_APLANES; }
+static bool a_planes_ok(const GemmP& p, const TileCfg& c, bool stat, const EngineOpts& o) {
+    if (planes_variant(p, stat) == V_LNXAPL && !(o.a_planes & 8)) return false;
+    return c.pipe == PIPE_X3H && !c.win_qs && (p.pro_act == ACT_NONE || p.pro_act == PRO_LNX) && c.fn[planes_variant(p, stat)] != nullptr &&
+           (p.Cin % BK) == 0 && (p.ldx % BK) == 0 &&
            !(p.groups > 1 && (p.strideX % BK) != 0) && p.a_mul == 1 && !p.rowbase && !(((unsigned long long)p.X) & 127);
 }
-static bool c_planes_ok(const GemmP& p, const TileCfg& c, bool stat) {
-    return c.pipe == PIPE_X3H && !c.x6_ks && !c.win_qs && p.groups == 1 && !p.R && !stat && (p.N & 31) == 0 && (p.ldc & 31) == 0 &&
+static bool c_planes_ok(const GemmP& p, const TileCfg& c, bool stat, const EngineOpts& o) {
+    if (c.x6_ks && !(o.a_planes & 16)) return false;
+    return c.pipe == PIPE_X3H && !c.win_qs && p.groups == 1 && !p.R && !stat && (p.N & 31) == 0 && (p.ldc & 31) == 0 &&
            (((unsigned long long)p.C) & 127) == 0 && (((unsigned long long)p.bias) & 15) == 0 && ((p.strideC | p.strideB) & 3) == 0 && p.Wh && p.wh_inv && p.M > 64;
 }
 static long long wh_ldb_of(const GemmP& p) { return p.wh_ldb ? p.wh_ldb : 4ll * ((p.ldw + 31) / 32 * 32); }
@@ -280,12 +284,13 @@
                nt <= 32 && (nt & 1) == 0 && ((((unsigned long long)p.stat_out) & 15) == 0);
         if (stat) { r.stat_w = c->stat_w; r.stat_nt = nt; }
     }
-    if (p.a_planes && !a_planes_ok(p, *c, stat)) return fail(hipErrorNotSupported);
-    if (p.c_planes && !c_planes_ok(p, *c, stat)) return fail(hipErrorNotSupported);
+    if (p.a_planes && !a_planes_ok(p, *c, stat, o)) return fail(hipErrorNotSupported);
+    if (p.c_planes && !c_planes_ok(p, *c, stat, o)) return fail(hipErrorNotSupported);
+    r.cpl = p.Cpl && x3h && !c->win_qs && stat && !p.c_planes && (p.N & 31) == 0 && (p.ldc & 31) == 0 && (((unsigned long long)p.Cpl) & 127) == 0;
     if (p.pro_act == PRO_LN || p.pro_act == PRO_LNA) return fail(hipErrorNotSupported);
-    r.variant = p.a_planes ? V_APLANES : ((p.pro_act == PRO_LNX || stat) ? V_LNX : (GemmVariant)p.pro_act);
+    r.variant = p.a_planes ? planes_variant(p, stat) : ((p.pro_act == PRO_LNX || stat) ? V_LNX : (GemmVariant)p.pro_act);
     r.lds = c->lds;
-    if (r.variant == V_LNX && !c->x6_ks) r.lds += (size_t)c->bm * 2 * sizeof(float);
+    if ((r.variant == V_LNX || r.variant == V_LNXAPL) && !c->x6_ks) r.lds += (size_t)c->bm * 2 * sizeof(float);
     if (x3h) {
         if (!p.Wh || !p.wh_inv || (p.K & 7) || (p.ldw & 7)) return fail(hipErrorInvalidValue);
         if ((((unsigned long long)p.Wh) & 127) || (wh_ldb_of(p) & 127) || (wh_gstride_of(p) & 127)) return fail(hipErrorInvalidValue);
@@ -312,12 +317,14 @@
     const GemmP p = normalise(p_in);
     if (!(o.x3h & 3) || o.force_cfg >= 0 || p.M <= 64 || !p.Wh || !p.wh_inv) return false;
     const TileCfg* c = cfg_table().row[choose_cfg(p, o)];
-    return a_planes_ok(p, *c, p.stat_out != nullptr) && c->fn[V_APLANES] != nullptr;
+    return a_planes_ok(p, *c, p.stat_out != nullptr, o);
 }
 bool gemm_writes_planes(const GemmP& p_in, const EngineOpts& o) {
     const GemmP p = normalise(p_in);
-    if (!(o.x3h & 1) || o.force_cfg >= 0 || p.M <= 64) return false;
-    return c_planes_ok(p, *cfg_table().row[choose_cfg(p, o)], p.stat_out != nullptr);
+    if (o.force_cfg >= 0 || p.M <= 64) return false;
+    const TileCfg* c = cfg_table().row[choose_cfg(p, o)];
+    if (!(o.x3h & (c->x6_ks ? 2 : 1))) return false;
+    return c_planes_ok(p, *c, p.stat_out != nullptr, o);
 }
 
 static std::atomic<unsigned long long> g_attr_done[kNumCfgs][kGemmVariants];
@@ -327,10 +334,11 @@
     const EngineOpts& o = opts ? *opts : kDefaults;
     const GemmRoute r = gemm_route(p_in, o);
     if (r.cfg < 0 && r.err == hipSuccess) return hipSuccess;
-    if (opts) { opts->last_stat_nt = r.stat_nt; opts->last_stat_w = r.stat_w; }
+    if (opts) { opts->last_stat_nt = r.stat_nt; opts->last_stat_w = r.stat_w; opts->last_cpl = r.cpl; }
     if (r.err != hipSuccess) return r.err;
     GemmP p = p_in;
     if (!r.stat_nt) p.stat_out = nullptr;
+    if (!r.cpl) p.Cpl = nullptr;
     p.stat_nt = r.stat_nt; p.stat_w = r.stat_w;
     if (r.cfg == CFG_SKINNYTM32 || r.cfg == CFG_SKINNYTM64) {
         p.sk_nw = o.skinny_nw;
diff --git a/megatts2_amd/csrc/gemm_tiles.h b/megatts2_amd/csrc/gemm_tiles.h
--- a/megatts2_amd/csrc/gemm_tiles.h
+++ b/megatts2_amd/csrc/gemm_tiles.h
@@ -12,6 +12,7 @@
     V_NONE, V_RELU, V_LRELU,
     V_APLANES,
     V_LNX,
+    V_LNXAPL,
     kGemmVariants
 };
 static_assert((int)V_NONE == ACT_NONE && (int)V_RELU == ACT_RELU && (int)V_LRELU == ACT_LRELU, "the activation variants are indexed by Act");
diff --git a/megatts2_amd/csrc/gemm_x3h.hip b/megatts2_amd/csrc/gemm_x3h.hip
--- a/megatts2_amd/csrc/gemm_x3h.hip
+++ b/megatts2_amd/csrc/gemm_x3h.hip
@@ -236,7 +236,8 @@
             inv_s[j] = inv[n < p.N ? n : 0];
         }
     }
-    constexpr bool LNXOK = TM == 1 && TM * TN <= 2 && PRO == PRO_LNX;
+    constexpr bool APL = PRO == PRO_APL || PRO == PRO_LNXAPL;
+    constexpr bool LNXOK = TM == 1 && TM * TN <= 2 && (PRO == PRO_LNX || PRO == PRO_LNXAPL);
     const bool lnx = LNXOK && p.pro_act == PRO_LNX;
     [[maybe_unused]] float* lnstat = reinterpret_cast<float*>(ring + NST * STAGE);
     if constexpr (LNXOK) {
@@ -284,7 +285,7 @@
         tcyc0 = __builtin_readcyclecounter();
         if (lane == 0) p.dbg[9] = treal0 - t_entry;
     }
-    if constexpr (PRO == PRO_APL) {
+    if constexpr (APL) {
         constexpr int N1 = 2 * TM + 2 * TN;
         static_assert(N1 <= 15, "lgkmcnt is four bits wide");
         u32x4 ra[2][TM][2];
@@ -518,7 +519,7 @@
                 }
             }
         }
-        if (p.stat_out) epilogue_t4<TM, TN, true>(p, acc, g, m0 + wm * WTM, n0 + wn * WTN, lane);
+        if (p.stat_out) epilogue_t4<TM, TN, true, false, true>(p, acc, g, m0 + wm * WTM, n0 + wn * WTN, lane);
         else epilogue_t4<TM, TN, false, true>(p, acc, g, m0 + wm * WTM, n0 + wn * WTN, lane);
     } else if (p.epi_t4 && epilogue_t4_ok(p)) epilogue_t4<TM, TN, false, true>(p, acc, g, m0 + wm * WTM, n0 + wn * WTN, lane);
     else epilogue<TM, TN>(p, acc, g, m0 + wm * WTM, n0 + wn * WTN, lane);
@@ -651,8 +652,10 @@
         const int n = n0 + wn * 32 + (lane & 31);
         inv_s = (p.wh_inv + (long long)g * p.wh_inv_stride)[n < p.N ? n : 0];
     }
+    constexpr bool APL = PRO == PRO_APL || PRO == PRO_LNXAPL;
+    constexpr bool LNX = PRO == PRO_LNX || PRO == PRO_LNXAPL;
     float ln_mu = 0.0f, ln_rs = 0.0f;
-    const bool lnx = PRO == PRO_LNX && p.pro_act == PRO_LNX;
+    const bool lnx = LNX && p.pro_act == PRO_LNX;
     if (lnx) lnx_row_stats<2>(p, m0 + wm * 32 + (lane & 31), lane >> 5, 32, ln_mu, ln_rs);
     f32x16 acc, acl;
 #pragma unroll
@@ -677,8 +680,8 @@
     f32x4 ra[2][2];
     u32x4 rb[2][2], pln[2];
     auto fetch = [&](int b, unsigned sa, unsigned sb) {
-        ra[b][0] = lds_read_b128(sa + (PRO == PRO_APL ? (unsigned)(((b * 2 + half) ^ swza) * 16) : koffa[b][0]));
-        ra[b][1] = lds_read_b128(sa + (PRO == PRO_APL ? (unsigned)(((4 + b * 2 + half) ^ swza) * 16) : koffa[b][1]));
+        ra[b][0] = lds_read_b128(sa + (APL ? (unsigned)(((b * 2 + half) ^ swza) * 16) : koffa[b][0]));
+        ra[b][1] = lds_read_b128(sa + (APL ? (unsigned)(((4 + b * 2 + half) ^ swza) * 16) : koffa[b][1]));
         rb[b][0] = __builtin_bit_cast(u32x4, lds_read_b128(sb + koffb[b][0]));
         rb[b][1] = __builtin_bit_cast(u32x4, lds_read_b128(sb + koffb[b][1]));
     };
@@ -710,11 +713,11 @@
         wait_block(0);
         wait_block(1);
         __builtin_amdgcn_sched_barrier(0);
-        if constexpr (PRO == PRO_APL) { pln[0] = __builtin_bit_cast(u32x4, ra[0][0]); pln[1] = __builtin_bit_cast(u32x4, ra[0][1]); }
+        if constexpr (APL) { pln[0] = __builtin_bit_cast(u32x4, ra[0][0]); pln[1] = __builtin_bit_cast(u32x4, ra[0][1]); }
         else split2_f16<PRO>(ra[0][0], ra[0][1], pro_slope, pln[0], pln[1], amax);
         products(0);
         __builtin_amdgcn_sched_barrier(0);
-        if constexpr (PRO == PRO_APL) { pln[0] = __builtin_bit_cast(u32x4, ra[1][0]); pln[1] = __builtin_bit_cast(u32x4, ra[1][1]); }
+        if constexpr (APL) { pln[0] = __builtin_bit_cast(u32x4, ra[1][0]); pln[1] = __builtin_bit_cast(u32x4, ra[1][1]); }
         else split2_f16<PRO>(ra[1][0], ra[1][1], pro_slope, pln[0], pln[1], amax);
         products(1);
         __builtin_amdgcn_sched_barrier(0);
@@ -756,8 +759,8 @@
                 out[i] = __shfl(ln_rs, rr) * (out[i] - __shfl(ln_mu, rr) * s_n);
             }
         }
-        if (PRO == PRO_LNX && p.stat_out) epilogue_pre<EPG, PRO == PRO_LNX>(p, out, pre, g, m0 + wm * 32, n0 + wn * 32, lane, kg * EPG);
-        else epilogue_pre<EPG>(p, out, pre, g, m0 + wm * 32, n0 + wn * 32, lane, kg * EPG);
+        if (LNX && p.stat_out) epilogue_pre<EPG, LNX, true>(p, out, pre, g, m0 + wm * 32, n0 + wn * 32, lane, kg * EPG);
+        else epilogue_pre<EPG, false, true>(p, out, pre, g, m0 + wm * 32, n0 + wn * 32, lane, kg * EPG);
     } else {
         float out[16];
 #pragma unroll
@@ -771,8 +774,8 @@
                 out[e] = __shfl(ln_rs, rr) * (out[e] - __shfl(ln_mu, rr) * s_n);
             }
         }
-        if (PRO == PRO_LNX && p.stat_out) epilogue_pre<16, PRO == PRO_LNX>(p, out, pre, g, m0 + wm * 32, n0 + wn * 32, lane, 0);
-        else epilogue_pre<16>(p, out, pre, g, m0 + wm * 32, n0 + wn * 32, lane, 0);
+        if (LNX && p.stat_out) epilogue_pre<16, LNX, true>(p, out, pre, g, m0 + wm * 32, n0 + wn * 32, lane, 0);
+        else epilogue_pre<16, false, true>(p, out, pre, g, m0 + wm * 32, n0 + wn * 32, lane, 0);
     }
     if (probe) {
         __builtin_amdgcn_s_waitcnt(0);
@@ -1051,13 +1054,15 @@
       "x3hldr" #BM_ "x" #BN_ "_" #WM_ "x" #WN_ "+" #NL_ "_s" #NST_ "xc",                                                    \
       { gemm_x3h_ldr_kernel<BM_, BN_, WM_, WN_, NL_, NST_, ACT_NONE>, gemm_x3h_ldr_kernel<BM_, BN_, WM_, WN_, NL_, NST_, ACT_RELU>, \
         gemm_x3h_ldr_kernel<BM_, BN_, WM_, WN_, NL_, NST_, ACT_LRELU>, gemm_x3h_ldr_kernel<BM_, BN_, WM_, WN_, NL_, NST_, PRO_APL>, \
-        gemm_x3h_ldr_kernel<BM_, BN_, WM_, WN_, NL_, NST_, PRO_LNX> }, PIPE_X3H, 0, 0, (BN_) / (WN_) }
+        gemm_x3h_ldr_kernel<BM_, BN_, WM_, WN_, NL_, NST_, PRO_LNX>, gemm_x3h_ldr_kernel<BM_, BN_, WM_, WN_, NL_, NST_, PRO_LNXAPL> },   \
+      PIPE_X3H, 0, 0, (BN_) / (WN_) }
 #define MT2_X3H_KS(IDX_, BM_, BN_, WM_, WN_, KS_, NL_, NST_)                                                                \
     { IDX_, BM_, BN_, (WM_* WN_ * KS_ + NL_) * 64, (size_t)KS_ * NST_ * ((size_t)BM_ * BK * 4 + (size_t)(2 * BN_ / 16) * 1024), \
       "x3hks" #BM_ "x" #BN_ "_" #WM_ "x" #WN_ "_k" #KS_ "+" #NL_ "_s" #NST_,                                                \
       { gemm_x3h_ks_kernel<BM_, BN_, WM_, WN_, KS_, NL_, NST_, ACT_NONE>, gemm_x3h_ks_kernel<BM_, BN_, WM_, WN_, KS_, NL_, NST_, ACT_RELU>, \
         gemm_x3h_ks_kernel<BM_, BN_, WM_, WN_, KS_, NL_, NST_, ACT_LRELU>, gemm_x3h_ks_kernel<BM_, BN_, WM_, WN_, KS_, NL_, NST_, PRO_APL>, \
-        gemm_x3h_ks_kernel<BM_, BN_, WM_, WN_, KS_, NL_, NST_, PRO_LNX> }, PIPE_X3H, 0, KS_, 32 }
+        gemm_x3h_ks_kernel<BM_, BN_, WM_, WN_, KS_, NL_, NST_, PRO_LNX>, gemm_x3h_ks_kernel<BM_, BN_, WM_, WN_, KS_, NL_, NST_, PRO_LNXAPL> }, \
+      PIPE_X3H, 0, KS_, 32 }
 #define MT2_X3H_WIN(IDX_, QS_, BM_, BN_, WM_, WN_, NST_, NL_)                                                               \
     { IDX_, BM_, BN_, (WM_* WN_ + NL_) * 64, (size_t)NST_ * (((2 * BN_ / 16 + NL_ - 1) / NL_) * NL_ * 1024),                  \
       "x3hwin" #BM_ "x" #BN_ "_" #WM_ "x" #WN_ "+" #NL_ "_s" #NST_,                                                          \
diff --git a/megatts2_amd/csrc/model_stages.hip b/megatts2_amd/csrc/model_stages.hip
--- a/megatts2_amd/csrc/model_stages.hip
+++ b/megatts2_amd/csrc/model_stages.hip
@@ -133,6 +133,7 @@
 struct Pending {
     const float* parts = nullptr; long long pstride = 0; int S = 0; const float* bias = nullptr;
     const float* stat = nullptr; int stat_nt = 0, stat_w = 0;
+    const float* xpl = nullptr;
 };
 struct LnOps {
     const float *g, *b, *W, *bias;
@@ -169,6 +170,11 @@
         GemmP q = p;
         q.pro_act = 5; q.W = w.Wl; q.bias = w.c; q.ln_g = w.s; q.ln_stat = st->stat; q.ln_nt = st->stat_nt; q.ln_w = st->stat_w;
         attach_planes(c.m, q);
+        if (st->xpl && p.a_mul == 1 && shift0 == 0 && Rx == M) {
+            GemmP qp = q;
+            qp.X = st->xpl; qp.a_planes = 1;
+            if (gemm_takes_planes(qp, c.m.opts)) q = qp;
+        }
         const hipError_t e = launch_gemm(q, c.s, &c.m.opts);
         if (e == hipSuccess) return;
         if (e != hipErrorNotSupported) MT2_HIP(e);
@@ -270,7 +276,7 @@
     const int* start = nullptr; const int* len = nullptr;
     int u_stride = 0, u_len = 0, B = 0, max_len = 0;
 };
-struct EncScratch { float *h, *qkv, *att, *f, *parts, *stat; };
+struct EncScratch { float *h, *qkv, *att, *f, *parts, *stat, *xpl; };
 static EncScratch enc_scratch(const Ctx& c, const EncW& e, int M) {
     EncScratch s;
     s.h = c.ws.get<float>((size_t)M * e.d);
@@ -279,6 +285,7 @@
     s.f = c.ws.get<float>((size_t)M * e.ff);
     s.parts = c.ws.get<float>(std::max((size_t)256 * 32 * 64 + (size_t)16 * 32 * e.d, (size_t)8 * M * e.d));
     s.stat = c.ws.get<float>((size_t)M * 128);
+    s.xpl = c.ws.get<float>((size_t)M * e.d);
     return s;
 }
 static AttnP attn_params(const Ctx& c, int H, int D) {
@@ -389,14 +396,24 @@
     return p;
 }
 static Pending linear_residual(const Ctx& c, const float* a, int lda, int M, const float* W, const float* b, int N, int K,
-                               float* x, float* stat, const float* res = nullptr, int ldr = 0, bool a_planes = false) {
+                               float* x, float* stat, const float* res = nullptr, int ldr = 0, bool a_planes = false, float* xpl = nullptr) {
     GemmP p = residual_params(c, a, lda, M, W, b, N, K, x, stat, res, ldr);
     const bool want = p.stat_out != nullptr;
     p.a_planes = a_planes ? 1 : 0;
+    if (want) p.Cpl = xpl;
     gemm(c, p);
     Pending r{};
-    if (want && c.m.opts.last_stat_nt > 0) { r.stat = stat; r.stat_nt = c.m.opts.last_stat_nt; r.stat_w = c.m.opts.last_stat_w; }
+    if (want && c.m.opts.last_stat_nt > 0) {
+        r.stat = stat; r.stat_nt = c.m.opts.last_stat_nt; r.stat_w = c.m.opts.last_stat_w;
+        if (p.Cpl && c.m.opts.last_cpl) r.xpl = xpl;
+    }
     return r;
+}
+static bool ln_pairs_takes_planes(const Ctx& c, const float* xpl, int M, const LnOps& w, int N, int K) {
+    if (!(c.m.opts.a_planes & 8) || !c.m.opts.ln_pairs || !w.Wl || c.m.opts.force_cfg >= 0 || M <= 64 || M > c.m.opts.ln_pairs_maxm) return false;
+    GemmP q{};
+    q.X = xpl; q.ldx = K; q.Rx = M; q.Cin = K; q.W = w.Wl; q.bias = w.c; q.M = M; q.N = N; q.pro_act = 5;
+    return gemm_takes_planes(planned(c, q), c.m.opts);
 }
 static void ar_tail_splits(const Ctx& c, const EncW& e, int M, int& S1, int& S2) {
     const int d = e.d;
@@ -417,7 +434,7 @@
     return gemm_takes_planes(planned(c, q), c.m.opts);
 }
 static Pending ar_layer_tail(const Ctx& c, const EncW& e, const EncLayerW& w, float* x, int M, const float* att,
-                             const EncScratch& s, bool att_planes = false) {
+                             const EncScratch& s, bool att_planes = false, const EncLayerW* next = nullptr) {
     const int d = e.d;
     int S1, S2;
     ar_tail_splits(c, e, M, S1, S2);
@@ -435,18 +452,20 @@
         Pending p1{s.parts, (long long)M * d, S1, w.bo};
         ln_pending_linear(c, x, d, M, p1, w.ln2g, w.ln2b, s.h, w.ff0w, w.ff0b, e.ff, s.f, e.ff, ACT_RELU, fpl);
     } else {
-        const Pending p1 = linear_residual(c, att, d, M, w.wo, w.bo, d, d, x, s.stat, nullptr, 0, att_planes);
+        float* xpl1 = ln_pairs_takes_planes(c, s.xpl, M, ln2_ff0(w, d), e.ff, d) ? s.xpl : nullptr;
+        const Pending p1 = linear_residual(c, att, d, M, w.wo, w.bo, d, d, x, s.stat, nullptr, 0, att_planes, xpl1);
         ln_linear(c, x, d, M, 1, 0, M, ln2_ff0(w, d), e.ff, d, s.f, e.ff, s.h, ACT_RELU, &p1, fpl);
     }
     if (S2 > 1) {
         linear_splitk(c, s.f, e.ff, M, w.ff1w, d, e.ff, S2, s.parts, fpl);
         return Pending{s.parts, (long long)M * d, S2, w.ff1b};
     }
-    return linear_residual(c, s.f, e.ff, M, w.ff1w, w.ff1b, d, e.ff, x, s.stat, nullptr, 0, fpl);
+    float* xpl2 = next && ln_pairs_takes_planes(c, s.xpl, M, ln1_qkv(*next, d), 3 * d, d) ? s.xpl : nullptr;
+    return linear_residual(c, s.f, e.ff, M, w.ff1w, w.ff1b, d, e.ff, x, s.stat, nullptr, 0, fpl, xpl2);
 }
 
 static Pending encoder_layer_ar(const Ctx& c, const EncW& e, const EncLayerW& w, float* x, int M, const AttnGeom& g,
-                                const EncScratch& s, const Pending& in) {
+                                const EncScratch& s, const Pending& in, const EncLayerW* next = nullptr) {
     MT2_REQUIRE(!e.conv_ff, "AR step layers use the Linear feed-forward");
     const int d = e.d;
     if (in.S) {
@@ -456,7 +475,7 @@
     }
     const bool opl = !g.start && ar_outproj_takes_planes(c, e, w, x, M, s.att, s);
     attention_self(c, e, g, s.qkv, s.att, opl);
-    return ar_layer_tail(c, e, w, x, M, s.att, s, opl);
+    return ar_layer_tail(c, e, w, x, M, s.att, s, opl, next);
 }
 
 static void encoder_layer_last(const Ctx& c, const EncW& e, const EncLayerW& w, float* x, int n, int A,
@@ -502,7 +521,7 @@
 }
 
 static Pending encoder_layer_first_cached(const Ctx& c, const EncW& e, const EncLayerW& w, float* x, int n, int A,
-                                          float* qkv_cache, int cs, const EncScratch& s, bool fill_all) {
+                                          float* qkv_cache, int cs, const EncScratch& s, bool fill_all, const EncLayerW* next = nullptr) {
     MT2_REQUIRE(!e.conv_ff, "AR step layers use the Linear feed-forward");
     const int d = e.d, M = A * n;
     if (fill_all && n > 1) {
@@ -520,7 +539,7 @@
     const bool opl = ar_outproj_takes_planes(c, e, w, x, M, s.att, s);
     a.o_planes = opl ? 1 : 0;
     MT2_HIP(launch_attention(a, c.s));
-    return ar_layer_tail(c, e, w, x, M, s.att, s, opl);
+    return ar_layer_tail(c, e, w, x, M, s.att, s, opl, next);
 }
 
 static const float* ar_step_layers(const Ctx& c, const EncW& e, float* x, int n, int A, float* qkv_cache, int cs,
@@ -530,9 +549,10 @@
     g.u_stride = n; g.u_len = n; g.B = A; g.max_len = n;
     Pending pend;
     for (int l = 0; l < L; ++l) {
+        const EncLayerW* next = l + 1 < L - 1 ? &e.layers[l + 1] : nullptr;
         if (l == L - 1) encoder_layer_last(c, e, e.layers[l], x, n, A, sc, ylast, pend);
-        else if (l == 0 && qkv_cache) pend = encoder_layer_first_cached(c, e, e.layers[l], x, n, A, qkv_cache, cs, sc, fill_cache);
-        else pend = encoder_layer_ar(c, e, e.layers[l], x, A * n, g, sc, pend);
+        else if (l == 0 && qkv_cache) pend = encoder_layer_first_cached(c, e, e.layers[l], x, n, A, qkv_cache, cs, sc, fill_cache, next);
+        else pend = encoder_layer_ar(c, e, e.layers[l], x, A * n, g, sc, pend, next);
     }
     return ylast;
 }
diff --git a/megatts2_amd/csrc/mt2_kernels.h b/megatts2_amd/csrc/mt2_kernels.h
--- a/megatts2_amd/csrc/mt2_kernels.h
+++ b/megatts2_amd/csrc/mt2_kernels.h
@@ -33,6 +33,7 @@
     int sk_nw = 8;
     int a_planes = 0;
     int c_planes = 0;
+    float* Cpl = nullptr;
     int ldr64 = 0;
     int ldr_prio = 0;
     const void* W3 = nullptr;
@@ -84,12 +85,19 @@
     std::vector<TraceRec> trace;
     const char* last_cfg = "";
     int last_stat_nt = 0, last_stat_w = 0;
+    int last_cpl = 0;
     int ln_pairs = 0;
     int ln_pairs_adm = 2;
     int ln_pairs_maxk = 1024;
     int ln_pairs_maxm = 1280;
 };
-struct GemmRoute { hipError_t err; int cfg; int variant; size_t lds; int stat_nt, stat_w; };
+constexpr int kModelPlanesBits = 8 | 16;
+inline EngineOpts model_engine_opts() {
+    EngineOpts o;
+    o.a_planes |= kModelPlanesBits;
+    return o;
+}
+struct GemmRoute { hipError_t err; int cfg; int variant; size_t lds; int stat_nt, stat_w; int cpl = 0; };
 GemmRoute gemm_route(const GemmP& p, const EngineOpts& o);
 hipError_t launch_gemm(const GemmP& p, hipStream_t s, EngineOpts* o = nullptr);
 bool gemm_takes_planes(const GemmP& p, const EngineOpts& o);
diff --git a/megatts2_amd/csrc/mt2_model.h b/megatts2_amd/csrc/mt2_model.h
--- a/megatts2_amd/csrc/mt2_model.h
+++ b/megatts2_amd/csrc/mt2_model.h
@@ -141,7 +141,7 @@
     bool call_pending = false;
     mt2::PinnedPool& pinned() { return pin[pin_idx]; }
 
-    mt2::EngineOpts opts;
+    mt2::EngineOpts opts = mt2::model_engine_opts();
 
     int ar_groups = 2;
     int adm_groups = 0, plm_groups = 0;
diff --git a/megatts2_amd/csrc/planes_store.h b/megatts2_amd/csrc/planes_store.h
--- a/megatts2_amd/csrc/planes_store.h
+++ b/megatts2_amd/csrc/planes_store.h
@@ -18,5 +18,20 @@
 __device__ __forceinline__ float store_planes4(float* __restrict__ row, int c, const float4& y) {
     return store_planes4(row, c, y.x, y.y, y.z, y.w);
 }
+__device__ __forceinline__ float store_planes_pair(float* __restrict__ row_a, float* __restrict__ row_b, int c, float va, float vb, bool ok_a,
+                                                   bool ok_b, int lane) {
+    const bool odd = lane & 1;
+    const float got = __shfl_xor(odd ? va : vb, 1);
+    const float y0 = odd ? got : va, y1 = odd ? vb : got;
+    if (!(odd ? ok_b : ok_a)) return 0.0f;
+    const pl_f16x2 h = __builtin_convertvector((pl_f32x2){y0, y1}, pl_f16x2);
+    const float s = 2048.0f;
+    const pl_f16x2 l = __builtin_convertvector((pl_f32x2){__builtin_fmaf((float)h[0], -s, y0 * s), __builtin_fmaf((float)h[1], -s, y1 * s)}, pl_f16x2);
+    const int c0 = c & ~1;
+    char* blk = reinterpret_cast<char*>(odd ? row_b : row_a) + (c0 >> 5) * 128 + (c0 & 31) * 2;
+    *reinterpret_cast<unsigned*>(blk) = __builtin_bit_cast(unsigned, h);
+    *reinterpret_cast<unsigned*>(blk + 64) = __builtin_bit_cast(unsigned, l);
+    return fmaxf(fabsf(y0), fabsf(y1));
+}
 
 }
diff --git a/megatts2_amd/runtime.py b/megatts2_amd/runtime.py
--- a/megatts2_amd/runtime.py
+++ b/megatts2_amd/runtime.py
@@ -992,6 +992,43 @@
     return out
 
 
+def op_gemm_x3h_handover(X, W, bias=None, R=None, epi_act=ACT_NONE, force_cfg=-1, want_stats=False, ln=None, eps=1e-5,
+                         a_planes=False, c_planes=False, copy=False, ldc=None, fill=None):
+    import torch
+    lib = load_library()
+    K, N = X.shape[1], W.shape[0]
+    M = X.shape[0]
+    dev = X.device
+    ldc = ldc or N
+    mk = (lambda: torch.full((M, ldc), float(fill), device=dev, dtype=torch.float32)) if fill is not None else \
+         (lambda: torch.empty(M, ldc, device=dev, dtype=torch.float32))
+    out = mk()
+    cpy = mk() if copy else None
+    stat = torch.zeros(M, 32, 2, device=dev, dtype=torch.float32) if want_stats else None
+    flag = torch.zeros(4, device=dev, dtype=torch.int32)
+    nt, pw, copied = C.c_int32(0), C.c_int32(0), C.c_int32(0)
+    ln_stat, ln_nt, ln_w, ln_s = None, 0, 0, None
+    if ln is not None:
+        gamma, beta, pairs, ln_w = ln
+        Wd = W.double().cpu()
+        Wl = (W.cpu() * gamma.cpu()[None, :]).to(torch.float32)
+        ln_s = Wl.double().sum(1).to(torch.float32).to(dev)
+        bias = (Wd @ beta.double().cpu() + (bias.double().cpu() if bias is not None else 0.0)).to(torch.float32).to(dev)
+        W = Wl.to(dev)
+        ln_stat = pairs.contiguous()
+        ln_nt = pairs.shape[1]
+    W = W.contiguous()
+    W3 = split_bf16x3(W).to(dev)
+    ph, inv = split_f16x2_rows(W)
+    ph, inv = ph.to(dev), inv.to(dev)
+    _check(lib.mt2_op_gemm_x3h_handover(_stream(), _ptr(X), K, M, 1, 0, _ptr(W), _ptr(W3), _ptr(ph), _ptr(inv), _ptr(bias), _ptr(R),
+                                        R.shape[1] if R is not None else 0, _ptr(out), ldc, M, N, K, epi_act, force_cfg, _ptr(stat),
+                                        C.byref(nt), C.byref(pw), _ptr(ln_stat), ln_nt, int(ln_w), _ptr(ln_s), C.c_float(eps),
+                                        (1 if a_planes else 0) | (2 if c_planes else 0), _ptr(cpy), C.byref(copied), _ptr(flag)))
+    pairs_out = stat.view(-1)[:M * nt.value * 2].reshape(M, nt.value, 2).clone() if want_stats else None
+    return dict(out=out, copy=cpy, copied=copied.value, pairs=pairs_out, pw=pw.value, flag=int(flag[0].item()))
+
+
 def op_sample_rows(logits, sampling, seeds, positions):
     import torch
     lib = load_library()
```
